# acproject/wsi-segmentation-pipeline

Hardware: AMD Instinct MI355X
Metric: patches/sec (256×256×3) whole-slide inference, 1/2/4/8 MI355X + CPU ref (higher is better)
Workload: dtype fp16 + MX-fp6 cross terms (fp32 accumulate); 1 GPU; cfg3: ONE 40000x40000 synthetic slide, tile 256 stride 256 -> 24648 tiles sharded over 1 rank(s) (each holds only its own slide regions: 4.80 GB on rank 0), ResNet-18 trunk + Classifier, fused read+normalise+conv HIP path, 1 all-gather, float64 stitch + softmax; tiles_total=24648, batch=6200, mode=mx, parallelism=tile-shard x1 + 1 all-gather, batches_in_flight=2

## Files before the change

### include/wsi_hip.h

```cpp
#ifndef WSI_HIP_H
#define WSI_HIP_H
#include <stddef.h>
#include <stdint.h>

#ifdef __cplusplus
extern "C" {
#endif

#define WSI_HIP_ABI_VERSION 8
int wsi_hip_abi_version(void);

size_t wsi_pf_bytes(int n, int h, int w, int c, int planes);
long long wsi_pf_pixel_index(int n, int y, int x, int h, int w);

size_t wsi_prepack_conv_bytes(int cout, int cin, int k, int planes);
int wsi_prepack_conv(const float* w, const float* bn_weight, const float* bn_bias, const float* bn_mean,
                     const float* bn_var, float eps, int cout, int cin, int k, int planes, void* wpk_out,
                     float* bias_out);
size_t wsi_prepack_stem_bytes(int planes);
int wsi_prepack_stem(const float* w, const float* bn_weight, const float* bn_bias, const float* bn_mean,
                     const float* bn_var, float eps, int planes, void* wpk_out, float* bias_out);
int wsi_prepack_stem_u8(const float* w, const float* bn_weight, const float* bn_bias, const float* bn_mean,
                        const float* bn_var, float eps, const float mean[3], const float std_[3], int planes,
                        void* wpk_out, float* bias_out);
int wsi_normalize_u8_lut(const float mean[3], const float std_[3], float* lut_out );

int wsi_stem_conv7x7_bn_relu_maxpool(const float* in_f32, const uint8_t* slide, long long slide_pitch_bytes,
                                     int slide_h, int slide_w, const int* tile_xy, const float* lut,
                                     const void* stem_wpk, const float* stem_bias,
                                     const void* stem_wpk_u8 ,
                                     const float* stem_bias_u8, const float* norm_mean_std ,
                                     int n, int h, int w, float* scratch, void* out_pf, int planes, void* stream);

enum {
    WSI_STEM_MODE_UNFUSED = 0,
    WSI_STEM_MODE_FUSED = 1,
    WSI_STEM_MODE_FUSED_LUT = 2,
    WSI_STEM_MODE_FUSED_ONE_STRIP = 3
};
int wsi_stem_set_mode(int fused, int rows_per_seg);

int wsi_conv3x3_bn_act(const void* in_pf, void* out_pf, const void* resid_pf, const void* wpk, const float* bias,
                       int n, int h_in, int w_in, int cin, int cout, int stride, int relu, int planes,
                       void* stream);
int wsi_conv1x1_bn(const void* in_pf, void* out_pf, const void* wpk, const float* bias, int n, int h_in, int w_in,
                   int cin, int cout, int stride, int planes, void* stream);
int wsi_conv3x3_up_concat_bn_act(const void* up_pf, const void* skip_pf, void* out_pf, const void* wpk, const float* bias, int n, int h, int w,
                                 int c_up, int c_skip, int cout, int relu, int planes, void* stream);
int wsi_conv3x3s2_ds_fused(const void* in_pf, void* out_conv_pf, void* out_ds_pf, const void* wpk3, const float* bias3,
                           const void* wpk1, const float* bias1, int n, int h_in, int w_in, int cin, int cout, int planes,
                           void* stream);
int wsi_s2_slab_images(int n, int h_in, int w_in, int cin, int planes);
size_t wsi_pf_split_bytes(int n, int h, int w, int c, int planes);
int wsi_conv3x3_bn_act_split(const void* in_pf, void* out_split, const void* resid_pf, const void* wpk, const float* bias,
                             int n, int h, int w, int cin, int cout, int relu, int planes, void* stream);
int wsi_conv3x3s2_ds_fused_split(const void* in_split, void* out_conv_pf, void* out_ds_pf, const void* wpk3,
                                 const float* bias3, const void* wpk1, const float* bias1, int n, int h_in, int w_in,
                                 int cin, int cout, int planes, void* stream);
enum {
    WSI_CONV_MODE_S2_GATHER = 0,
    WSI_CONV_MODE_S2_SLAB = 1,
    WSI_CONV_MODE_S2_SLAB_128 = 3,
    WSI_CONV_MODE_XCD_ORDER = 8,
    WSI_CONV_MODE_WIDE_FROM_256 = 16,
    WSI_CONV_MODE_WIDE_NEVER = 32,
    WSI_CONV_MODE_S2_ABLATE = 64,
    WSI_CONV_MODE_NO_S2_SPLIT = 128,
    WSI_CONV_MODE_XCD_RANGES_OFF = 256,
    WSI_CONV_MODE_XCD_RANGES_L1 = 512,
    WSI_CONV_MODE_L1_SLAB3 = 1024,
    WSI_CONV_MODE_NO_DS_FOLD = 2048,
    WSI_CONV_MODE_NO_SLAB_PAIR = 4096,
    WSI_CONV_MODE_L1_LINES128 = 16384,
    WSI_CONV_MODE_S2_NT2 = 32768,
    WSI_CONV_MODE_UNET_CONCAT_PASS = 65536,
    WSI_CONV_MODE_WIDE_NO_D8 = 131072,
    WSI_CONV_MODE_L1_PERSISTENT = 1048576,
    WSI_CONV_MODE_UNET_NO_TAIL = 2097152,
    WSI_CONV_MODE_UNET_TAIL_FORM1 = 4194304,
    WSI_CONV_MODE_UNET_X0_UNFUSED = 8388608
};
int wsi_conv_set_mode(int mode);
int wsi_conv3x3_bn_act_cfg(const void* in_pf, void* out_pf, const void* resid_pf, const void* wpk, const float* bias,
                           int n, int h_in, int w_in, int cin, int cout, int stride, int relu, int planes, int cfg,
                           void* stream);

int wsi_avgpool_fc(const void* in_pf, int n, int h, int w, int c, const float* fc_w, const float* fc_b, int k,
                   float* feat_out, float* logits_out, int planes, void* stream);
int wsi_linear(const float* x, const float* w, const float* bias, float* y, int b, int k, int j, int relu,
               void* stream);

int wsi_pf_pack(const float* in_nchw, void* out_pf, int n, int c, int h, int w, int planes, void* stream);
int wsi_pf_unpack(const void* in_pf, float* out_nchw, int n, int c, int h, int w, int planes, void* stream);

typedef struct {
    const void* stem_w;   const float* stem_b;
    const void* stem_w_u8; const float* stem_b_u8;
    float norm[6];
    const void* conv_w[16]; const float* conv_b[16];
    const void* down_w[3];  const float* down_b[3];
    const float* head_w;  const float* head_b;  int head_k;
    int planes;
} wsi_trunk_weights;

size_t wsi_trunk_workspace_bytes(int n, int h, int w, int planes);
int wsi_trunk_workspace_init(void* workspace, int n, int h, int w, int planes, void* stream);
int wsi_trunk_workspace_release(void* workspace);
int wsi_trunk_forward(const wsi_trunk_weights* wt, const float* in_f32, const uint8_t* slide,
                      long long slide_pitch_bytes, int slide_h, int slide_w, const int* tile_xy, const float* lut,
                      int n, int h, int w, void* workspace, int workspace_n, float* feat_out ,
                      float* logits_out , float* fmap_out ,
                      void* stream);
int wsi_trunk_set_chunks(int stem_chunk, int layer1_chunk);
int wsi_trunk_forward_tap(const wsi_trunk_weights* wt, const float* in_f32, const uint8_t* slide,
                          long long slide_pitch_bytes, int slide_h, int slide_w, const int* tile_xy, const float* lut,
                          int n, int h, int w, void* workspace, int workspace_n, int stop_after, float* tap_out_nchw,
                          void* stream);

int wsi_prof_begin(int max_records);
int wsi_prof_end(float* ms_out, int* kind_out, double* flops_out, int cap);

int wsi_tile_gather(const uint8_t* slide, long long slide_pitch_bytes, int slide_h, int slide_w, const int* tile_xy,
                    const float* lut, float* out_nchw, int n, int ph, int pw, void* stream);
int wsi_stitch_add(const float* tile_logits, const int* map_xy, int t, int c, int dy, int dx, double* pred, int map_h,
                   int map_w, void* stream);
int wsi_stitch_add_dense(const float* tile_pred, const int* map_xy, int t, int c, int ph, int pw, double* pred, int map_h,
                         int map_w, void* stream);
int wsi_softmax_threshold_argmax(const double* pred, int c, long long hw, const double* class_thresh, double* probs,
                                 uint8_t* classes, const uint8_t* mask, int heat_mode, uint8_t* heat, void* stream);
typedef struct wsi_ring wsi_ring;
typedef struct wsi_resample_plan wsi_resample_plan;
int wsi_ring_create(wsi_ring** out, int slots, size_t slot_bytes);
void* wsi_ring_host_slot(wsi_ring* ring, int slot);
int wsi_ring_wait_slot(wsi_ring* ring, int slot);
int wsi_ring_submit(wsi_ring* ring, int slot, int rows, int width, int channels, long long src_pitch, uint8_t* level_rows, long long level_pitch);
int wsi_ring_acquire(wsi_ring* ring, void* compute_stream);
int wsi_ring_fence(wsi_ring* ring, void* compute_stream);
int wsi_ring_device(const wsi_ring* ring);
int wsi_ring_drain(wsi_ring* ring);
void wsi_ring_destroy(wsi_ring* ring);
int wsi_resample_plan_create(wsi_resample_plan** out, int in_h, int in_w, int out_h, int out_w);
void wsi_resample_plan_destroy(wsi_resample_plan* plan);
size_t wsi_resample_scratch_bytes(const wsi_resample_plan* plan, int n);
int wsi_resample_tiles(const wsi_resample_plan* plan, const uint8_t* slide, long long pitch, int sh, int sw, const int* tile_xy, int n,
                       uint8_t* out, void* scratch, void* stream);
int wsi_find_nuclei_hsv(const uint8_t* rgb, long long npix, int pixel_stride, double mu_percent, uint8_t* mask_out, void* stream);
size_t wsi_connected_components_scratch_bytes(int h, int w);
int wsi_connected_components(const uint8_t* mask, int h, int w, int* labels_out, int* count_out, void* scratch, void* stream);
int wsi_kmeans_points(const int* points_xy, int n, double* centres_xy, int k, int max_iters, int* labels_out, void* scratch, void* stream);
int wsi_kmeans_seed_farthest(const int* points_xy, int n, int k, double* centres_xy_out, void* scratch, void* stream);
int wsi_find_nuclei_lab(const uint8_t* rgb, long long npix, int pixel_stride, double mu_percent, uint8_t* mask_out, void* scratch, void* stream);
size_t wsi_fill_holes_scratch_bytes(int h, int w);
int wsi_fill_holes(const uint8_t* mask, int h, int w, uint8_t* out, void* scratch, void* stream);
size_t wsi_slic_scratch_bytes(int h, int w, int k);
int wsi_slic(const uint8_t* rgb, int h, int w, const double* gauss_weights, int radius, double* segments, int k, int step_y, int step_x,
             double step, double compactness, int iters, int* labels_out, void* scratch, void* stream);
long long wsi_tile_grid_candidates(int iw, int ih, int ph, int pw, int sh, int sw);
size_t wsi_tile_grid_scratch_bytes(long long candidates);
int wsi_tile_grid(int iw, int ih, int ph, int pw, int sh, int sw, const uint8_t* mask, int mask_h, int mask_w, double m, double thresh,
                  int* tile_xy_out, int* count_out, void* scratch, void* stream);
int wsi_exponent_span(const float* values, long long n, int* out2, void* stream);
int wsi_paint_regions(const long long* pixel_idx, const int* region_of, long long n, const uint8_t* region_class, int* winner_scratch,
                      long long* label, long long npix, void* stream);

int wsi_resize_bilinear_f64(const double* src, int c, int hs, int ws, double* dst, int hd, int wd, void* stream);
int wsi_argmax_classes(const double* pred, int c, long long hw, uint8_t* classes, void* stream);
int wsi_morph_rect(const uint8_t* src, uint8_t* dst, uint8_t* tmp, int h, int w, int k, int op, void* stream);
int wsi_bwperim(const uint8_t* src, uint8_t* dst, int h, int w, void* stream);
size_t wsi_tumor_bed_workspace_bytes(int h, int w);
int wsi_convex_hull_image(const uint8_t* src, uint8_t* dst, int h, int w, void* workspace, void* stream);
int wsi_tumor_bed(const uint8_t* codes, int h, int w, int min_code, int open_k, int dilate_k, uint8_t* opened_out,
                  uint8_t* tb_pred_out, uint8_t* outline_out, void* workspace, void* stream);
int wsi_hull_polygon(void* workspace, int h, int w, double* out_xy, int cap, int* count_out, void* stream);
int wsi_mask_iou_counts(const uint8_t* a, const uint8_t* b, long long n, unsigned long long* out2, void* stream);
int wsi_score_counts(const uint8_t* p, const uint8_t* gt, const uint8_t* mask, long long n, unsigned long long* out6,
                     void* stream);
int wsi_esp(const double* pts_xy, int n, int num_pts, double* out_xy, double* scratch, void* stream);

typedef struct {
    const void* conv_w[10]; const float* conv_b[10];
    int cin[10], cout[10];
    const float* head_w; const float* head_b;
    int head_cin, classes;
    const void* tail_w;
} wsi_unet_decoder_weights;
size_t wsi_unet_tail_prepack_bytes(void);
int wsi_unet_tail_prepack(const float* w1, const float* bn1_weight, const float* bn1_bias, const float* bn1_mean, const float* bn1_var,
                          const float* w2, const float* bn2_weight, const float* bn2_bias, const float* bn2_mean, const float* bn2_var,
                          float eps, const float* head_w, const float* head_b, int cin, int cmid, int classes, void* out);
int wsi_unet_tail_bands(int n, int h, int cus);
int wsi_unet_tail_timeouts(unsigned long long* out, int reset);
size_t wsi_unet_workspace_bytes(const wsi_unet_decoder_weights* dw, int n, int h, int w, int planes);
int wsi_unet_workspace_init(const wsi_unet_decoder_weights* dw, void* workspace, int n, int h, int w, int planes, void* stream);
int wsi_unet_forward(const wsi_trunk_weights* wt, const wsi_unet_decoder_weights* dw, const float* in_f32, const uint8_t* slide,
                     long long slide_pitch_bytes, int slide_h, int slide_w, const int* tile_xy, const float* lut, int n, int h,
                     int w, void* workspace, int workspace_n, float* logits_out, float* enc_out[5], void* stream);
int wsi_unet_decoder(const wsi_unet_decoder_weights* dw, const float* const enc_nchw[5], int n, int h, int w, int planes,
                     void* workspace, int workspace_n, float* logits_out, void* stream);
int wsi_resize_nearest_f32(const float* src, long long planes_n, int hs, int ws, float* dst, int hd, int wd, void* stream);

#ifdef __cplusplus
}
#endif
#endif
```

### wsi_segmentation_pipeline_amd/csrc/capi.hip

```cpp
#include "internal.h"
#include "../../include/wsi_hip.h"

ConvRoutes g_routes;

StemArgs stem_args(const TileSource& src, const void* wpk, const float* bias, float* scratch, int n, int h, int w) {
    StemArgs a;
    a.mode = src.in_f32 ? 0 : 1;
    a.in_f32 = src.in_f32; a.slide = src.slide; a.slide_pitch = src.pitch; a.SH = src.SH; a.SW = src.SW;
    a.origins = src.tile_xy; a.lut = src.lut; a.wpk = wpk; a.bias = bias; a.out = scratch;
    a.N = n; a.H = h; a.W = w; a.wpk_u8 = nullptr; a.bias_u8 = nullptr;
    return a;
}

int stem_run(const TileSource& src, const void* stem_wpk, const float* stem_bias, const void* stem_wpk_u8, const float* stem_bias_u8,
             const float* norm_mean_std, int n, int h, int w, float* scratch, void* out_pf, int planes, void* stream, int out96,
             long long plane96, void* x0_pf) {
    if (!stem_wpk || !stem_bias || !scratch || !out_pf || n <= 0 || h % 16 || w % 4) return WSI_EINVAL;
    if (!src.valid()) return WSI_EINVAL;
    StemArgs a = stem_args(src, stem_wpk, stem_bias, scratch, n, h, w);
    if (stem_wpk_u8 && stem_bias_u8 && norm_mean_std && !src.in_f32 && g_routes.stem_u8x) { a.wpk_u8 = stem_wpk_u8; a.bias_u8 = stem_bias_u8; }
    if (out96 && planes != 3) return WSI_EINVAL;
    if (x0_pf && !(a.wpk_u8 && g_routes.stem_fused && planes == 2)) return WSI_EINVAL;
    if (g_routes.stem_fused || planes == 3) return wsi_stem_pool_dispatch(a, out_pf, planes, g_routes.stem_rows, (hipStream_t)stream, out96, plane96, x0_pf);
    int rc = wsi_stem_dispatch(a, planes, (hipStream_t)stream);
    if (rc) return rc;
    return wsi_maxpool_dispatch(scratch, out_pf, n, h / 2, w / 2, planes, (hipStream_t)stream);
}

#ifdef WSI_STUDY
static void* g_study_debug = nullptr;
extern "C" int wsi_study_set_debug(void* dev_buf) { g_study_debug = dev_buf; return WSI_OK; }
#endif

static ConvArgs conv_args(const ConvCall& c) {
    ConvArgs a;
    a.in = c.in; a.out = c.out; a.resid = c.resid; a.wpk = c.wpk; a.bias = c.bias;
    a.gi = pf_geom_fd(c.n, c.h, c.w, c.cin);
    a.go = pf_geom_fd(c.n, c.h / c.stride, c.w / c.stride, c.cout);
    a.stride = c.stride; a.ksize = c.ksize; a.relu = c.relu & 1; a.flags = 0;
    a.out2 = nullptr; a.wpk2 = nullptr; a.bias2 = nullptr;
    a.in_split_pixels = 0; a.out_split_pixels = 0;
    return a;
}

int conv_common(const ConvCall& c) {
    const hipStream_t st = (hipStream_t)c.stream;
    int cfg = c.cfg;
    if ((!c.in && !(c.in_up && c.up_c == c.cin)) || !c.out || !c.wpk || !c.bias || c.in == c.out || c.in_up == c.out || c.n <= 0) return WSI_EINVAL;
    if (c.line_flags && (c.planes != 3 || c.stride != 1 || c.ksize != 3 || c.cin != 64 || c.cout != 64 || (c.split_out && (c.line_flags & CONV_OUT96)) ||
                         (c.line_flags & ~(CONV_IN96 | CONV_OUT96 | CONV_RESID96)) || ((c.line_flags & CONV_RESID96) && !c.resid)))
        return WSI_EINVAL;
    if ((c.stride != 1 && c.stride != 2) || c.h % c.stride || c.w % c.stride) return WSI_EINVAL;
    if (c.planes == 3 && c.stride == 2 && c.resid) return WSI_EINVAL;
    ConvArgs a = conv_args(c);
    a.plane96 = c.line_flags ? (c.plane96 > 0 ? c.plane96 : (long long)pf_alloc_pixels(c.n, c.h, c.w) * 96) : 0;
#ifdef WSI_STUDY
    if (c.relu & 2) a.flags |= CONV_ABL_NO_STORE;
    if (c.relu & 64) a.flags |= CONV_ABL_DISPATCH_ONLY;
    if (c.relu & 128) a.flags |= CONV_ABL_NO_MAINLOOP;
    if (c.relu & 256) a.flags |= CONV_NONTEMPORAL;
    if (c.relu & 512) a.flags |= CONV_XCD_ORDER;
    if (c.relu & 16384) a.flags |= CONV_XCD_RANGES;
    if (c.relu & 65536) a.flags |= CONV_RESID_DIRECT;
    a.flags |= ((c.relu >> 10) & 15) << CONV_WCOPIES_SHIFT;
#else
    if (c.relu & ~1) return WSI_EINVAL;
#endif
    a.flags |= c.line_flags;
    if (c.in_up) {
        if (c.stride != 1 || c.ksize != 3 || c.h % 2 || c.w % 2 || c.up_c <= 0 || c.up_c > c.cin || c.resid || c.in2 || c.line_flags || c.split_out) return WSI_EINVAL;
        a.in_up = c.in_up; a.up_c = c.up_c; a.gup = pf_geom_fd(c.n, c.h / 2, c.w / 2, c.up_c);
    }
    if (c.in2) {
        if (c.planes != 3 || c.stride != 1 || c.ksize != 3 || c.resid || !c.wpk2 || !c.bias2 || c.in2_c <= 0 || c.in2_c % 32 || c.cout % 128 || cfg >= 0) return WSI_EINVAL;
        a.in2 = c.in2; a.in2_c = c.in2_c; a.wpk2 = c.wpk2; a.bias2 = c.bias2;
        cfg = 60;
    }
#ifdef WSI_STUDY
    if (cfg == 75 || cfg == 76) a.out2 = g_study_debug;
#endif
    a.out_split_pixels = c.split_out ? (c.split_pixels ? c.split_pixels : pf_alloc_pixels(c.n, c.h / 2, c.w / 2)) : 0;
    if (c.split_out && (c.stride != 1 || c.ksize != 3 || c.h % 2 || c.w % 2 || c.planes < 2)) return WSI_EINVAL;
    if (c.ksize == 3 && c.stride == 2 && c.cout % 128 == 0 && cfg != 0 && g_routes.s2_slab) {
        const int rc = wsi_s2_dispatch(a, c.planes, st);
        if (rc != WSI_EINVAL) return rc;
    }
    return wsi_conv_dispatch(a, c.planes, cfg, st);
}

static ConvArgs s2_ds_args(const void* in, void* out_conv_pf, void* out_ds_pf, const void* wpk3, const float* bias3, const void* wpk1,
                           const float* bias1, int n, int h_in, int w_in, int cin, int cout) {
    ConvArgs a = conv_args({.in = in, .out = out_conv_pf, .wpk = wpk3, .bias = bias3, .n = n, .h = h_in, .w = w_in, .cin = cin, .cout = cout,
                            .stride = 2, .ksize = 3, .relu = 1});
    a.out2 = out_ds_pf; a.wpk2 = out_ds_pf ? wpk1 : nullptr; a.bias2 = out_ds_pf ? bias1 : nullptr;
    return a;
}

static bool s2_ds_ok(const void* in, const void* out_conv_pf, const void* out_ds_pf, const void* wpk3, const float* bias3, const void* wpk1,
                     const float* bias1, int n, int h_in, int w_in, bool ds_optional) {
    if (!in || !out_conv_pf || !wpk3 || !bias3 || n <= 0 || h_in % 2 || w_in % 2) return false;
    if (out_ds_pf ? (!wpk1 || !bias1) : !ds_optional) return false;
    return in != out_conv_pf && in != out_ds_pf && out_conv_pf != out_ds_pf;
}

int s2_split_common(const void* in_split, void* out_conv_pf, void* out_ds_pf, const void* wpk3, const float* bias3, const void* wpk1,
                    const float* bias1, int n, int h_in, int w_in, int cin, int cout, int planes, void* stream, long long split_pixels) {
    if (!s2_ds_ok(in_split, out_conv_pf, out_ds_pf, wpk3, bias3, wpk1, bias1, n, h_in, w_in, true)) return WSI_EINVAL;
    ConvArgs a = s2_ds_args(in_split, out_conv_pf, out_ds_pf, wpk3, bias3, wpk1, bias1, n, h_in, w_in, cin, cout);
    a.in_split_pixels = split_pixels ? split_pixels : pf_alloc_pixels(n, h_in / 2, w_in / 2);
    return wsi_s2_dispatch(a, planes, (hipStream_t)stream);
}

extern "C" {

int wsi_hip_abi_version(void) { return WSI_HIP_ABI_VERSION; }

size_t wsi_pf_bytes(int n, int h, int w, int c, int planes) {
    if (n <= 0 || h <= 0 || w <= 0 || c <= 0 || planes < 1 || planes > 3) return 0;
    return (size_t)pf_alloc_pixels(n, h, w) * (size_t)c * (planes == 1 ? 2 : 4);
}
long long wsi_pf_pixel_index(int n, int y, int x, int h, int w) {
    return (long long)(w + 2) + (long long)n * (h + 1) * (w + 1) + (long long)y * (w + 1) + x;
}

int wsi_stem_set_mode(int fused, int rows_per_seg) {
    if (rows_per_seg <= 0) return WSI_EINVAL;
    g_routes.stem_fused = fused != WSI_STEM_MODE_UNFUSED; g_routes.stem_rows = rows_per_seg;
    g_routes.stem_u8x = fused != WSI_STEM_MODE_FUSED_LUT;
    g_routes.stem_shared_weights = fused != WSI_STEM_MODE_FUSED_ONE_STRIP;
    return WSI_OK;
}

int wsi_stem_conv7x7_bn_relu_maxpool(const float* in_f32, const uint8_t* slide, long long slide_pitch_bytes,
                                     int slide_h, int slide_w, const int* tile_xy, const float* lut,
                                     const void* stem_wpk, const float* stem_bias, const void* stem_wpk_u8,
                                     const float* stem_bias_u8, const float* norm_mean_std, int n, int h, int w,
                                     float* scratch, void* out_pf, int planes, void* stream) {
    return stem_run({in_f32, slide, slide_pitch_bytes, slide_h, slide_w, tile_xy, lut}, stem_wpk, stem_bias, stem_wpk_u8, stem_bias_u8,
                    norm_mean_std, n, h, w, scratch, out_pf, planes, stream, 0);
}

int wsi_conv3x3_bn_act(const void* in_pf, void* out_pf, const void* resid_pf, const void* wpk, const float* bias,
                       int n, int h_in, int w_in, int cin, int cout, int stride, int relu, int planes,
                       void* stream) {
    return conv_common({.in = in_pf, .out = out_pf, .resid = resid_pf, .wpk = wpk, .bias = bias, .n = n, .h = h_in, .w = w_in, .cin = cin,
                        .cout = cout, .stride = stride, .ksize = 3, .relu = relu, .planes = planes, .stream = stream});
}

size_t wsi_pf_split_bytes(int n, int h, int w, int c, int planes) {
    if (h % 2 || w % 2) return 0;
    return 4 * wsi_pf_bytes(n, h / 2, w / 2, c, planes);
}

int wsi_conv3x3_bn_act_split(const void* in_pf, void* out_split, const void* resid_pf, const void* wpk, const float* bias,
                             int n, int h, int w, int cin, int cout, int relu, int planes, void* stream) {
    return conv_common({.in = in_pf, .out = out_split, .resid = resid_pf, .wpk = wpk, .bias = bias, .n = n, .h = h, .w = w, .cin = cin,
                        .cout = cout, .stride = 1, .ksize = 3, .relu = relu, .planes = planes, .stream = stream, .split_out = 1});
}

int wsi_conv3x3s2_ds_fused_split(const void* in_split, void* out_conv_pf, void* out_ds_pf, const void* wpk3,
                                 const float* bias3, const void* wpk1, const float* bias1, int n, int h_in, int w_in,
                                 int cin, int cout, int planes, void* stream) {
    return s2_split_common(in_split, out_conv_pf, out_ds_pf, wpk3, bias3, wpk1, bias1, n, h_in, w_in, cin, cout, planes, stream, 0);
}

int wsi_conv3x3_bn_act_cfg(const void* in_pf, void* out_pf, const void* resid_pf, const void* wpk, const float* bias,
                           int n, int h_in, int w_in, int cin, int cout, int stride, int relu, int planes, int cfg,
                           void* stream) {
    return conv_common({.in = in_pf, .out = out_pf, .resid = resid_pf, .wpk = wpk, .bias = bias, .n = n, .h = h_in, .w = w_in, .cin = cin,
                        .cout = cout, .stride = stride, .ksize = 3, .relu = relu, .planes = planes, .stream = stream, .cfg = cfg});
}

int wsi_conv3x3_up_concat_bn_act(const void* up_pf, const void* skip_pf, void* out_pf, const void* wpk, const float* bias, int n, int h, int w,
                                 int c_up, int c_skip, int cout, int relu, int planes, void* stream) {
    if (!up_pf || c_up <= 0 || c_skip < 0 || (c_skip > 0 && !skip_pf)) return WSI_EINVAL;
    return conv_common({.in = c_skip ? skip_pf : nullptr, .out = out_pf, .wpk = wpk, .bias = bias, .n = n, .h = h, .w = w, .cin = c_up + c_skip,
                        .cout = cout, .stride = 1, .ksize = 3, .relu = relu, .planes = planes, .stream = stream, .in_up = up_pf, .up_c = c_up});
}

int wsi_s2_slab_images(int n, int h_in, int w_in, int cin, int planes) {
    if (n <= 0 || h_in <= 0 || w_in <= 0 || cin <= 0 || planes < 1 || planes > 3) return WSI_EINVAL;
    const unsigned long long pix = (unsigned long long)cin * (planes == 1 ? PFmt<1>::BPC : PFmt<2>::BPC);
    auto fits = [&](int m) { return (unsigned long long)pf_alloc_pixels(m, h_in, w_in) * pix < 0xffffffffull; };
    if (fits(n)) return n;
    if (!fits(1)) return 0;
    int lo = 1, hi = n;
    while (hi - lo > 1) {
        const int mid = lo + (hi - lo) / 2;
        (fits(mid) ? lo : hi) = mid;
    }
    return lo;
}

int wsi_conv3x3s2_ds_fused(const void* in_pf, void* out_conv_pf, void* out_ds_pf, const void* wpk3, const float* bias3,
                           const void* wpk1, const float* bias1, int n, int h_in, int w_in, int cin, int cout, int planes,
                           void* stream) {
    if (!s2_ds_ok(in_pf, out_conv_pf, out_ds_pf, wpk3, bias3, wpk1, bias1, n, h_in, w_in, false)) return WSI_EINVAL;
    ConvArgs a = s2_ds_args(in_pf, out_conv_pf, out_ds_pf, wpk3, bias3, wpk1, bias1, n, h_in, w_in, cin, cout);
    const int per = wsi_s2_slab_images(n, h_in, w_in, cin, planes);
    const size_t bpc = planes == 1 ? PFmt<1>::BPC : PFmt<2>::BPC;
    const size_t in_img = (size_t)(h_in + 1) * (w_in + 1) * cin * bpc, out_img = (size_t)(h_in / 2 + 1) * (w_in / 2 + 1) * cout * bpc;
    int rc = WSI_EINVAL;
    for (int n0 = 0; per > 0 && n0 < n; n0 += per) {
        const int nn = n - n0 < per ? n - n0 : per;
        a.in = (const char*)in_pf + n0 * in_img;
        a.out = (char*)out_conv_pf + n0 * out_img;
        a.out2 = (char*)out_ds_pf + n0 * out_img;
        a.gi = pf_geom_fd(nn, h_in, w_in, cin);
        a.go = pf_geom_fd(nn, h_in / 2, w_in / 2, cout);
        rc = wsi_s2_dispatch(a, planes, (hipStream_t)stream);
        if (rc) break;
    }
    if (rc == WSI_EINVAL) {
        ConvCall c = {.in = in_pf, .out = out_conv_pf, .wpk = wpk3, .bias = bias3, .n = n, .h = h_in, .w = w_in, .cin = cin, .cout = cout,
                      .stride = 2, .ksize = 3, .relu = 1, .planes = planes, .stream = stream, .cfg = 0};
        rc = conv_common(c);
        c.out = out_ds_pf; c.wpk = wpk1; c.bias = bias1; c.ksize = 1; c.relu = 0;
        if (!rc) rc = conv_common(c);
    }
    return rc;
}

int wsi_conv_set_mode(int mode) {
    ConvRoutes& r = g_routes;
    const int base = mode & 7;
    r.s2_slab = base != WSI_CONV_MODE_S2_GATHER;
    r.s2_small_tiles = base != WSI_CONV_MODE_S2_SLAB_128;
    r.xcd_order = (mode & WSI_CONV_MODE_XCD_ORDER) ? 1 : 0;
    r.wide_min_c = (mode & WSI_CONV_MODE_WIDE_FROM_256) ? 256 : (mode & WSI_CONV_MODE_WIDE_NEVER) ? (1 << 30) : 128;
    r.s2_ablate = (mode & WSI_CONV_MODE_S2_ABLATE) ? 1 : 0;
    r.s2_split = (mode & WSI_CONV_MODE_NO_S2_SPLIT) ? 0 : 1;
    r.xcd_ranges = (mode & WSI_CONV_MODE_XCD_RANGES_OFF) ? 0 : (mode & WSI_CONV_MODE_XCD_RANGES_L1) ? 1 : 2;
    r.l1_rows = (mode & WSI_CONV_MODE_L1_SLAB3) ? 0 : 1;
    r.ds_fold = (mode & WSI_CONV_MODE_NO_DS_FOLD) ? 0 : 1;
    r.slab_pair = (mode & WSI_CONV_MODE_NO_SLAB_PAIR) ? 0 : 1;
    r.l1_lines96 = (mode & WSI_CONV_MODE_L1_LINES128) ? 0 : 1;
    r.s2_nt4 = (mode & WSI_CONV_MODE_S2_NT2) ? 0 : 1;
    r.unet_fuse_up = (mode & WSI_CONV_MODE_UNET_CONCAT_PASS) ? 0 : 1;
    r.wide_d8 = (mode & WSI_CONV_MODE_WIDE_NO_D8) ? 0 : 1;
    r.l1p = (mode & WSI_CONV_MODE_L1_PERSISTENT) ? 1 : 0;
    r.unet_tail = (mode & WSI_CONV_MODE_UNET_NO_TAIL) ? 0 : 1;
    r.unet_tail_form = (mode & WSI_CONV_MODE_UNET_TAIL_FORM1) ? 1 : 2;
    r.unet_x0_fused = (mode & WSI_CONV_MODE_UNET_X0_UNFUSED) ? 0 : 1;
    return WSI_OK;
}

int wsi_conv1x1_bn(const void* in_pf, void* out_pf, const void* wpk, const float* bias, int n, int h_in, int w_in,
                   int cin, int cout, int stride, int planes, void* stream) {
    return conv_common({.in = in_pf, .out = out_pf, .wpk = wpk, .bias = bias, .n = n, .h = h_in, .w = w_in, .cin = cin, .cout = cout,
                        .stride = stride, .ksize = 1, .relu = 0, .planes = planes, .stream = stream});
}

int wsi_avgpool_fc(const void* in_pf, int n, int h, int w, int c, const float* fc_w, const float* fc_b, int k,
                   float* feat_out, float* logits_out, int planes, void* stream) {
    if (!in_pf || n <= 0 || (logits_out && (!fc_w || !fc_b || k <= 0))) return WSI_EINVAL;
    return wsi_avgpool_fc_dispatch(in_pf, pf_geom(n, h, w, c), fc_w, fc_b, k, feat_out, logits_out, planes,
                                   (hipStream_t)stream);
}

int wsi_linear(const float* x, const float* w, const float* bias, float* y, int b, int k, int j, int relu,
               void* stream) {
    if (!x || !w || !y) return WSI_EINVAL;
    return wsi_linear_dispatch(x, w, bias, y, b, k, j, relu, (hipStream_t)stream);
}

int wsi_pf_pack(const float* in_nchw, void* out_pf, int n, int c, int h, int w, int planes, void* stream) {
    if (!in_nchw || !out_pf || n <= 0 || planes < 1 || planes > 3 || c % (planes == 1 ? 64 : 32)) return WSI_EINVAL;
    return wsi_pf_pack_dispatch(in_nchw, out_pf, pf_geom(n, h, w, c), planes, (hipStream_t)stream);
}

int wsi_pf_unpack(const void* in_pf, float* out_nchw, int n, int c, int h, int w, int planes, void* stream) {
    if (!in_pf || !out_nchw || n <= 0 || planes < 1 || planes > 3 || c % (planes == 1 ? 64 : 32)) return WSI_EINVAL;
    return wsi_pf_unpack_dispatch(in_pf, out_nchw, pf_geom(n, h, w, c), planes, (hipStream_t)stream);
}

int wsi_tile_gather(const uint8_t* slide, long long slide_pitch_bytes, int slide_h, int slide_w, const int* tile_xy,
                    const float* lut, float* out_nchw, int n, int ph, int pw, void* stream) {
    if (!slide || !tile_xy || !lut || !out_nchw) return WSI_EINVAL;
    return wsi_tile_gather_dispatch(slide, slide_pitch_bytes, slide_h, slide_w, tile_xy, lut, out_nchw, n, ph, pw,
                                    (hipStream_t)stream);
}

int wsi_stitch_add(const float* tile_logits, const int* map_xy, int t, int c, int dy, int dx, double* pred, int map_h,
                   int map_w, void* stream) {
    if (!tile_logits || !map_xy || !pred || map_h <= 0 || map_w <= 0) return WSI_EINVAL;
    return wsi_stitch_add_dispatch(tile_logits, map_xy, t, c, dy, dx, pred, map_h, map_w, (hipStream_t)stream);
}

int wsi_stitch_add_dense(const float* tile_pred, const int* map_xy, int t, int c, int ph, int pw, double* pred, int map_h,
                         int map_w, void* stream) {
    if (!tile_pred || !map_xy || !pred || map_h <= 0 || map_w <= 0) return WSI_EINVAL;
    return wsi_stitch_add_dense_dispatch(tile_pred, map_xy, t, c, ph, pw, pred, map_h, map_w, (hipStream_t)stream);
}

int wsi_softmax_threshold_argmax(const double* pred, int c, long long hw, const double* class_thresh, double* probs,
                                 uint8_t* classes, const uint8_t* mask, int heat_mode, uint8_t* heat, void* stream) {
    if (!pred || !class_thresh) return WSI_EINVAL;
    return wsi_softmax_dispatch(pred, c, hw, class_thresh, probs, classes, mask, heat_mode, heat, (hipStream_t)stream);
}

int wsi_find_nuclei_hsv(const uint8_t* rgb, long long npix, int pixel_stride, double mu_percent, uint8_t* mask_out, void* stream) {
    if (!rgb || !mask_out) return WSI_EINVAL;
    return wsi_hsv_mask_dispatch(rgb, npix, pixel_stride, mu_percent, mask_out, (hipStream_t)stream);
}
size_t wsi_connected_components_scratch_bytes(int h, int w) { return (h <= 0 || w <= 0) ? 0 : wsi_cc_scratch_bytes(h, w); }
int wsi_connected_components(const uint8_t* mask, int h, int w, int* labels_out, int* count_out, void* scratch, void* stream) {
    if (!mask || !labels_out || !scratch) return WSI_EINVAL;
    return wsi_cc_dispatch(mask, h, w, labels_out, count_out, scratch, (hipStream_t)stream);
}
int wsi_find_nuclei_lab(const uint8_t* rgb, long long npix, int pixel_stride, double mu_percent, uint8_t* mask_out, void* scratch, void* stream) {
    return wsi_lab_mask_dispatch(rgb, npix, pixel_stride, mu_percent, mask_out, scratch, (hipStream_t)stream);
}
int wsi_fill_holes(const uint8_t* mask, int h, int w, uint8_t* out, void* scratch, void* stream) {
    return wsi_fill_holes_dispatch(mask, h, w, out, scratch, (hipStream_t)stream);
}
int wsi_slic(const uint8_t* rgb, int h, int w, const double* gauss_weights, int radius, double* segments, int k, int step_y, int step_x,
             double step, double compactness, int iters, int* labels_out, void* scratch, void* stream) {
    return wsi_slic_dispatch(rgb, h, w, gauss_weights, radius, segments, k, step_y, step_x, step, compactness, iters, labels_out, scratch,
                             (hipStream_t)stream);
}
int wsi_kmeans_points(const int* points_xy, int n, double* centres_xy, int k, int max_iters, int* labels_out, void* scratch, void* stream) {
    if (!points_xy || !centres_xy || !labels_out || !scratch) return WSI_EINVAL;
    return wsi_kmeans_dispatch(points_xy, n, centres_xy, k, max_iters, labels_out, scratch, (hipStream_t)stream);
}

int wsi_kmeans_seed_farthest(const int* points_xy, int n, int k, double* centres_xy_out, void* scratch, void* stream) {
    if (!points_xy || !centres_xy_out || !scratch) return WSI_EINVAL;
    return wsi_kmeans_seed_farthest_dispatch(points_xy, n, k, centres_xy_out, scratch, (hipStream_t)stream);
}

int wsi_tile_grid(int iw, int ih, int ph, int pw, int sh, int sw, const uint8_t* mask, int mask_h, int mask_w, double m, double thresh,
                  int* tile_xy_out, int* count_out, void* scratch, void* stream) {
    if (!tile_xy_out || !count_out || !scratch) return WSI_EINVAL;
    return wsi_tile_grid_dispatch(iw, ih, ph, pw, sh, sw, mask, mask_h, mask_w, m, thresh, tile_xy_out, count_out, scratch, (hipStream_t)stream);
}

int wsi_exponent_span(const float* values, long long n, int* out2, void* stream) {
    if (!values || !out2) return WSI_EINVAL;
    return wsi_exponent_span_dispatch(values, n, out2, (hipStream_t)stream);
}

int wsi_paint_regions(const long long* pixel_idx, const int* region_of, long long n, const uint8_t* region_class, int* winner_scratch,
                      long long* label, long long npix, void* stream) {
    if (!region_class || !winner_scratch || !label || (n && (!pixel_idx || !region_of))) return WSI_EINVAL;
    return wsi_paint_dispatch(pixel_idx, region_of, n, region_class, winner_scratch, label, npix, (hipStream_t)stream);
}

int wsi_resize_bilinear_f64(const double* src, int c, int hs, int ws, double* dst, int hd, int wd, void* stream) {
    if (!src || !dst || src == dst) return WSI_EINVAL;
    return wsi_resize_dispatch(src, c, hs, ws, dst, hd, wd, (hipStream_t)stream);
}
int wsi_argmax_classes(const double* pred, int c, long long hw, uint8_t* classes, void* stream) {
    if (!pred || !classes) return WSI_EINVAL;
    return wsi_argmax_dispatch(pred, c, hw, classes, (hipStream_t)stream);
}
int wsi_morph_rect(const uint8_t* src, uint8_t* dst, uint8_t* tmp, int h, int w, int k, int op, void* stream) {
    if (!src || !dst || !tmp) return WSI_EINVAL;
    return wsi_morph_dispatch(src, dst, tmp, h, w, k, op, (hipStream_t)stream);
}
int wsi_bwperim(const uint8_t* src, uint8_t* dst, int h, int w, void* stream) {
    if (!src || !dst) return WSI_EINVAL;
    return wsi_bwperim_dispatch(src, dst, h, w, (hipStream_t)stream);
}
size_t wsi_tumor_bed_workspace_bytes(int h, int w) {
    if (h <= 0 || w <= 0) return 0;
    return 3 * align_up((size_t)h * w, 256) + align_up(wsi_hull_ws_bytes(h), 256);
}
int wsi_convex_hull_image(const uint8_t* src, uint8_t* dst, int h, int w, void* workspace, void* stream) {
    if (!src || !dst || !workspace || src == dst) return WSI_EINVAL;
    return wsi_hull_dispatch(src, dst, h, w, (char*)workspace + 3 * align_up((size_t)h * w, 256), (hipStream_t)stream);
}
int wsi_tumor_bed(const uint8_t* codes, int h, int w, int min_code, int open_k, int dilate_k, uint8_t* opened_out,
                  uint8_t* tb_pred_out, uint8_t* outline_out, void* workspace, void* stream) {
    if (!codes || !tb_pred_out || !outline_out || !workspace || h <= 0 || w <= 0 || open_k <= 0 || dilate_k <= 0 ||
        tb_pred_out == outline_out)
        return WSI_EINVAL;
    hipStream_t st = (hipStream_t)stream;
    const size_t plane = align_up((size_t)h * w, 256);
    uint8_t *A = (uint8_t*)workspace, *B = A + plane, *Cc = B + plane;
    void* hws = Cc + plane;
    int rc = wsi_threshold_dispatch(codes, (long long)h * w, min_code, A, st);
    if (!rc) rc = wsi_morph_dispatch(A, B, Cc, h, w, open_k, 2, st);
    if (!rc && opened_out && hipMemcpyAsync(opened_out, B, (size_t)h * w, hipMemcpyDeviceToDevice, st) != hipSuccess) rc = WSI_EFAULT;
    if (!rc) rc = wsi_hull_dispatch(B, tb_pred_out, h, w, hws, st);
    if (!rc) rc = wsi_bwperim_dispatch(tb_pred_out, A, h, w, st);
    if (!rc) rc = wsi_morph_dispatch(A, outline_out, Cc, h, w, dilate_k, 1, st);
    return rc;
}
int wsi_hull_polygon(void* workspace, int h, int w, double* out_xy, int cap, int* count_out, void* stream) {
    if (!workspace || !out_xy || !count_out || h <= 0 || w <= 0 || cap <= 0) return WSI_EINVAL;
    char* hws = (char*)workspace + 3 * align_up((size_t)h * w, 256);
    int rc = wsi_hull_polygon_dispatch(hws, h, out_xy, cap, (hipStream_t)stream);
    if (rc) return rc;
    const int* counts = (const int*)hws + 2 * (2 * (size_t)h + 1);
    return hipMemcpyAsync(count_out, counts + 2, sizeof(int), hipMemcpyDeviceToDevice, (hipStream_t)stream) == hipSuccess ? WSI_OK : WSI_EFAULT;
}
// ... 20 lines not shown
```

### wsi_segmentation_pipeline_amd/csrc/common.h

```cpp
#pragma once
#include <hip/hip_runtime.h>
#include <stdint.h>

typedef __attribute__((ext_vector_type(8))) __bf16 bf16x8;
typedef __attribute__((ext_vector_type(4))) __bf16 bf16x4;
typedef __attribute__((ext_vector_type(16))) float f32x16;
typedef __attribute__((ext_vector_type(4))) float f32x4;

#define WSI_OK 0
#define WSI_EINVAL (-22)
#define WSI_ENOMEM (-12)
#define WSI_EFAULT (-14)

struct FastDiv { unsigned m; int s; };
static inline FastDiv fastdiv_make(int d) {
    FastDiv f;
    if (d <= 1) { f.m = 0u; f.s = -1; return f; }
    int l = 0;
    while ((1ll << l) < d) ++l;
    f.m = (unsigned)(((1ull << (31 + l)) / (unsigned long long)d) + 1ull);
    f.s = l - 1;
    return f;
}
#ifdef __HIPCC__
static inline __device__ int fd_div(int i, const FastDiv& f) { return f.s < 0 ? i : (int)(__umulhi((unsigned)i, f.m) >> f.s); }
#endif

struct PFGeom {
    int N, H, W, C;
    int P, S, G;
    int NS;
    FastDiv dHW, dW, dS, dP;
};

static inline __host__ __device__ PFGeom pf_geom(int n, int h, int w, int c) {
    PFGeom g;
    g.N = n; g.H = h; g.W = w; g.C = c;
    g.P = w + 1; g.S = (h + 1) * (w + 1); g.G = w + 2; g.NS = n * g.S;
    g.dHW.m = g.dW.m = g.dS.m = g.dP.m = 0u; g.dHW.s = g.dW.s = g.dS.s = g.dP.s = 0;
    return g;
}
static inline PFGeom pf_geom_fd(int n, int h, int w, int c) {
    PFGeom g = pf_geom(n, h, w, c);
    g.dHW = fastdiv_make(h * w); g.dW = fastdiv_make(w); g.dS = fastdiv_make(g.S); g.dP = fastdiv_make(g.P);
    return g;
}
static inline __device__ int pf_pos_of_index(const PFGeom& g, int i) {
    const int n = fd_div(i, g.dHW), rem = i - n * (g.H * g.W);
    const int y = fd_div(rem, g.dW), x = rem - y * g.W;
    return g.G + n * g.S + y * g.P + x;
}

#define PF_TILE_ROUND 512

static inline __host__ __device__ long long pf_alloc_pixels(int n, int h, int w) {
    long long P = w + 1, S = (long long)(h + 1) * P, G = P + 1;
    long long body = ((long long)n * S + PF_TILE_ROUND - 1) / PF_TILE_ROUND * PF_TILE_ROUND;
    return 2 * G + body + PF_TILE_ROUND;
}

static inline __device__ bool pf_is_pixel(const PFGeom& g, int q) {
    int r = q - g.G;
    if (r < 0 || r >= g.NS) return false;
    int x = r % g.P;
    int y = (r / g.P) % (g.H + 1);
    return x != g.W && y != g.H;
}

template <int PLANES> struct PFmt {
    static constexpr int BPC = PLANES == 1 ? 2 : 4;
    static constexpr int CPL = PLANES == 1 ? 64 : 32;
};
typedef __attribute__((ext_vector_type(8))) _Float16 f16x8;
typedef __attribute__((ext_vector_type(4))) _Float16 f16x4;
typedef __attribute__((ext_vector_type(8))) int i32x8;
typedef __attribute__((ext_vector_type(4))) unsigned int u32x4;
typedef __attribute__((ext_vector_type(2))) float f32x2;
typedef __attribute__((ext_vector_type(2))) _Float16 f16x2;
typedef __attribute__((ext_vector_type(4))) int i32x4;

struct ConvArgs {
    const void* in;
    void* out;
    const void* resid;
    const void* wpk;
    const float* bias;
    PFGeom gi, go;
    int stride;
    int ksize;
    int relu;
    int flags;
    void* out2;
    const void* wpk2;
    const float* bias2;
    long long out_split_pixels, in_split_pixels;
    int mtiles = 0;
    const void* in2 = nullptr;
    int in2_c = 0;
    const void* in_up = nullptr;
    int up_c = 0;
    PFGeom gup = {};
    long long plane96 = 0;
};

enum : int {
    CONV_XCD_ORDER = 1,
    CONV_XCD_RANGES = 2,
    CONV_RESID_DIRECT = 4,
    CONV_IN96 = 16, CONV_OUT96 = 32, CONV_RESID96 = 64,
    CONV_ABL_NO_STORE = 1 << 8, CONV_ABL_DISPATCH_ONLY = 1 << 9, CONV_ABL_NO_MAINLOOP = 1 << 10, CONV_NONTEMPORAL = 1 << 11,
    CONV_WCOPIES_SHIFT = 16,
};
#ifdef WSI_STUDY
#define CONV_STUDY(a, bits) ((a).flags & (bits))
#else
#define CONV_STUDY(a, bits) 0
#endif

static inline __device__ size_t pf_out_offset(const PFGeom& g, long long split_pixels, int q, size_t pixstride) {
    if (!split_pixels) return (size_t)q * pixstride;
    int r = q - g.G;
    const int n = fd_div(r, g.dS);
    r -= n * g.S;
    const int y = fd_div(r, g.dP), x = r - y * g.P;
    const int P2 = g.W / 2 + 1, S2 = (g.H / 2 + 1) * P2;
    const long long q2 = (long long)(P2 + 1) + (long long)n * S2 + (y >> 1) * P2 + (x >> 1);
    return (size_t)(((y & 1) * 2 + (x & 1)) * split_pixels + q2) * pixstride;
}

static inline __device__ f32x16 mfma_bf16(bf16x8 a, bf16x8 b, f32x16 c) {
    return __builtin_amdgcn_mfma_f32_32x32x16_bf16(a, b, c, 0, 0, 0);
}
template <int PLANES> struct PairElem { typedef __bf16 T; };
template <> struct PairElem<2> { typedef _Float16 T; };
template <int PLANES>
static inline __device__ f32x16 mfma16(bf16x8 a, bf16x8 b, f32x16 c) {
    typedef __attribute__((ext_vector_type(8))) _Float16 h8;
    if constexpr (PLANES == 2) return __builtin_amdgcn_mfma_f32_32x32x16_f16(__builtin_bit_cast(h8, a), __builtin_bit_cast(h8, b), c, 0, 0, 0);
    else return __builtin_amdgcn_mfma_f32_32x32x16_bf16(a, b, c, 0, 0, 0);
}

typedef __attribute__((ext_vector_type(6))) unsigned u32x6;
typedef __attribute__((ext_vector_type(16))) unsigned u32x16;
typedef __attribute__((ext_vector_type(32))) float f32x32;
static inline __host__ __device__ int mx6_scale_byte(float amax) {
    union { float f; unsigned u; } c;
    c.f = amax;
    const unsigned u = c.u & 0x7fffffffu;
    if (u == 0u) return 0;
    const int e = (int)(u >> 23) - 2 + ((u & 0x7fffffu) > 0x780000u ? 1 : 0);
    return e < 1 ? 1 : (e > 254 ? 254 : e);
}
static inline __host__ __device__ float mx_scale_value(int s) {
    union { float f; unsigned u; } c;
    c.u = (unsigned)s << 23;
    return c.f;
}
static inline __host__ __device__ int mx_line_pos(int c) { return 16 * ((c >> 2) & 1) + 4 * (c >> 3) + (c & 3); }
static inline __host__ __device__ int mx_line_chan(int p) { return 8 * ((p & 15) >> 2) + 4 * (p >> 4) + (p & 3); }
static inline __host__ __device__ int mx6_field_of_pos(int p) { return 2 * (p & 15) + (p >> 4); }
static inline __host__ __device__ int mx6_field_chan(int f) { return mx_line_chan(16 * (f & 1) + (f >> 1)); }
#define MX6_PLANE_LO(q) (64 + 16 * (q))
#define MX6_PLANE_HI(q) (96 + 16 * (q))
#define MX6_SCALE(q) (104 + 16 * (q))

static inline __host__ __device__ float fp6_value(unsigned c) {
    const int e = (c >> 3) & 3, m = c & 7;
    const float v = e ? (float)(8 + m) * (e == 1 ? 0.125f : e == 2 ? 0.25f : 0.5f) : (float)m * 0.125f;
    return (c & 32) ? -v : v;
}
static inline __host__ __device__ unsigned fp6_encode(float y) {
    union { float f; unsigned u; } c;
    c.f = y;
    const unsigned sign = (c.u >> 31) ? 32u : 0u;
    c.u &= 0x7fffffffu;
    const float a = c.f;
    if (!(a < 7.5f)) return sign | 31u;
    const float step = a < 2.f ? 0.125f : a < 4.f ? 0.25f : 0.5f;
    const float t = a / step;
    float r = (float)(int)t;
    const float frac = t - r;
    if (frac > 0.5f || (frac == 0.5f && ((int)r & 1))) r += 1.f;
    const float q = r * step;
    unsigned code;
    if (q < 1.f) code = (unsigned)(q * 8.f);
    else if (q < 2.f) code = 8u + (unsigned)((q - 1.f) * 8.f);
    else if (q < 4.f) code = 16u + (unsigned)((q - 2.f) * 4.f);
    else code = 24u + (unsigned)((q - 4.f) * 2.f);
    return sign | code;
}
static inline __host__ __device__ unsigned mx6_get_field(const unsigned* w, int f) {
    const int bit = 6 * f, d = bit >> 5, s = bit & 31;
    unsigned v = w[d] >> s;
    if (s > 26) v |= w[d + 1] << (32 - s);
    return v & 63u;
}
static inline __host__ __device__ void mx6_set_field(unsigned* w, int f, unsigned code) {
    const int bit = 6 * f, d = bit >> 5, s = bit & 31;
    w[d] |= code << s;
    if (s > 26) w[d + 1] |= code >> (32 - s);
}

#ifdef __HIPCC__
static __device__ __forceinline__ u32x6 mx6_pack32(f32x16 a, f32x16 b, float scale) {
    u32x6 r;
    asm volatile("v_cvt_scalef32_2xpk16_fp6_f32 %0, %1, %2, %3" : "=&v"(r) : "v"(a), "v"(b), "v"(scale));
    return r;
}
static __device__ __forceinline__ f32x32 mx6_unpack32(u32x6 q, float scale) {
    f32x32 r;
    asm volatile("v_cvt_scalef32_pk32_f32_fp6 %0, %1, %2" : "=&v"(r) : "v"(q), "v"(scale));
    return r;
}
static __device__ __forceinline__ void swap32_halves(f32x16& a, f32x16& b) {
#pragma unroll
    for (int k = 0; k < 16; k += 8) {
        float a0 = a[k], a1 = a[k + 1], a2 = a[k + 2], a3 = a[k + 3], a4 = a[k + 4], a5 = a[k + 5], a6 = a[k + 6], a7 = a[k + 7];
        float b0 = b[k], b1 = b[k + 1], b2 = b[k + 2], b3 = b[k + 3], b4 = b[k + 4], b5 = b[k + 5], b6 = b[k + 6], b7 = b[k + 7];
        asm volatile("s_nop 1\n\tv_permlane32_swap_b32 %0, %8\n\tv_permlane32_swap_b32 %1, %9\n\tv_permlane32_swap_b32 %2, %10\n\t"
                     "v_permlane32_swap_b32 %3, %11\n\tv_permlane32_swap_b32 %4, %12\n\tv_permlane32_swap_b32 %5, %13\n\t"
                     "v_permlane32_swap_b32 %6, %14\n\tv_permlane32_swap_b32 %7, %15\n\ts_nop 1"
                     : "+v"(a0), "+v"(a1), "+v"(a2), "+v"(a3), "+v"(a4), "+v"(a5), "+v"(a6), "+v"(a7),
                       "+v"(b0), "+v"(b1), "+v"(b2), "+v"(b3), "+v"(b4), "+v"(b5), "+v"(b6), "+v"(b7));
        a[k] = a0; a[k + 1] = a1; a[k + 2] = a2; a[k + 3] = a3; a[k + 4] = a4; a[k + 5] = a5; a[k + 6] = a6; a[k + 7] = a7;
        b[k] = b0; b[k + 1] = b1; b[k + 2] = b2; b[k + 3] = b3; b[k + 4] = b4; b[k + 5] = b5; b[k + 6] = b6; b[k + 7] = b7;
    }
}
static __device__ __forceinline__ void pair_max2(float& x, float& y) {
    float x2 = x, y2 = y;
    asm volatile("s_nop 1\n\tv_permlane32_swap_b32 %0, %1\n\tv_permlane32_swap_b32 %2, %3\n\ts_nop 1" : "+v"(x), "+v"(x2), "+v"(y), "+v"(y2));
    x = fmaxf(x, x2);
    y = fmaxf(y, y2);
}

#endif

static inline __device__ void split_f16(float x, _Float16& hi, _Float16& lo) {
    x = __builtin_amdgcn_fmed3f(x, -65504.f, 65504.f);
    hi = (_Float16)x;
    lo = (_Float16)(x - (float)hi);
}
static inline __device__ void split_f16x4(const float* v, f16x4& hi, f16x4& lo) {
#pragma unroll
    for (int i = 0; i < 4; ++i) {
        _Float16 a, b;
        split_f16(v[i], a, b);
        hi[i] = a;
        lo[i] = b;
    }
}
static inline __device__ const float* conv_wscale_inv(const void* wpk, int cout, int cin, int ksize) {
    return (const float*)((const char*)wpk + (size_t)(cout / 32) * (cin / 32) * ksize * ksize * 4096);
}

struct StemArgs {
    int mode;
    const float* in_f32;
    const uint8_t* slide;
    long long slide_pitch;
    int SH, SW;
    const int* origins;
    const float* lut;
    const void* wpk;
    const float* bias;
    float* out;
    int N, H, W;
    const void* wpk_u8;
    const float* bias_u8;
    void* out_pf = nullptr;
    int out_planes = 0;
};

struct ConvRoutes {
    int stem_fused = 1;
    int stem_rows = 64;
    int stem_u8x = 1;
    int stem_shared_weights = 1;
    int chunk_stem = 0;
    int chunk_l1 = 0;
    int s2_slab = 1;
    int s2_small_tiles = 1;
    int xcd_order = 0;
    int wide_min_c = 128;
    int s2_ablate = 0;
    int s2_split = 1;
    int xcd_ranges = 2;
    int l1_rows = 1;
    int ds_fold = 1;
    int slab_pair = 1;
    int l1_lines96 = 1;
    int s2_nt4 = 1;
    int unet_fuse_up = 1;
    int wide_d8 = 1;
    int l1p = 0;
    int unet_tail = 1;
    int unet_tail_form = 2;
    int unet_x0_fused = 1;
};
extern ConvRoutes g_routes;
```

### wsi_segmentation_pipeline_amd/csrc/conv.hip

```cpp
#include "conv_dev.h"
#include "internal.h"

template <int MT, int WM, int WN, int PLANES>
__global__ __launch_bounds__(WM* WN * 64) void conv_gather_kernel(ConvArgs a) {
    extern __shared__ __attribute__((aligned(16))) char smem[];
    constexpr int BM = WM * MT * 32;
    constexpr int NTHREADS = WM * WN * 64;
    constexpr int PPT = BM * 8 / NTHREADS;
    constexpr int PIX_STEP = NTHREADS / 8;
    const int tid = threadIdx.x, lane = tid & 63, wave = tid >> 6;
    const int wm = wave / WN, wn = wave % WN;
    const int l31 = lane & 31, h = lane >> 5;
    const int nblocks = a.go.C / (WN * 32);
    const int nb = blockIdx.x % nblocks;
    const int mtile = blockIdx.x / nblocks;
    const int q0 = a.go.G + mtile * BM;
    const int ntile = nb * WN + wn;
    const int NC = a.gi.C / PFmt<PLANES>::CPL;
    const int KS = a.ksize, NT = KS * KS, pad = KS / 2;
    const size_t in_pixstride = (size_t)a.gi.C * PFmt<PLANES>::BPC;
    const bf16x8* wbase = (const bf16x8*)a.wpk + (size_t)ntile * NC * NT * 4 * 64 + lane;

    int inq[PPT];
    const int sp = tid & 7;
// ... 547 lines not shown
        asm volatile("s_waitcnt lgkmcnt(0)" ::: "memory");
        __builtin_amdgcn_s_barrier();
        asm volatile("" ::: "memory");
    };

    const int ntile = wn;
    const __amdgpu_buffer_rsrc_t wrs = __builtin_amdgcn_make_buffer_rsrc(
        (void*)((const char*)a.wpk + (size_t)ntile * NC * 9 * 4096), 0, NC * 9 * 4096, 0x00020000);
    const int wvoff = lane * 16;
    f32x16 acc[1][MT];
    bf16x8 wbuf[3][4], xf[2][4];
    auto wload = [&](bf16x8(&w)[4], int soff) {
#pragma unroll
        for (int f = 0; f < 4; ++f)
            w[f] = __builtin_bit_cast(bf16x8, __builtin_amdgcn_raw_buffer_load_b128(wrs, wvoff, soff + f * 1024, 0));
    };
    const int xoff0 = wm * 32 + l31;

    if (producer) {
        dma_slab(0);
        asm volatile("s_waitcnt vmcnt(0)" ::: "memory");
    }
    barrier();
    if (producer && nunits > 1) dma_slab(1);
    mx96_rebuild_hi6(smem, NPIX, tid, 320);
    barrier();

    for (int k = 0; k < ntl; ++k) {
#pragma unroll
    for (int c = 0; c < NC; ++c) {
        const int u = k * NC + c;
        const bool last_line = c == NC - 1;
        if (producer) {
            asm volatile("s_waitcnt vmcnt(0)" ::: "memory");
        } else {
            const char* const xl = smem + (c & 1) * L1P_SLAB;
            auto xload = [&](bf16x8(&x)[4], int Pl) {
                asm volatile("" : "+v"(Pl));
                const int base = lds_xbase(Pl, h);
#pragma unroll
                for (int f = 0; f < 4; ++f) x[f] = *(const bf16x8*)(xl + (base ^ (f << 5)));
            };
            if (c == 0) acc_init_bias<MT>(acc[0], a.bias, ntile, lane);
#pragma unroll
            for (int dy = 0; dy < 3; ++dy) wload(wbuf[dy], (c * 9 + dy * 3) * 4096);
            int Pc = P;
            asm volatile("" : "+s"(Pc));
            const int sline = c * 9 * 4096;
            xload(xf[0], xoff0);
#pragma unroll
            for (int dx = 0; dx < 3; ++dx) {
#pragma unroll
                for (int j = 0; j < 6; ++j) {
                    const int kk = dx * 6 + j;
                    if (j < 5) xload(xf[(kk + 1) & 1], xoff0 + (j + 1) * Pc + dx);
                    else if (dx < 2) xload(xf[(kk + 1) & 1], xoff0 + dx + 1);
                    __builtin_amdgcn_sched_barrier(0);
#pragma unroll
                    for (int mt = 0; mt < MT; ++mt) {
                        const int dy = j - mt;
                        if (dy >= 0 && dy < 3) acc[0][mt] = mfma_mx6(acc[0][mt], wbuf[dy], xf[kk & 1]);
                    }
                    __builtin_amdgcn_sched_barrier(0);
                    if (j >= 3 && dx < 2) {
                        wload(wbuf[j - 3], sline + ((j - 3) * 3 + dx + 1) * 4096);
                        __builtin_amdgcn_sched_barrier(0);
                    }
                }
            }
        }
        barrier();
        if (producer) {
            if (u + 2 < nunits) dma_slab(u + 2);
            if (a.resid && u + 1 < nunits && (u + 1) % NC == NC - 1) dma_resid((u + 1) / NC);
        }
        if (u + 1 < nunits) mx96_rebuild_hi6(smem + ((c + 1) & 1) * L1P_SLAB, NPIX, tid, 320);
        barrier();
        if (!producer && last_line) {
            const int p0 = tile_p0(k);
            int qs[MT];
            bool valid[MT];
#pragma unroll
            for (int mt = 0; mt < MT; ++mt) {
                qs[mt] = p0 + mt * P + wm * 32 + l31;
                valid[mt] = true;
            }
            if (a.resid) {
                bf16x8 iw[4];
                {
                    int lo = l31;
                    asm volatile("" : "+v"(lo));
                    const int pp = mx_line_pos(lo), f0 = mx6_field_of_pos(pp);
                    f16x8 k0, k1;
#pragma unroll
                    for (int jj = 0; jj < 8; ++jj) {
                        k0[jj] = (pp == 8 * h + jj) ? (_Float16)1.0f : (_Float16)0.0f;
                        k1[jj] = (pp == 16 + 8 * h + jj) ? (_Float16)1.0f : (_Float16)0.0f;
                    }
                    unsigned q[6];
#pragma unroll
                    for (int d = 0; d < 6; ++d) {
                        const int bit = 6 * f0 + 3 - 32 * d;
                        q[d] = (h == 0 && bit >= 0 && bit < 32) ? (1u << (bit & 31)) : 0u;
                    }
                    iw[0] = __builtin_bit_cast(bf16x8, k0);
                    iw[1] = __builtin_bit_cast(bf16x8, k1);
                    iw[2] = __builtin_bit_cast(bf16x8, u32x4{q[0], q[1], q[2], q[3]});
                    iw[3] = __builtin_bit_cast(bf16x8, u32x4{q[4], q[5], 127u, 0u});
                }
#pragma unroll
                for (int mt = 0; mt < MT; ++mt) {
                    const char* t = stage + (wave * MT + mt) * 3072 + l31 * 96;
                    bf16x8 x[4];
                    x[0] = *(const bf16x8*)(t + h * 16);
                    x[1] = *(const bf16x8*)(t + (2 + h) * 16);
                    if (h == 0) {
                        x[2] = *(const bf16x8*)(t + 4 * 16);
                        x[3] = *(const bf16x8*)(t + 5 * 16);
                    } else {
                        x[2] = __builtin_bit_cast(bf16x8, u32x4{0u, 0u, 0u, 0u});
                        x[3] = x[2];
                    }
                    acc[0][mt] = mfma_mx6(acc[0][mt], iw, x);
                }
            }
            conv_epilogue_mx<MT>(a, acc[0], qs, valid, ntile, lane);
        }
    }
    }
}

static int g_l1p_grid = 0;
static int launch_l1p(const ConvArgs& a, hipStream_t st) {
    if (a.go.C != 64 || a.gi.C % 32 || a.gi.C < 64 || a.gi.W != 64 || a.gi.H % 4 || a.in2 || a.in_up || !(a.flags & CONV_IN96) ||
        (a.resid && !(a.flags & CONV_RESID96)))
        return WSI_EINVAL;
    if (!g_l1p_grid) {
        int dev = 0, cus = 0;
        if (hipGetDevice(&dev) != hipSuccess || hipDeviceGetAttribute(&cus, hipDeviceAttributeMultiprocessorCount, dev) != hipSuccess || cus < 8)
            return WSI_EFAULT;
        g_l1p_grid = cus / 8 * 8;
    }
    const long long mtiles = (long long)a.gi.N * a.gi.H * a.gi.W / 256;
    int grid = g_l1p_grid;
    if (mtiles < grid) grid = (int)((mtiles + 7) / 8 * 8);
    if (a.gi.C != 64) return WSI_EINVAL;
    auto k = conv3x3s1_l1p_kernel<2>;
    if (hipFuncSetAttribute((const void*)k, hipFuncAttributeMaxDynamicSharedMemorySize, L1P_LDS) != hipSuccess) return WSI_EINVAL;
    hipLaunchKernelGGL(k, dim3(grid), dim3(320), L1P_LDS, st, a);
    return hipGetLastError() == hipSuccess ? WSI_OK : WSI_EFAULT;
}


template <int PLANES, int MINW, int ABL = 0, int WM = 2, int WN = 2, int NT = 2, bool D8 = false>
__global__ __launch_bounds__(WM* WN * 64, MINW) void conv3x3s1_wide_kernel(ConvArgs a) {
    extern __shared__ __attribute__((aligned(16))) char smem[];
    constexpr int MT = 4, BM = WM * 128, NTHREADS = WM * WN * 64, NTILES = WN * NT, WB = NTILES * 4096;
    constexpr int D8_ZB = 304;
    static_assert(!D8 || (BM == 256 && NTHREADS == 256), "D8: four whole 8 x 8 images per tile, 32 slab pixels per DMA round");
    constexpr int RESID_NBUF = 4;
    char* const wl = smem;
    char* const xl = smem + 2 * WB;
    const int tid = threadIdx.x, lane = tid & 63;
    WSTAMP(const unsigned long long st_begin = __builtin_readcyclecounter(); unsigned long long st_pro = 0, st_line = 0, st_tap = 0, st_a = 0;)
    const int wave = __builtin_amdgcn_readfirstlane(tid >> 6);
    const int wm = wave / WN, wn = wave % WN;
    const int l31 = lane & 31, h = lane >> 5;
    const int nblocks = a.go.C / (NTILES * 32);
    int nb = blockIdx.x % nblocks, mtile = blockIdx.x / nblocks;
    if (a.flags & CONV_XCD_RANGES) {
        const int chunk = gridDim.x >> 3, lin = (blockIdx.x & 7) * chunk + (blockIdx.x >> 3);
        nb = lin % nblocks;
        mtile = lin / nblocks;
        if (mtile >= (a.gi.N * a.gi.H * a.gi.W + BM - 1) / BM) return;
    }
    const int P = a.gi.P;
    const int NC = a.gi.C / PFmt<PLANES>::CPL;
    const size_t in_pixstride = (size_t)a.gi.C * PFmt<PLANES>::BPC;
    int xoff[MT];
    bool valid[MT];
    int slab0, npieces;
    const int lpix = a.gi.W < 32 ? dense_lane_pixel(l31) : l31;
    const int Rtot = a.gi.N * a.gi.H * a.gi.W;
    if constexpr (D8) {
        const int i0 = mtile * BM, i1 = min(i0 + BM, Rtot) - 1, n0 = i0 >> 6;
        slab0 = a.gi.G + n0 * a.gi.S - P;
        npieces = (1 + 9 * ((i1 >> 6) - n0 + 1)) * 64;
#pragma unroll
        for (int mt = 0; mt < MT; ++mt) {
            const int i = i0 + wm * MT * 32 + mt * 32 + lpix;
            valid[mt] = i < Rtot;
            const int ii = valid[mt] ? i : i1;
            xoff[mt] = 8 * (9 * ((ii >> 6) - n0) + ((ii >> 3) & 7)) + (ii & 7) - 1;
        }
    } else {
        auto pos = [&](int i) { return pf_pos_of_index(a.gi, i); };
        const int i0 = mtile * BM, i1 = min(i0 + BM, Rtot) - 1;
        slab0 = pos(i0) - P - 1;
        npieces = (pos(i1) + P + 1 - slab0 + 1) * 8;
#pragma unroll
        for (int mt = 0; mt < MT; ++mt) {
            const int i = i0 + wm * MT * 32 + mt * 32 + lpix;
            valid[mt] = i < Rtot;
            xoff[mt] = pos(valid[mt] ? i : i1) - slab0 - (P + 1);
        }
    }
    const bool d8_left = D8 && (lpix & 7) == 0, d8_right = D8 && (lpix & 7) == 7;
    constexpr int RPIX = D8 ? 36 : NTHREADS / 8;
    static_assert((NTHREADS / 8) % 16 == 0, "whole swizzle periods per DMA round");
    const size_t slab_byte0 = (size_t)slab0 * in_pixstride;
    const size_t in_bytes = (size_t)pf_alloc_pixels(a.gi.N, a.gi.H, a.gi.W) * in_pixstride;
    const __amdgpu_buffer_rsrc_t xrs = __builtin_amdgcn_make_buffer_rsrc(
        (void*)((const char*)a.in + slab_byte0), 0, (int)min(in_bytes - slab_byte0, (size_t)0x7fffffff), 0x00020000);
    int xvoff;
    {
        const int i = wave * 64 + lane, Pl = i >> 3, sl = (i & 7) ^ ((Pl >> 1) & 7);
        xvoff = (D8 ? (Pl >> 3) * 9 + (Pl & 7) : Pl) * (int)in_pixstride + sl * 16;
    }
    if constexpr (D8) {
        if (tid < 128) *(u32x4*)(xl + D8_ZB * 128 + tid * 16) = u32x4{0u, 0u, 0u, 0u};
    }
    const __amdgpu_buffer_rsrc_t wrs = __builtin_amdgcn_make_buffer_rsrc(
        (void*)((const char*)a.wpk + (size_t)(nb * NTILES) * NC * 9 * 4096), 0, NTILES * NC * 9 * 4096, 0x00020000);
    const int wvoff = (tid & 255) * 16;
    const unsigned wl_addr = lds_addr_of(wl), xl_addr = lds_addr_of(xl);
    auto wdma = [&](int c, int t, int wboff) {
#pragma unroll
        for (int p0 = 0; p0 < NTILES * 256; p0 += NTHREADS) {
            static_assert((NTILES * 256) % NTHREADS == 0, "whole DMA rounds");
            const int pw = p0 + wave * 64;
            dma16_buf_asm(wrs, wl_addr + wboff + pw * 16, wvoff, (((pw >> 8) * NC + c) * 9 + t) * 4096);
        }
    };

    f32x16 acc[NT][MT];
#pragma unroll
    for (int nt = 0; nt < NT; ++nt) {
        if constexpr (PLANES == 3) acc_init_bias<MT>(acc[nt], a.bias, nb * NTILES + wn * NT + nt, lane);
        else {
#pragma unroll
            for (int mt = 0; mt < MT; ++mt)
#pragma unroll
                for (int r = 0; r < 16; ++r) acc[nt][mt][r] = 0.f;
        }
    }

    auto xload = [&](bf16x8(&x)[4], int Pl, int tx = 1) {
        asm volatile("" : "+v"(Pl));
        if constexpr (D8) {
            if (tx == 0) Pl = d8_left ? D8_ZB + (Pl & 15) : Pl;
            if (tx == 2) Pl = d8_right ? D8_ZB + (Pl & 15) : Pl;
        }
        const int base = lds_xbase(Pl, h);
#pragma unroll
        for (int f = 0; f < 4; ++f) x[f] = *(const bf16x8*)(xl + (base ^ (f << 5)));
    };
    auto wread = [&](bf16x8(&w)[4], const char* wb, int nt) {
        const char* src = wb + (wn * NT + nt) * 4096 + lane * 16;
#pragma unroll
        for (int f = 0; f < 4; ++f) w[f] = *(const bf16x8*)(src + f * 1024);
    };

    int kpar = 0;
    WSTAMP(const unsigned long long st_setup = __builtin_readcyclecounter();)
    for (int c = 0; c < NC; ++c) {
        WSTAMP(st_a = __builtin_readcyclecounter();)
        if (c) __syncthreads();
        for (int i0 = wave * 64, r = 0; i0 < npieces; i0 += NTHREADS, ++r)
            dma16_buf_asm(xrs, xl_addr + i0 * 16, xvoff, c * 128 + r * RPIX * (int)in_pixstride);
        wdma(c, 0, kpar * WB);
        asm volatile("s_waitcnt vmcnt(0)" ::: "memory");
        __syncthreads();
        WSTAMP(if (c) st_line += __builtin_readcyclecounter() - st_a; else st_pro = __builtin_readcyclecounter() - st_a;)
        int Pc = D8 ? 8 : P;
        asm volatile("" : "+s"(Pc));
        bf16x8 xf[2][4], wf[NT][4];
        xload(xf[0], xoff[0], 0);
#pragma unroll
        for (int t = 0; t < 9; ++t) {
            const char* wb = wl + kpar * WB;
            if (t < 8) wdma(c, t + 1, (kpar ^ 1) * WB);
#pragma unroll
            for (int nt = 0; nt < NT; ++nt) wread(wf[nt], wb, nt);
            const int toff = (t / 3) * Pc + (t % 3);
            const int toff_next = ((t + 1) / 3) * Pc + ((t + 1) % 3);
#pragma unroll
            for (int mt = 0; mt < MT; ++mt) {
                const int k = t * MT + mt;
                if constexpr (!(ABL & 32)) {
                    if (mt + 1 < MT) xload(xf[(k + 1) & 1], xoff[mt + 1] + toff, t % 3);
                    else if (t < 8) xload(xf[(k + 1) & 1], xoff[0] + toff_next, (t + 1) % 3);
                }
                __builtin_amdgcn_sched_barrier(0);
                const bf16x8(&x)[4] = xf[k & 1];
#pragma unroll
                for (int nt = 0; nt < NT; ++nt) {
                    mfma_step<PLANES>(acc[nt][mt], wf[nt], x);
                }
            }
            if (t < 8) {
                WSTAMP(st_a = __builtin_readcyclecounter();)
                asm volatile("s_waitcnt vmcnt(0)" ::: "memory");
                __syncthreads();
                WSTAMP(st_tap += __builtin_readcyclecounter() - st_a;)
            }
            kpar ^= 1;
        }
    }
    WSTAMP(const unsigned long long st_loop_end = __builtin_readcyclecounter();)
    int qs[MT];
#pragma unroll
    for (int mt = 0; mt < MT; ++mt) {
        if constexpr (D8) {
            const int i = mtile * BM + wm * MT * 32 + mt * 32 + lpix;
            qs[mt] = pf_pos_of_index(a.gi, valid[mt] ? i : min(mtile * BM + BM, Rtot) - 1);
        } else {
            qs[mt] = xoff[mt] + slab0 + (P + 1);
        }
    }
    if constexpr (PLANES == 3) {
        if (a.in2) {
            const int NC2 = a.in2_c / 32;
            const size_t ps2 = (size_t)a.in2_c * 4, sb2 = (size_t)slab0 * ps2;
            const size_t bytes2 = (size_t)pf_alloc_pixels(a.gi.N, a.gi.H, a.gi.W) * ps2;
            const __amdgpu_buffer_rsrc_t xrs2 = __builtin_amdgcn_make_buffer_rsrc(
                (void*)((const char*)a.in2 + sb2), 0, (int)min(bytes2 - sb2, (size_t)0x7fffffff), 0x00020000);
            int xvoff2;
            {
                const int i = wave * 64 + lane, Pl = i >> 3, sl = (i & 7) ^ ((Pl >> 1) & 7);
                xvoff2 = (D8 ? (Pl >> 3) * 9 + (Pl & 7) : Pl) * (int)ps2 + sl * 16;
            }
            const char* wsrc2 = (const char*)a.wpk2 + (size_t)(nb * NTILES) * NC2 * 4096 + (size_t)(tid & 255) * 16;
#pragma unroll
            for (int nt = 0; nt < NT; ++nt) {
                f32x16 b2[1];
                acc_init_bias<1>(b2, a.bias2, nb * NTILES + wn * NT + nt, lane);
#pragma unroll
                for (int mt = 0; mt < MT; ++mt)
#pragma unroll
                    for (int r = 0; r < 16; ++r) acc[nt][mt][r] += b2[0][r];
            }
            for (int c = 0; c < NC2; ++c) {
                __syncthreads();
                for (int i0 = wave * 64, r = 0; i0 < npieces; i0 += NTHREADS, ++r)
                    dma16_buf(xrs2, xl + (size_t)i0 * 16, xvoff2, c * 128 + r * RPIX * (int)ps2);
#pragma unroll
                for (int p0 = 0; p0 < NTILES * 256; p0 += NTHREADS) {
                    const int pw = p0 + wave * 64;
                    dma16(wsrc2 + (size_t)((pw >> 8) * NC2 + c) * 4096, wl + pw * 16);
                }
                asm volatile("s_waitcnt vmcnt(0)" ::: "memory");
                __syncthreads();
                bf16x8 wf2[NT][4];
#pragma unroll
                for (int nt = 0; nt < NT; ++nt) wread(wf2[nt], wl, nt);
#pragma unroll
                for (int mt = 0; mt < MT; ++mt) {
                    bf16x8 x2[4];
                    xload(x2, xoff[mt] + (D8 ? 8 : P) + 1);
#pragma unroll
                    for (int nt = 0; nt < NT; ++nt) mfma_step<PLANES>(acc[nt][mt], wf2[nt], x2);
                }
            }
        }
        if (a.resid) __syncthreads();
        conv_tail_mx<NT, MT, RESID_NBUF>(a, acc, qs, valid, nb * NTILES + wn * NT, lane, smem + wave * (RESID_NBUF * 4096), slab0);
    } else {
        char* scratch = nullptr;
        if (PLANES == 2 && a.resid && !(a.flags & CONV_RESID_DIRECT)) {
            __syncthreads();
            scratch = xl + wave * 8192;
        }
#pragma unroll
        for (int nt = 0; nt < NT; ++nt) conv_epilogue_q<MT, PLANES>(a, acc[nt], qs, valid, nb * NTILES + wn * NT + nt, lane, scratch);
    }
#ifdef WSI_STUDY
    asm volatile("s_waitcnt vmcnt(0)" ::: "memory");
    if (lane == 0 && (blockIdx.x & 63) == 0) {
        const unsigned long long st_end = __builtin_readcyclecounter();
        atomicAdd(&g_wide_stamps[0], 1ull);
        atomicAdd(&g_wide_stamps[1], st_end - st_begin);
        atomicAdd(&g_wide_stamps[2], st_setup - st_begin);
        atomicAdd(&g_wide_stamps[3], st_pro);
        atomicAdd(&g_wide_stamps[4], st_line);
        atomicAdd(&g_wide_stamps[5], st_tap);
        atomicAdd(&g_wide_stamps[6], st_end - st_loop_end);
    }
#endif
}


template <int PLANES, int MINW, int ABL = 0, int WM = 2, int WN = 2, int NT = 2, bool D8 = false>
static int launch_wide(const ConvArgs& a, hipStream_t st) {
    constexpr int BM = WM * 128, NTHREADS = WM * WN * 64, BN = WN * NT * 32;
    if (a.go.C % BN) return WSI_EINVAL;
    if constexpr (!D8 && ABL == 0 && WM == 2 && WN == 2 && NT == 2) {
        if (g_routes.wide_d8 && a.gi.W == 8 && a.gi.H == 8) return launch_wide<PLANES, MINW, 0, 2, 2, 2, true>(a, st);
    }
    const int nblocks = a.go.C / BN;
    const long long R = (long long)a.gi.N * a.gi.H * a.gi.W;
    const int mtiles = (int)((R + BM - 1) / BM);
    size_t xbytes = D8 ? (size_t)(304 + 16) * 128
                       : (size_t)((dense_max_slab_pixels(a, BM) * 8 + NTHREADS - 1) / NTHREADS * NTHREADS) * 16;
    if (xbytes < (size_t)WM * WN * 8192) xbytes = (size_t)WM * WN * 8192;
    size_t lds = 2 * (BN / 32) * 4096 + xbytes;
    if (PLANES == 3 && lds < (size_t)WM * WN * 4 * 4096) lds = (size_t)WM * WN * 4 * 4096;
    if (lds > 160 * 1024) return WSI_EINVAL;
    auto k = conv3x3s1_wide_kernel<PLANES, MINW, ABL, WM, WN, NT, D8>;
    if (lds > 64 * 1024 && hipFuncSetAttribute((const void*)k, hipFuncAttributeMaxDynamicSharedMemorySize, (int)lds) != hipSuccess)
        return WSI_EINVAL;
    const int grid = (a.flags & CONV_XCD_RANGES) ? (mtiles * nblocks + 7) / 8 * 8 : mtiles * nblocks;
    hipLaunchKernelGGL(k, dim3(grid), dim3(NTHREADS), lds, st, a);
    return hipGetLastError() == hipSuccess ? WSI_OK : WSI_EFAULT;
}


template <int MT, int WM, int WN, int PLANES, int MINW, bool FUSE, int PMAX = 34, int ABL = 0>
__global__ __launch_bounds__(WM* WN * 64, MINW) void conv3x3s2_slab_kernel(ConvArgs a) {
    extern __shared__ __attribute__((aligned(16))) char smem[];
    constexpr int BM = WM * MT * 32;
    constexpr int NTHREADS = WM * WN * 64;
    constexpr int KMAX = ((4 * BM + 2 * PMAX + 2) * 8 + NTHREADS - 1) / NTHREADS;
    constexpr int NT = FUSE ? 10 : 9;
    constexpr int RING = FUSE ? 2 : 3;
    const int tid = threadIdx.x, lane = tid & 63;
    const int wave = __builtin_amdgcn_readfirstlane(tid >> 6);
    const int wm = wave / WN, wn = wave % WN;
    const int l31 = lane & 31, h = lane >> 5;
    const int nblocks = a.go.C / (WN * 32);
    int nb = blockIdx.x % nblocks, mtile = blockIdx.x / nblocks;
    if (a.flags & CONV_XCD_ORDER) {
        const int per = 8 * nblocks, r = blockIdx.x % per;
        nb = r >> 3;
        mtile = (blockIdx.x / per) * 8 + (r & 7);
        if (mtile >= (a.go.NS + BM - 1) / BM) return;
    }
    const int P = a.go.P;
    const int q0 = a.go.G + mtile * BM;
    const int R01 = BM, R10 = 2 * BM + 1, R11 = 3 * BM + 1 + P;
    const int npix = 4 * BM + 2 * P + 2;
    const int npieces = npix * 8;
    const int ntile = nb * WN + wn;
    const int NC = a.gi.C / PFmt<PLANES>::CPL;
    const size_t in_pixstride = (size_t)a.gi.C * PFmt<PLANES>::BPC;
    const __amdgpu_buffer_rsrc_t wrs = __builtin_amdgcn_make_buffer_rsrc(
        (void*)((const char*)a.wpk + (size_t)ntile * NC * 9 * 4096), 0, NC * 9 * 4096, 0x00020000);
    const __amdgpu_buffer_rsrc_t wrd = __builtin_amdgcn_make_buffer_rsrc(
        (void*)((const char*)(FUSE ? a.wpk2 : a.wpk) + (size_t)ntile * NC * 4096), 0, NC * 4096, 0x00020000);
    const int wvoff = lane * 16;

    int srcpix[KMAX];
#pragma unroll
    for (int k = 0; k < KMAX; ++k) {
        const int i = wave * 64 + k * NTHREADS + lane;
        const int Pl = i >> 3;
        int reg = 0, j = Pl;
        if (Pl >= R11) { reg = 3; j = Pl - R11; }
        else if (Pl >= R10) { reg = 2; j = Pl - R10; }
        else if (Pl >= R01) { reg = 1; j = Pl - R01; }
        const int py = reg >> 1, px = reg & 1;
        const int v = q0 - (py ? P : 0) - px + j;
        int src = 0;
        int r = v - a.go.G;
        if (Pl < npix && r >= 0 && r < a.go.NS) {
            const int n = r / a.go.S;
            r -= n * a.go.S;
            const int y = r / P, x = r - y * P;
            if (x != a.go.W && y != a.go.H) src = a.gi.G + n * a.gi.S + (2 * y + py) * a.gi.P + 2 * x + px;
        }
        const int sl = (i & 7) ^ ((Pl >> 1) & 7);
        srcpix[k] = (int)((unsigned)src * (unsigned)in_pixstride + (unsigned)sl * 16u);
    }
    const __amdgpu_buffer_rsrc_t irs = __builtin_amdgcn_make_buffer_rsrc((void*)a.in, 0, 0xffffffff, 0x00020000);

    f32x16 acc[MT], accd[FUSE ? MT : 1];
    if constexpr (PLANES == 3) {
        acc_init_bias<MT>(acc, a.bias, ntile, lane);
        if constexpr (FUSE) acc_init_bias<MT>(accd, a.bias2, ntile, lane);
    } else {
#pragma unroll
        for (int mt = 0; mt < MT; ++mt)
#pragma unroll
            for (int r = 0; r < 16; ++r) acc[mt][r] = 0.f;
        if constexpr (FUSE) {
#pragma unroll
            for (int mt = 0; mt < MT; ++mt)
#pragma unroll
                for (int r = 0; r < 16; ++r) accd[mt][r] = 0.f;
        }
    }
    int xoff[MT];
#pragma unroll
    for (int mt = 0; mt < MT; ++mt) xoff[mt] = wm * MT * 32 + mt * 32 + l31;

    auto wload = [&](bf16x8(&w)[4], int c, int t) {
#pragma unroll
        for (int f = 0; f < 4; ++f) {
            const u32x4 v = (t < 9) ? __builtin_amdgcn_raw_buffer_load_b128(wrs, wvoff + f * 1024, (c * 9 + t) * 4096, 0)
                                    : __builtin_amdgcn_raw_buffer_load_b128(wrd, wvoff + f * 1024, c * 4096, 0);
            w[f] = __builtin_bit_cast(bf16x8, v);
        }
    };
    auto xload = [&](bf16x8(&x)[4], int Pl) {
        const int base = lds_xbase(Pl, h);
#pragma unroll
        for (int f = 0; f < 4; ++f) x[f] = *(const bf16x8*)(smem + (base ^ (f << 5)));
    };
    auto tap_off = [&](int t, int Pc) {
        if (t == 9) return 0;
        const int kh = t / 3, kw = t % 3;
        const int py = kh != 1, px = kw != 1;
        const int base = py ? (px ? 3 * BM + 1 + Pc : 2 * BM + 1) : (px ? BM : 0);
        const int back = (py ? Pc : 0) + px;
        return base + back + (kh == 0 ? -Pc : 0) + (kw == 0 ? -1 : 0);
    };

    bf16x8 wbuf[RING][4], xf[2][4];
    wload(wbuf[0], 0, 0);
    for (int c = 0; c < NC; ++c) {
        int Pc = P;
        asm volatile("" : "+s"(Pc));
        if (c) __syncthreads();
#pragma unroll
        for (int k = 0; k < KMAX; ++k) {
            const int i0 = wave * 64 + k * NTHREADS;
            if (i0 < npieces)
                dma16_buf(irs, smem + (size_t)i0 * 16, srcpix[k], c * 128);
        }
        asm volatile("s_waitcnt vmcnt(0)" ::: "memory");
        __syncthreads();
        xload(xf[0], xoff[0] + tap_off(0, Pc));
#pragma unroll
        for (int t = 0; t < NT; ++t) {
            asm volatile("" ::: "memory");
            if constexpr (!(ABL & 16)) {
                if (t + 1 < NT) wload(wbuf[(t + 1) % RING], c, t + 1);
                else if (c + 1 < NC) wload(wbuf[0], c + 1, 0);
            }
            asm volatile("" ::: "memory");
            const int toff = tap_off(t, Pc);
            const int toff_next = t + 1 < NT ? tap_off(t + 1, Pc) : 0;
#pragma unroll
            for (int mt = 0; mt < MT; ++mt) {
                const int k = t * MT + mt;
                if (mt + 1 < MT) xload(xf[(k + 1) & 1], xoff[mt + 1] + toff);
                else if (t + 1 < NT) xload(xf[(k + 1) & 1], xoff[0] + toff_next);
                const bf16x8(&w)[4] = wbuf[t % RING];
                const bf16x8(&x)[4] = xf[k & 1];
                f32x16& d = (FUSE && t == 9) ? accd[FUSE ? mt : 0] : acc[mt];
                if constexpr (PLANES == 3) {
                    d = mfma_mx6(d, w, x);
                } else if constexpr (PLANES == 2) {
                    mfma_step<2>(d, w, x);
                } else {
#pragma unroll
                    for (int f = 0; f < 4; ++f) d = mfma_bf16(w[f], x[f], d);
                }
            }
        }
    }
    conv_epilogue_any<MT, PLANES>(a, acc, q0 + wm * MT * 32, ntile, lane);
// ... 198 lines not shown
        if constexpr (DS) {
            ConvArgs a2 = a;
            a2.out = a.out2; a2.bias = a.bias2; a2.resid = nullptr; a2.relu = 0;
            a2.wpk = a.wpk2; a2.ksize = 1;
            if constexpr (PLANES == 3) conv_epilogue_mx<MT>(a2, accd[nt], qs, valid, ntile, lane);
            else conv_epilogue_q<MT, PLANES>(a2, accd[nt], qs, valid, ntile, lane);
        }
    }
}

template <int PLANES>
static int launch_s2wide(const ConvArgs& a, hipStream_t st) {
    constexpr int BM = 256, XB = 45056;
    const bool ds = a.out2 != nullptr;
    if (a.go.C % 128 || a.go.P > 34 || !a.in_split_pixels || (ds && (!a.wpk2 || !a.bias2)) || a.out_split_pixels) return WSI_EINVAL;
    const long long R = (long long)a.go.N * a.go.H * a.go.W;
    const bool nt4 = !ds && PLANES == 3 && g_routes.s2_nt4 && a.go.C % 256 == 0;
    const int nblocks = a.go.C / (nt4 ? 256 : 128);
    ConvArgs g = a;
    g.gi = a.go;
    const long long span = dense_max_slab_pixels(g, BM) - (a.go.P + 1);
    const bool dense = (span * 8 + 255) / 256 * 256 * 16 <= XB;
    const int mtiles = dense ? (int)((R + BM - 1) / BM) : (a.go.NS + BM - 1) / BM;
    const size_t lds = 4 * 16384 + 2 * XB;
    auto k = nt4 ? (dense ? conv3x3s2_wide_kernel<PLANES, true, false, 4> : conv3x3s2_wide_kernel<PLANES, false, false, 4>)
           : dense ? (ds ? conv3x3s2_wide_kernel<PLANES, true, true> : conv3x3s2_wide_kernel<PLANES, true, false>)
                   : (ds ? conv3x3s2_wide_kernel<PLANES, false, true> : conv3x3s2_wide_kernel<PLANES, false, false>);
    if (hipFuncSetAttribute((const void*)k, hipFuncAttributeMaxDynamicSharedMemorySize, (int)lds) != hipSuccess) return WSI_EINVAL;
    ConvArgs b = a;
    b.mtiles = mtiles;
    hipLaunchKernelGGL(k, dim3((mtiles * nblocks + 7) / 8 * 8), dim3(512), lds, st, b);
    return hipGetLastError() == hipSuccess ? WSI_OK : WSI_EFAULT;
}

int wsi_s2_dispatch(const ConvArgs& a_in, int planes, hipStream_t st) {
    ConvArgs a = a_in;
    if (a.in_split_pixels)
        return planes == 3 ? launch_s2wide<3>(a, st) : planes == 2 ? launch_s2wide<2>(a, st) : WSI_EINVAL;
    if (g_routes.xcd_order && a.go.C > 128) a.flags |= CONV_XCD_ORDER;
    if (a.gi.C % 64 || a.go.C % 128 || planes < 1 || planes > 3) return WSI_EINVAL;
    if (a.go.H * 2 != a.gi.H || a.go.W * 2 != a.gi.W || a.gi.N != a.go.N) return WSI_EINVAL;
    const bool fuse = a.out2 != nullptr;
    if (fuse && (!a.wpk2 || !a.bias2)) return WSI_EINVAL;
    if (a.go.P > 34) {
        if (planes == 3) return fuse ? launch_s2slab<2, 1, 4, 3, 2, true, 130>(a, st) : launch_s2slab<2, 1, 4, 3, 2, false, 130>(a, st);
        if (planes == 2) return fuse ? launch_s2slab<2, 1, 4, 2, 2, true, 130>(a, st) : launch_s2slab<2, 1, 4, 2, 2, false, 130>(a, st);
        return WSI_EINVAL;
    }
#ifdef WSI_STUDY
    if (g_routes.s2_ablate && planes == 3 && fuse) return launch_s2slab<2, 1, 4, 3, 3, true, 34, 16>(a, st);
#endif
    if (g_routes.s2_small_tiles) {
        if (planes == 3) return fuse ? launch_s2slab<2, 1, 4, 3, 3, true>(a, st) : launch_s2slab<2, 1, 4, 3, 3, false>(a, st);
        if (planes == 2) return fuse ? launch_s2slab<2, 1, 4, 2, 3, true>(a, st) : launch_s2slab<2, 1, 4, 2, 3, false>(a, st);
    }
    if (planes == 3) return fuse ? launch_s2slab<4, 1, 4, 3, 2, true>(a, st) : launch_s2slab<4, 1, 4, 3, 2, false>(a, st);
    if (planes == 2) return fuse ? launch_s2slab<4, 1, 4, 2, 2, true>(a, st) : launch_s2slab<4, 1, 4, 2, 2, false>(a, st);
    return fuse ? launch_s2slab<4, 1, 4, 1, 2, true>(a, st) : launch_s2slab<4, 1, 4, 1, 2, false>(a, st);
}

template <int MT, int WM, int WN, int PLANES>
static int launch_gather(const ConvArgs& a, hipStream_t st) {
    constexpr int BM = WM * MT * 32;
    if (a.go.C % (WN * 32)) return WSI_EINVAL;
    const int mtiles = (a.go.NS + BM - 1) / BM;
    const int nblocks = a.go.C / (WN * 32);
    const size_t lds = (size_t)BM * 128;
    hipLaunchKernelGGL((conv_gather_kernel<MT, WM, WN, PLANES>), dim3(mtiles * nblocks), dim3(WM * WN * 64), lds, st, a);
    return hipGetLastError() == hipSuccess ? WSI_OK : WSI_EFAULT;
}

#define SLAB3_CFGS(X) \
    X(20, 4, 1, 4, 2, false) \
    X(21, 4, 2, 2, 2, false) \
    X(25, 2, 2, 4, 3, false) \
    X(27, 4, 4, 2, 1, false) \
    X(28, 2, 2, 2, 3, true) \
    X(29, 2, 2, 2, 4, true) \
    X(39, 4, 4, 2, 1, true) \
    X(26, 4, 1, 2, 3, false) \
    X(30, 4, 1, 4, 2, true) \
    X(31, 4, 2, 2, 2, true) \
    X(32, 2, 2, 4, 3, true) \
    X(33, 8, 1, 4, 2, true) \
    X(34, 8, 1, 2, 2, true) \
    X(35, 8, 2, 2, 2, true) \
    X(36, 4, 2, 4, 2, true) \
    X(37, 4, 1, 4, 3, true) \
    X(38, 4, 2, 2, 3, true)



int wsi_slab_dispatch_cfg(const ConvArgs& a_in, int planes, int cfg, hipStream_t st) {
    ConvArgs a = a_in;
    if (g_routes.xcd_order && cfg >= 20 && cfg < 40 && !CONV_STUDY(a, ~7)) a.flags |= CONV_XCD_ORDER;
    if (g_routes.xcd_ranges && !CONV_STUDY(a, ~7) && ((cfg >= 20 && cfg < 42) || cfg == 60 || cfg == 90 || cfg == 91 || (cfg >= 70 && cfg < 90)) && (g_routes.xcd_ranges == 2 || a.go.C == 64)) a.flags |= CONV_XCD_RANGES;
    if ((a.flags & CONV_IN96) && !((cfg >= 20 && cfg <= 42) || cfg == 90 || cfg == 91)) return WSI_EINVAL;
    if (a.in_up && !((cfg >= 20 && cfg < 40) || cfg == 90 || cfg == 91)) return WSI_EINVAL;
    if (cfg < 20) return WSI_EINVAL;
    if (cfg >= 70 && cfg < 90) return wsi_pp_dispatch(a, planes, cfg, st);
    if (cfg == 90) return planes == 3 ? launch_slab3<2, 8, 1, 3, 1, true>(a, st) : planes == 2 ? launch_slab3<2, 8, 1, 2, 1, true>(a, st) : WSI_EINVAL;
    if (cfg == 91) return planes == 3 ? launch_slab3<2, 4, 1, 3, 2, true>(a, st) : planes == 2 ? launch_slab3<2, 4, 1, 2, 2, true>(a, st) : WSI_EINVAL;
    if (cfg == 42) return planes == 3 ? launch_l1p(a, st) : WSI_EINVAL;
    if (cfg == 40) return planes == 3 ? launch_rows<3>(a, st) : WSI_EINVAL;
    if (cfg == 41) return planes == 3 ? launch_rows<2>(a, st) : WSI_EINVAL;
    if (cfg == 60) return planes == 3 ? launch_wide<3, 2>(a, st) : planes == 2 ? launch_wide<2, 2>(a, st) : launch_wide<1, 2>(a, st);
#ifdef WSI_STUDY
    if (cfg == 61 && planes == 3) return launch_wide<3, 2, 32>(a, st);
    if (cfg == 67) return planes == 3 ? launch_wide<3, 1, 0, 4, 2, 1>(a, st) : planes == 2 ? launch_wide<2, 1, 0, 4, 2, 1>(a, st) : WSI_EINVAL;
    if (cfg == 68) return planes == 3 ? launch_wide<3, 2, 0, 2, 2, 1>(a, st) : planes == 2 ? launch_wide<2, 2, 0, 2, 2, 1>(a, st) : WSI_EINVAL;
    if (cfg >= 50 && cfg <= 53 && planes == 3) {
        switch (cfg) {
        case 50: return launch_slab3<4, 1, 4, 3, 2, true, 16>(a, st);
        case 51: return launch_slab3<4, 1, 4, 3, 2, true, 32>(a, st);
        case 52: return launch_slab3<4, 1, 4, 3, 2, true, 48>(a, st);
        case 53: return launch_slab3<4, 1, 4, 3, 2, true, 8>(a, st);
        }
    }
    switch (cfg) {
#define X(id, MT, WM, WN, MINW, DENSE) \
    case id: return planes == 3 ? launch_slab3<MT, WM, WN, 3, MINW, DENSE>(a, st) \
                  : planes == 2 ? launch_slab3<MT, WM, WN, 2, MINW, DENSE>(a, st) : launch_slab3<MT, WM, WN, 1, MINW, DENSE>(a, st);
        SLAB3_CFGS(X)
#undef X
    }
#else
    if (cfg == 30) return planes == 3 ? launch_slab3<4, 1, 4, 3, 2, true>(a, st) : planes == 2 ? launch_slab3<4, 1, 4, 2, 2, true>(a, st) : launch_slab3<4, 1, 4, 1, 2, true>(a, st);
    if (cfg == 31) return planes == 3 ? launch_slab3<4, 2, 2, 3, 2, true>(a, st) : planes == 2 ? launch_slab3<4, 2, 2, 2, 2, true>(a, st) : launch_slab3<4, 2, 2, 1, 2, true>(a, st);
    if (cfg == 38) {
        if (planes != 3) return WSI_EINVAL;
        const int rc = g_routes.slab_pair ? launch_slab3<4, 2, 2, 3, 3, true, 0, true>(a, st) : WSI_EINVAL;
        return rc != WSI_EINVAL ? rc : launch_slab3<4, 2, 2, 3, 3, true>(a, st);
    }
    if (cfg == 39) return planes == 3 ? launch_slab3<4, 4, 2, 3, 1, true>(a, st) : planes == 2 ? launch_slab3<4, 4, 2, 2, 1, true>(a, st) : launch_slab3<4, 4, 2, 1, 1, true>(a, st);
#endif
    return WSI_EINVAL;
}

static int slab_default_cfg(const ConvArgs& a, int planes, bool fallback) {
    if (a.go.C % 64) return fallback ? 91 : 90;
    if (a.in_up) return a.go.C % 128 == 0 ? 30 : (a.gi.W > 128 && !fallback ? 39 : 31);
    if (a.gi.W <= 4 && a.go.C % 128 == 0 && planes == 3) return 30;
    if (a.go.C % 128 == 0 && a.go.C >= g_routes.wide_min_c && !(planes == 1 && a.gi.W > 33)) return 60;
    if (a.go.C % 128 != 0 && a.gi.W > 128 && !fallback) return 39;
    if (a.go.C == 64 && a.gi.C == 64 && planes == 3 && !fallback && g_routes.l1_rows && g_routes.l1p && a.gi.W == 64 && a.gi.H % 4 == 0 && !a.in2 && (a.flags & CONV_IN96) &&
        (!a.resid || (a.flags & CONV_RESID96)))
        return 42;
    if (a.go.C % 128 != 0 && planes == 3 && !fallback && g_routes.l1_rows && a.gi.W == 64 && a.gi.H % 4 == 0 && !a.in2) return 40;
    if (a.go.C % 128 != 0 && planes == 3 && !fallback && a.gi.W != 64) return 31;
    if (a.go.C % 128 != 0 && planes == 3 && !fallback) return 38;
    return a.go.C % 128 == 0 ? 30 : 31;
}

int wsi_conv_dispatch(const ConvArgs& a, int planes, int cfg, hipStream_t st) {
    const int cout = a.go.C;
    if (planes < 1 || planes > 3) return WSI_EINVAL;
    const int cmul = planes == 1 ? 64 : 32;
    if (a.gi.C % cmul || cout % cmul) return WSI_EINVAL;
    if ((a.gi.C % 64 || cout % 64) && !(a.ksize == 3 && a.stride == 1)) return WSI_EINVAL;
    if (planes == 3 && !(a.ksize == 3 && a.stride == 1)) return WSI_EINVAL;
    if (a.ksize == 3 && a.stride == 1) {
        if (a.gi.H != a.go.H || a.gi.W != a.go.W || a.gi.N != a.go.N) return WSI_EINVAL;
        if (cfg >= 0) return wsi_slab_dispatch_cfg(a, planes, cfg, st);
        const int rc = wsi_slab_dispatch_cfg(a, planes, slab_default_cfg(a, planes, false), st);
        return rc != WSI_EINVAL ? rc : wsi_slab_dispatch_cfg(a, planes, slab_default_cfg(a, planes, true), st);
    }
    if ((a.ksize == 3 || a.ksize == 1) && (a.stride == 1 || a.stride == 2)) {
        if (a.go.H * a.stride != a.gi.H || a.go.W * a.stride != a.gi.W || a.gi.N != a.go.N) return WSI_EINVAL;
        if (cout % 128 == 0) return planes == 2 ? launch_gather<8, 1, 4, 2>(a, st) : launch_gather<8, 1, 4, 1>(a, st);
        return planes == 2 ? launch_gather<4, 2, 2, 2>(a, st) : launch_gather<4, 2, 2, 1>(a, st);
    }
    return WSI_EINVAL;
}
```

### wsi_segmentation_pipeline_amd/csrc/conv_dev.h

```cpp
#pragma once
#include "common.h"

static __device__ __forceinline__ void dma16(const void* gsrc, char* lds_wave_base) {
    __builtin_amdgcn_global_load_lds((const __attribute__((address_space(1))) void*)gsrc,
                                     (__attribute__((address_space(3))) void*)lds_wave_base, 16, 0, 0);
}

static __device__ __forceinline__ void dma16_buf(__amdgpu_buffer_rsrc_t rs, char* lds_wave_base, int voff, int soff) {
    __builtin_amdgcn_raw_ptr_buffer_load_lds(rs, (__attribute__((address_space(3))) void*)lds_wave_base, 16, voff, soff, 0, 0);
}

static __device__ __forceinline__ unsigned lds_addr_of(const char* p) {
    return (unsigned)(size_t)(const __attribute__((address_space(3))) char*)p;
}
static __device__ __forceinline__ void dma16_asm(const void* gsrc, unsigned lds) {
    unsigned keep;
    asm volatile("s_mov_b32 %0, m0\n\ts_mov_b32 m0, %1\n\ts_nop 0\n\tglobal_load_lds_dwordx4 %2, off\n\ts_mov_b32 m0, %0"
                 : "=&s"(keep) : "s"(lds), "v"(gsrc) : "memory");
}
static __device__ __forceinline__ void dma16_buf_asm(__amdgpu_buffer_rsrc_t rs, unsigned lds, int voff, int soff) {
    unsigned keep;
    asm volatile("s_mov_b32 %0, m0\n\ts_mov_b32 m0, %1\n\ts_nop 0\n\tbuffer_load_dwordx4 %2, %3, %4 offen lds\n\ts_mov_b32 m0, %0"
                 : "=&s"(keep) : "s"(lds), "v"(voff), "s"(rs), "s"(soff) : "memory");
}
// ... 89 lines not shown
            }
    }
    float bias[16], wsi[16];
#pragma unroll
    for (int g = 0; g < 4; ++g)
#pragma unroll
        for (int i = 0; i < 4; ++i) bias[g * 4 + i] = a.bias[ntile * 32 + 8 * g + 4 * h + i];
    if constexpr (PLANES == 2) {
        const float* ws = conv_wscale_inv(a.wpk, a.go.C, a.gi.C, a.ksize) + ntile * 32 + 4 * h;
#pragma unroll
        for (int g = 0; g < 4; ++g) {
            const f32x4 v = *(const f32x4*)(ws + 8 * g);
#pragma unroll
            for (int i = 0; i < 4; ++i) wsi[g * 4 + i] = v[i];
        }
    }
#pragma unroll
    for (int mt = 0; mt < MT; ++mt) {
        if (via_lds) {
            asm volatile("s_waitcnt vmcnt(0)" ::: "memory");
            if (mt + 1 < MT)
                resid_tile_dma(a.resid, valid[mt + 1] ? qs[mt + 1] : a.go.G, pixstride, (size_t)ntile * 128, lane, scratch + ((mt + 1) & 1) * 4096);
            const char* t = scratch + (mt & 1) * 4096 + l31 * 128 + 8 * h;
            const int sw = (l31 >> 1) & 7;
#pragma unroll
            for (int g = 0; g < 4; ++g) {
                rh[mt][g] = *(const Ex4*)(t + ((g ^ sw) << 4));
                rl[mt][g] = *(const Ex4*)(t + (((4 + g) ^ sw) << 4));
            }
        }
#pragma unroll
        for (int g = 0; g < 4; ++g) {
            float v[4];
#pragma unroll
            for (int i = 0; i < 4; ++i) {
                if constexpr (PLANES == 2) v[i] = acc[mt][4 * g + i] * wsi[4 * g + i] + bias[4 * g + i];
                else v[i] = acc[mt][4 * g + i] + bias[4 * g + i];
            }
            if (a.resid) {
#pragma unroll
                for (int i = 0; i < 4; ++i) v[i] += (float)rh[mt][g][i];
                if constexpr (PLANES == 2) {
#pragma unroll
                    for (int i = 0; i < 4; ++i) v[i] += (float)rl[mt][g][i];
                }
            }
            Ex4 hi, lo;
            if constexpr (PLANES == 2) {
                const float lo_clamp = a.relu ? 0.f : -65504.f;
#pragma unroll
                for (int i = 0; i < 4; ++i) {
                    v[i] = __builtin_amdgcn_fmed3f(v[i], lo_clamp, 65504.f);
                    hi[i] = (E)v[i];
                    lo[i] = (E)(v[i] - (float)hi[i]);
                }
            } else {
                if (a.relu) {
#pragma unroll
                    for (int i = 0; i < 4; ++i) v[i] = fmaxf(v[i], 0.f);
                }
#pragma unroll
                for (int i = 0; i < 4; ++i) {
                    hi[i] = (E)v[i];
                    lo[i] = (E)(v[i] - (float)hi[i]);
                }
            }
            if (valid[mt] && !CONV_STUDY(a, CONV_ABL_NO_STORE)) {
                char* op = (char*)a.out + ooff[mt] + 16 * g;
                if (CONV_STUDY(a, CONV_NONTEMPORAL)) {
                    __builtin_nontemporal_store(hi, (Ex4*)op);
                    if constexpr (PLANES == 2) __builtin_nontemporal_store(lo, (Ex4*)(op + 64));
                } else {
                    *(Ex4*)op = hi;
                    if constexpr (PLANES == 2) *(Ex4*)(op + 64) = lo;
                }
            }
        }
    }
}

static __device__ __forceinline__ f32x16 mfma_mx6(f32x16 d, const bf16x8 (&w)[4], const bf16x8 (&x)[4]) {
    d = __builtin_amdgcn_mfma_f32_32x32x16_f16(__builtin_bit_cast(f16x8, w[0]), __builtin_bit_cast(f16x8, x[0]), d, 0, 0, 0);
    d = __builtin_amdgcn_mfma_f32_32x32x16_f16(__builtin_bit_cast(f16x8, w[1]), __builtin_bit_cast(f16x8, x[1]), d, 0, 0, 0);
    const i32x4 wq = __builtin_bit_cast(i32x4, w[2]), wr = __builtin_bit_cast(i32x4, w[3]);
    const i32x4 xq = __builtin_bit_cast(i32x4, x[2]), xr = __builtin_bit_cast(i32x4, x[3]);
    const i32x8 wa = {wq[0], wq[1], wq[2], wq[3], wr[0], wr[1], wr[2], wr[3]}, xa = {xq[0], xq[1], xq[2], xq[3], xr[0], xr[1], xr[2], xr[3]};
    return __builtin_amdgcn_mfma_scale_f32_32x32x64_f8f6f4(wa, xa, d, 2, 2, 0, wr[2], 0, xr[2]);
}

template <int MT>
static __device__ __forceinline__ void acc_init_bias(f32x16 (&acc)[MT], const float* bias, int ntile, int lane) {
    const int h = lane >> 5;
    float b[16];
#pragma unroll
    for (int g = 0; g < 4; ++g) {
        const f32x4 v = *(const f32x4*)(bias + ntile * 32 + 8 * g + 4 * h);
#pragma unroll
        for (int i = 0; i < 4; ++i) b[4 * g + i] = v[i];
    }
#pragma unroll
    for (int mt = 0; mt < MT; ++mt)
#pragma unroll
        for (int r = 0; r < 16; ++r) acc[mt][r] = b[r];
}

template <int MT, int MTN = MT>
static __device__ __forceinline__ void conv_epilogue_mx(const ConvArgs& a, f32x16 (&acc)[MT], const int (&qs)[MT],
                                                        const bool (&valid)[MT], int ntile, int lane, int mt0 = 0) {
    const int h = lane >> 5;
    const bool o96 = a.flags & CONV_OUT96;
    const size_t pixstride = o96 ? (size_t)96 : (size_t)a.go.C * 4;
    const float lo_clamp = a.relu ? 0.f : -65504.f;
#pragma unroll
    for (int mt = mt0; mt < mt0 + MTN; ++mt) {
        const size_t loff = (size_t)(valid[mt] ? qs[mt] : a.go.G) * pixstride + (o96 ? (size_t)ntile * (size_t)a.plane96 : (size_t)ntile * 128);
        f32x16 v = acc[mt];
        f32x16 hi, lo;
        f16x8 hv[2];
        float mv = 0.f, ml = 0.f;
#pragma unroll
        for (int r = 0; r < 16; r += 2) {
            const float v0 = __builtin_amdgcn_fmed3f(v[r], lo_clamp, 65504.f);
            const float v1 = __builtin_amdgcn_fmed3f(v[r + 1], lo_clamp, 65504.f);
            const f16x2 hh = __builtin_convertvector(f32x2{v0, v1}, f16x2);
            hv[r >> 3][r & 7] = hh[0];
            hv[r >> 3][(r & 7) + 1] = hh[1];
            hi[r] = (float)hh[0];
            hi[r + 1] = (float)hh[1];
            lo[r] = v0 - hi[r];
            lo[r + 1] = v1 - hi[r + 1];
            mv = fmaxf(mv, fmaxf(fabsf(hi[r]), fabsf(hi[r + 1])));
            ml = fmaxf(ml, fmaxf(fabsf(lo[r]), fabsf(lo[r + 1])));
        }
        pair_max2(mv, ml);
        const int sh = mx6_scale_byte(mv), sl = mx6_scale_byte(ml);
        const int sb = h ? sh : sl;
        swap32_halves(lo, hi);
        const u32x6 q = mx6_pack32(lo, hi, sb ? mx_scale_value(sb) : 1.f);
        if (valid[mt] && !CONV_STUDY(a, CONV_ABL_NO_STORE)) {
            char* ol = (char*)a.out + (a.out_split_pixels ? pf_out_offset(a.go, a.out_split_pixels, qs[mt], pixstride) + (size_t)ntile * 128 : loff);
            *(f16x8*)(ol + 32 * h) = hv[0];
            *(f16x8*)(ol + 32 * h + 16) = hv[1];
            if (!o96) {
                *(u32x4*)(ol + MX6_PLANE_LO(0) + 16 * h) = u32x4{q[0], q[1], q[2], q[3]};
                *(u32x4*)(ol + MX6_PLANE_HI(0) + 16 * h) = u32x4{q[4], q[5], (unsigned)sb, 0u};
            } else if (h == 0) {
                *(u32x4*)(ol + 64) = u32x4{q[0], q[1], q[2], q[3]};
                *(u32x4*)(ol + 80) = u32x4{q[4], q[5], (unsigned)sl, (unsigned)sh};
            }
        }
    }
}

template <int NT, int MT, int NBUF>
static __device__ __forceinline__ void conv_tail_mx(const ConvArgs& a, f32x16 (&acc)[NT][MT], const int (&qs)[MT], const bool (&valid)[MT],
                                                    int ntile0, int lane, char* scratch, int slab0) {
    constexpr int T = NT * MT;
    static_assert(MT % NBUF == 0 || NBUF % MT == 0, "a batch is part of one channel tile or whole channel tiles");
    static_assert(NBUF <= T && T % NBUF == 0, "whole batches");
    if (!a.resid) {
#pragma unroll
        for (int nt = 0; nt < NT; ++nt) conv_epilogue_mx<MT>(a, acc[nt], qs, valid, ntile0 + nt, lane);
        return;
    }
    const int h = lane >> 5, l31 = lane & 31;
    const bool r96 = a.flags & CONV_RESID96;
    const int pixstride = r96 ? 96 : a.go.C * 4;
    const size_t rbase = (size_t)slab0 * pixstride, rbytes = (size_t)pf_alloc_pixels(a.go.N, a.go.H, a.go.W) * pixstride;
    const __amdgpu_buffer_rsrc_t rrs = __builtin_amdgcn_make_buffer_rsrc((void*)((const char*)a.resid + rbase), 0,
                                                                          (int)min(rbytes - rbase, (size_t)0x7fffffff), 0x00020000);
    bf16x8 iw[4];
    {
        const int p = mx_line_pos(l31), f0 = mx6_field_of_pos(p);
        f16x8 k0, k1;
#pragma unroll
        for (int j = 0; j < 8; ++j) {
            k0[j] = (p == 8 * h + j) ? (_Float16)1.0f : (_Float16)0.0f;
            k1[j] = (p == 16 + 8 * h + j) ? (_Float16)1.0f : (_Float16)0.0f;
        }
        unsigned q[6];
#pragma unroll
        for (int d = 0; d < 6; ++d) {
            const int bit = 6 * f0 + 3 - 32 * d;
            q[d] = (h == 0 && bit >= 0 && bit < 32) ? (1u << (bit & 31)) : 0u;
        }
        iw[0] = __builtin_bit_cast(bf16x8, k0);
        iw[1] = __builtin_bit_cast(bf16x8, k1);
        iw[2] = __builtin_bit_cast(bf16x8, u32x4{q[0], q[1], q[2], q[3]});
        iw[3] = __builtin_bit_cast(bf16x8, u32x4{q[4], q[5], 127u, 0u});
    }
    auto rdma = [&](int k) {
        const int nt = k / MT, mt = k % MT;
        int qr = qs[mt] - slab0;
        asm volatile("" : "+v"(qr));
        if (r96) {
            const __amdgpu_buffer_rsrc_t prs = __builtin_amdgcn_make_buffer_rsrc(
                (void*)((const char*)a.resid + (size_t)(ntile0 + nt) * (size_t)a.plane96 + rbase), 0, (int)min(rbytes - rbase, (size_t)0x7fffffff), 0x00020000);
            resid_tile_dma_buf96(prs, qr, pixstride, 0, lane, scratch + (k % NBUF) * 4096);
        }
        else resid_tile_dma_buf(rrs, qr, pixstride, (ntile0 + nt) * 128, lane, scratch + (k % NBUF) * 4096);
    };
    const int xb = l31 * 128 + ((h ^ ((l31 >> 1) & 7)) << 4);
#pragma unroll
    for (int k = 0; k < NBUF; ++k) rdma(k);
#pragma unroll
    for (int b0 = 0; b0 < T; b0 += NBUF) {
        asm volatile("s_waitcnt vmcnt(0)" ::: "memory");
#pragma unroll
        for (int k = b0; k < b0 + NBUF; ++k) {
            const char* t = scratch + (k % NBUF) * 4096;
            bf16x8 x[4];
#pragma unroll
            for (int f = 0; f < 4; ++f) x[f] = *(const bf16x8*)(t + (xb ^ (f << 5)));
            if (r96 && h) {
                x[2] = __builtin_bit_cast(bf16x8, u32x4{0u, 0u, 0u, 0u});
                x[3] = x[2];
            }
            acc[k / MT][k % MT] = mfma_mx6(acc[k / MT][k % MT], iw, x);
        }
        if (b0 + NBUF < T) {
            asm volatile("s_waitcnt lgkmcnt(0)" ::: "memory");
#pragma unroll
            for (int k = b0 + NBUF; k < b0 + 2 * NBUF; ++k) rdma(k);
        }
        if constexpr (NBUF >= MT) {
#pragma unroll
            for (int nt = b0 / MT; nt < (b0 + NBUF) / MT; ++nt) conv_epilogue_mx<MT>(a, acc[nt], qs, valid, ntile0 + nt, lane);
        } else {
            conv_epilogue_mx<MT, NBUF>(a, acc[b0 / MT], qs, valid, ntile0 + b0 / MT, lane, b0 % MT);
        }
    }
}

template <int MT, int PLANES>
static __device__ __forceinline__ void conv_epilogue(const ConvArgs& a, f32x16 (&acc)[MT], int q_base, int ntile,
                                                     int lane) {
    int qs[MT];
    bool valid[MT];
#pragma unroll
    for (int mt = 0; mt < MT; ++mt) {
        qs[mt] = q_base + mt * 32 + (lane & 31);
        valid[mt] = pf_is_pixel(a.go, qs[mt]);
    }
    conv_epilogue_q<MT, PLANES>(a, acc, qs, valid, ntile, lane);
}

template <int MT, int PLANES>
static __device__ __forceinline__ void conv_epilogue_any(const ConvArgs& a, f32x16 (&acc)[MT], int q_base, int ntile, int lane) {
    if constexpr (PLANES == 3) {
        int qs[MT];
        bool valid[MT];
#pragma unroll
        for (int mt = 0; mt < MT; ++mt) {
            qs[mt] = q_base + mt * 32 + (lane & 31);
            valid[mt] = pf_is_pixel(a.go, qs[mt]);
        }
        conv_epilogue_mx<MT>(a, acc, qs, valid, ntile, lane);
    } else {
        conv_epilogue<MT, PLANES>(a, acc, q_base, ntile, lane);
    }
}

template <int MT, int PLANES>
static __device__ __forceinline__ void mfma_line(f32x16 (&acc)[MT], const bf16x8 (&wf)[4], const char* smem,
                                                 const int (&xbase)[MT]) {
    bf16x8 xf[2][4];
#pragma unroll
    for (int f = 0; f < 4; ++f) xf[0][f] = *(const bf16x8*)(smem + (xbase[0] ^ (f << 5)));
#pragma unroll
    for (int mt = 0; mt < MT; ++mt) {
        const bf16x8(&x)[4] = xf[mt & 1];
        if (mt + 1 < MT) {
#pragma unroll
            for (int f = 0; f < 4; ++f) xf[(mt + 1) & 1][f] = *(const bf16x8*)(smem + (xbase[mt + 1] ^ (f << 5)));
        }
        if constexpr (PLANES == 2) {
            acc[mt] = mfma16<2>(wf[2], x[0], acc[mt]);
            acc[mt] = mfma16<2>(wf[3], x[1], acc[mt]);
            acc[mt] = mfma16<2>(wf[0], x[2], acc[mt]);
            acc[mt] = mfma16<2>(wf[1], x[3], acc[mt]);
            acc[mt] = mfma16<2>(wf[0], x[0], acc[mt]);
            acc[mt] = mfma16<2>(wf[1], x[1], acc[mt]);
        } else {
#pragma unroll
            for (int f = 0; f < 4; ++f) acc[mt] = mfma_bf16(wf[f], x[f], acc[mt]);
        }
    }
}

static __device__ __forceinline__ int dense_lane_pixel(int l31) {
    return l31 < 4 ? l31 : l31 < 12 ? l31 + 12 : l31 < 16 ? l31 - 8 : l31 < 20 ? l31 + 8 : l31 < 28 ? l31 - 12 : l31;
}

static __device__ __forceinline__ int lds_xbase(int Pl, int h) { return Pl * 128 + ((h ^ ((Pl >> 1) & 7)) << 4); }
template <int PLANES>
static __device__ __forceinline__ void mfma_step(f32x16& d, const bf16x8 (&w)[4], const bf16x8 (&x)[4]) {
    if constexpr (PLANES == 3) {
        d = mfma_mx6(d, w, x);
    } else if constexpr (PLANES == 2) {
        d = mfma16<2>(w[2], x[0], d);
        d = mfma16<2>(w[3], x[1], d);
        d = mfma16<2>(w[0], x[2], d);
        d = mfma16<2>(w[1], x[3], d);
        d = mfma16<2>(w[0], x[0], d);
        d = mfma16<2>(w[1], x[1], d);
    } else {
#pragma unroll
        for (int f = 0; f < 4; ++f) d = mfma_bf16(w[f], x[f], d);
    }
}
```

### wsi_segmentation_pipeline_amd/csrc/heads.hip

```cpp
#include "pf_lines.h"
#include "internal.h"

static __device__ __forceinline__ float wave_sum(float v) {
#pragma unroll
    for (int o = 32; o > 0; o >>= 1) v += __shfl_xor(v, o);
    return v;
}

template <int PLANES>
__global__ __launch_bounds__(256) void avgpool_fc_kernel(const void* in, PFGeom g, const float* w, const float* b, int K,
                                                         float* feat, float* logits) {
    extern __shared__ __attribute__((aligned(16))) char smem[];
    float* f = (float*)smem;
    const int n = blockIdx.x, tid = threadIdx.x;
    const size_t pixstride = (size_t)g.C * PFmt<PLANES>::BPC;
    const float inv = 1.0f / (float)(g.H * g.W);
    if constexpr (PLANES == 3) {
        const int NL = g.C / 32, HW = g.H * g.W;
        float* part = f + g.C;
        const int slice = tid & 3, line = (tid >> 2) % NL, pg = tid / (4 * NL), npg = 256 / (4 * NL);
        float sm[8] = {0.f, 0.f, 0.f, 0.f, 0.f, 0.f, 0.f, 0.f};
        if (pg < npg) {
            for (int p = pg; p < HW; p += npg) {
                const int y = p / g.W, x = p - y * g.W;
                const char* L = (const char*)in + (size_t)(g.G + n * g.S + y * g.P + x) * pixstride + (size_t)line * 128;
                const f16x8 hi = *(const f16x8*)(L + 16 * slice);
                const u32x4 p0 = *(const u32x4*)(L + MX6_PLANE_LO(0)), p1 = *(const u32x4*)(L + MX6_PLANE_HI(0));
                const unsigned sl = p1[2] & 255u;
                const f32x32 dd = mx6_unpack32(u32x6{p0[0], p0[1], p0[2], p0[3], p1[0], p1[1]}, sl ? mx_scale_value((int)sl) : 0.f);
                float d[8];
#pragma unroll
                for (int i = 0; i < 8; ++i) {
                    const float e0 = (slice >> 1) ? dd[2 * i + 1] : dd[2 * i], e1 = (slice >> 1) ? dd[16 + 2 * i + 1] : dd[16 + 2 * i];
                    d[i] = (slice & 1) ? e1 : e0;
                }
#pragma unroll
                for (int i = 0; i < 8; ++i) sm[i] += (float)hi[i] + d[i];
            }
#pragma unroll
            for (int i = 0; i < 8; ++i) part[pg * g.C + line * 32 + mx_line_chan(8 * slice + i)] = sm[i];
        }
        __syncthreads();
        for (int c = tid; c < g.C; c += 256) {
            float t = 0.f;
            for (int k = 0; k < npg; ++k) t += part[k * g.C + c];
            f[c] = t * inv;
            if (feat) feat[(size_t)n * g.C + c] = t * inv;
        }
    } else
    for (int c4 = tid; c4 < g.C / 4; c4 += 256) {
        const int c = c4 * 4;
        const size_t coff = PLANES == 2 ? (size_t)(c >> 5) * 128 + (c & 31) * 2 : (size_t)c * 2;
        float s[4] = {0.f, 0.f, 0.f, 0.f};
        for (int y = 0; y < g.H; ++y)
            for (int x = 0; x < g.W; ++x) {
                const char* p = (const char*)in + (size_t)(g.G + n * g.S + y * g.P + x) * pixstride + coff;
                typedef __attribute__((ext_vector_type(4))) typename PairElem<PLANES>::T Ex4;
                const Ex4 hi = *(const Ex4*)p;
#pragma unroll
                for (int k = 0; k < 4; ++k) s[k] += (float)hi[k];
                if constexpr (PLANES == 2) {
                    const Ex4 lo = *(const Ex4*)(p + 64);
#pragma unroll
                    for (int k = 0; k < 4; ++k) s[k] += (float)lo[k];
                }
            }
#pragma unroll
        for (int k = 0; k < 4; ++k) {
            f[c + k] = s[k] * inv;
            if (feat) feat[(size_t)n * g.C + c + k] = s[k] * inv;
        }
    }
    __syncthreads();
    if (!logits) return;
    const int lane = tid & 63, wave = tid >> 6;
    for (int k = wave; k < K; k += 4) {
        float acc = 0.f;
        for (int c = lane; c < g.C; c += 64) acc += f[c] * w[(size_t)k * g.C + c];
        acc = wave_sum(acc);
        if (lane == 0) logits[(size_t)n * K + k] = acc + b[k];
    }
}

template <int BT>
__global__ __launch_bounds__(256) void linear_kernel(const float* x, const float* w, const float* bias, float* y, int B,
                                                     int K, int J, int relu) {
    const int lane = threadIdx.x & 63;
    const int j = blockIdx.x * 4 + (threadIdx.x >> 6);
    if (j >= J) return;
    const f32x4* wr = (const f32x4*)(w + (size_t)j * K);
    for (int b0 = 0; b0 < B; b0 += BT) {
        float acc[BT];
#pragma unroll
        for (int t = 0; t < BT; ++t) acc[t] = 0.f;
        for (int k4 = lane; k4 < K / 4; k4 += 64) {
            const f32x4 wv = wr[k4];
#pragma unroll
            for (int t = 0; t < BT; ++t) {
                if (b0 + t < B) {
                    const f32x4 xv = ((const f32x4*)(x + (size_t)(b0 + t) * K))[k4];
                    acc[t] += wv[0] * xv[0] + wv[1] * xv[1] + wv[2] * xv[2] + wv[3] * xv[3];
                }
            }
        }
#pragma unroll
        for (int t = 0; t < BT; ++t) {
            const float s = wave_sum(acc[t]);
            if (lane == 0 && b0 + t < B) {
                float v = s + (bias ? bias[j] : 0.f);
                if (relu) v = fmaxf(v, 0.f);
                y[(size_t)(b0 + t) * J + j] = v;
            }
        }
    }
}

template <int JMAX>
__global__ __launch_bounds__(256) void linear_rows_kernel(const float* x, const float* w, const float* bias, float* y, int B, int K,
                                                          int J, int relu) {
    const int lane = threadIdx.x & 63;
    const int b = blockIdx.x * 4 + (threadIdx.x >> 6);
    if (b >= B) return;
    const f32x4* xr = (const f32x4*)(x + (size_t)b * K);
    float acc[JMAX];
#pragma unroll
    for (int j = 0; j < JMAX; ++j) acc[j] = 0.f;
    for (int k4 = lane; k4 < K / 4; k4 += 64) {
        const f32x4 xv = xr[k4];
#pragma unroll
        for (int j = 0; j < JMAX; ++j) {
            if (j < J) {
                const f32x4 wv = ((const f32x4*)(w + (size_t)j * K))[k4];
                acc[j] += wv[0] * xv[0] + wv[1] * xv[1] + wv[2] * xv[2] + wv[3] * xv[3];
            }
        }
    }
#pragma unroll
    for (int j = 0; j < JMAX; ++j) {
        if (j < J) {
            const float s = wave_sum(acc[j]);
            if (lane == 0) {
                float v = s + (bias ? bias[j] : 0.f);
                if (relu) v = fmaxf(v, 0.f);
                y[(size_t)b * J + j] = v;
            }
        }
    }
}

__global__ __launch_bounds__(256) void linear_mfma_f32_kernel(const float* x, const float* w, const float* bias, float* y, int B,
                                                              int K, int J, int relu) {
    constexpr int BM = 64, BN = 128, KB = 32;
    __shared__ float Xs[KB][BM];
    __shared__ float Ws[KB][BN];
    const int tid = threadIdx.x, lane = tid & 63, wave = tid >> 6;
    const int l31 = lane & 31, h = lane >> 5;
    const int n0 = blockIdx.x * BN, m0 = blockIdx.y * BM;
    const int xr = tid >> 2, xk = (tid & 3) * 8;
    const int wr = tid >> 1, wk = (tid & 1) * 16;
    const float* xp = x + (size_t)min(m0 + xr, B - 1) * K + xk;
    const float* wp = w + (size_t)(n0 + wr) * K + wk;
    f32x4 xv[2], wv[4];
    auto fetch = [&](int k0) {
#pragma unroll
        for (int q = 0; q < 2; ++q) xv[q] = *(const f32x4*)(xp + k0 + 4 * q);
#pragma unroll
        for (int q = 0; q < 4; ++q) wv[q] = *(const f32x4*)(wp + k0 + 4 * q);
    };
    auto commit = [&]() {
#pragma unroll
        for (int q = 0; q < 2; ++q)
#pragma unroll
            for (int e = 0; e < 4; ++e) Xs[xk + 4 * q + e][xr] = xv[q][e];
#pragma unroll
        for (int q = 0; q < 4; ++q)
#pragma unroll
            for (int e = 0; e < 4; ++e) Ws[wk + 4 * q + e][wr] = wv[q][e];
    };
    f32x16 acc[2];
#pragma unroll
    for (int mt = 0; mt < 2; ++mt)
#pragma unroll
        for (int r = 0; r < 16; ++r) acc[mt][r] = 0.f;
    fetch(0);
    for (int k0 = 0; k0 < K; k0 += KB) {
        __syncthreads();
        commit();
        __syncthreads();
        if (k0 + KB < K) fetch(k0 + KB);
#pragma unroll
        for (int kk = 0; kk < KB / 2; ++kk) {
            const float b = Ws[2 * kk + h][wave * 32 + l31];
#pragma unroll
            for (int mt = 0; mt < 2; ++mt)
                acc[mt] = __builtin_amdgcn_mfma_f32_32x32x2f32(Xs[2 * kk + h][mt * 32 + l31], b, acc[mt], 0, 0, 0);
        }
    }
    const int j = n0 + wave * 32 + l31;
    const float bj = bias ? bias[j] : 0.f;
#pragma unroll
    for (int mt = 0; mt < 2; ++mt)
#pragma unroll
        for (int r = 0; r < 16; ++r) {
            const int row = m0 + mt * 32 + (r & 3) + 8 * (r >> 2) + 4 * h;
            if (row < B) {
                float v = acc[mt][r] + bj;
                if (relu) v = fmaxf(v, 0.f);
                y[(size_t)row * J + j] = v;
            }
        }
}

template <int PLANES>
__global__ __launch_bounds__(256) void pf_pack_kernel(const float* in, void* out, PFGeom g) {
    const long long total = (long long)g.N * g.H * g.W * g.C;
    for (long long i = blockIdx.x * 256LL + threadIdx.x; i < total; i += (long long)gridDim.x * 256) {
        const int c = (int)(i % g.C);
        long long p = i / g.C;
        const int x = (int)(p % g.W); p /= g.W;
        const int y = (int)(p % g.H);
        const int n = (int)(p / g.H);
        const float v = in[(((size_t)n * g.C + c) * g.H + y) * g.W + x];
        char* o = (char*)out + (size_t)(g.G + n * g.S + y * g.P + x) * ((size_t)g.C * PLANES * 2);
        if constexpr (PLANES == 2) {
            _Float16 hi, lo;
            split_f16(v, hi, lo);
            *(_Float16*)(o + (c >> 5) * 128 + (c & 31) * 2) = hi;
            *(_Float16*)(o + (c >> 5) * 128 + 64 + (c & 31) * 2) = lo;
        } else {
            *(__bf16*)(o + c * 2) = (__bf16)v;
        }
    }
}

template <int PLANES>
__global__ __launch_bounds__(256) void pf_unpack_kernel(const void* in, float* out, PFGeom g) {
    const long long total = (long long)g.N * g.H * g.W * g.C;
    for (long long i = blockIdx.x * 256LL + threadIdx.x; i < total; i += (long long)gridDim.x * 256) {
        const int c = (int)(i % g.C);
        long long p = i / g.C;
        const int x = (int)(p % g.W); p /= g.W;
        const int y = (int)(p % g.H);
        const int n = (int)(p / g.H);
        const char* o = (const char*)in + (size_t)(g.G + n * g.S + y * g.P + x) * ((size_t)g.C * PLANES * 2);
        float v;
        if constexpr (PLANES == 2)
            v = (float)*(const _Float16*)(o + (c >> 5) * 128 + (c & 31) * 2) +
                (float)*(const _Float16*)(o + (c >> 5) * 128 + 64 + (c & 31) * 2);
        else
            v = (float)*(const __bf16*)(o + c * 2);
        out[(((size_t)n * g.C + c) * g.H + y) * g.W + x] = v;
    }
}

__global__ __launch_bounds__(256) void pf_pack_mx_kernel(const float* in, void* out, PFGeom g) {
    const long long total = (long long)g.N * g.H * g.W * (g.C / 32);
    for (long long i = blockIdx.x * 256LL + threadIdx.x; i < total; i += (long long)gridDim.x * 256) {
        const int l = (int)(i % (g.C / 32));
        long long p = i / (g.C / 32);
        const int x = (int)(p % g.W); p /= g.W;
        const int y = (int)(p % g.H);
        const int n = (int)(p / g.H);
        float v[32];
        for (int c = 0; c < 32; ++c) v[c] = in[(((size_t)n * g.C + 32 * l + c) * g.H + y) * g.W + x];
        mx_line_encode(v, (char*)out + (size_t)(g.G + n * g.S + y * g.P + x) * ((size_t)g.C * 4) + (size_t)l * 128);
    }
}

__global__ __launch_bounds__(256) void pf_unpack_mx_kernel(const void* in, float* out, PFGeom g) {
    const long long total = (long long)g.N * g.H * g.W * g.C;
    for (long long i = blockIdx.x * 256LL + threadIdx.x; i < total; i += (long long)gridDim.x * 256) {
        const int c = (int)(i % g.C);
        long long p = i / g.C;
        const int x = (int)(p % g.W); p /= g.W;
        const int y = (int)(p % g.H);
        const int n = (int)(p / g.H);
        const char* line = (const char*)in + (size_t)(g.G + n * g.S + y * g.P + x) * ((size_t)g.C * 4) + (size_t)(c >> 5) * 128;
        out[(((size_t)n * g.C + c) * g.H + y) * g.W + x] = mx_line_decode(line, c & 31);
    }
}

static int grid_for(long long total) {
    long long g = (total + 255) / 256;
    return (int)(g > 16384 ? 16384 : (g < 1 ? 1 : g));
}

int wsi_avgpool_fc_dispatch(const void* in, const PFGeom& g, const float* w, const float* b, int K, float* feat,
                            float* logits, int planes, hipStream_t st) {
    if (g.N <= 0 || g.H <= 0 || g.W <= 0 || g.C <= 0 || planes < 1 || planes > 3 || g.C % (planes == 1 ? PFmt<1>::CPL : PFmt<2>::CPL)) return WSI_EINVAL;
    size_t lds = (size_t)g.C * 4;
    if (planes == 3) {
        if (g.C > 2048) return WSI_EINVAL;
        lds += (size_t)(256 / (4 * (g.C / 32))) * g.C * 4;
    }
    if (planes == 3)
        hipLaunchKernelGGL(avgpool_fc_kernel<3>, dim3(g.N), dim3(256), lds, st, in, g, w, b, K, feat, logits);
    else if (planes == 2)
        hipLaunchKernelGGL(avgpool_fc_kernel<2>, dim3(g.N), dim3(256), lds, st, in, g, w, b, K, feat, logits);
    else
        hipLaunchKernelGGL(avgpool_fc_kernel<1>, dim3(g.N), dim3(256), lds, st, in, g, w, b, K, feat, logits);
    return hipGetLastError() == hipSuccess ? WSI_OK : WSI_EFAULT;
}

int wsi_linear_dispatch(const float* x, const float* w, const float* bias, float* y, int B, int K, int J, int relu,
                        hipStream_t st) {
    if (K % 4 || B <= 0 || J <= 0) return WSI_EINVAL;
    if (J % 128 == 0 && K % 32 == 0 && B >= 8 && (long long)J * K >= (1 << 20)) {
        hipLaunchKernelGGL(linear_mfma_f32_kernel, dim3(J / 128, (B + 63) / 64), dim3(256), 0, st, x, w, bias, y, B, K, J, relu);
        return hipGetLastError() == hipSuccess ? WSI_OK : WSI_EFAULT;
    }
    if (J <= 16 && B >= 32) {
        if (J <= 4) hipLaunchKernelGGL(linear_rows_kernel<4>, dim3((B + 3) / 4), dim3(256), 0, st, x, w, bias, y, B, K, J, relu);
        else hipLaunchKernelGGL(linear_rows_kernel<16>, dim3((B + 3) / 4), dim3(256), 0, st, x, w, bias, y, B, K, J, relu);
        return hipGetLastError() == hipSuccess ? WSI_OK : WSI_EFAULT;
    }
    hipLaunchKernelGGL(linear_kernel<8>, dim3((J + 3) / 4), dim3(256), 0, st, x, w, bias, y, B, K, J, relu);
    return hipGetLastError() == hipSuccess ? WSI_OK : WSI_EFAULT;
}

int wsi_pf_pack_dispatch(const float* in, void* out, const PFGeom& g, int planes, hipStream_t st) {
    const long long total = (long long)g.N * g.H * g.W * g.C;
    if (planes == 3)
        hipLaunchKernelGGL(pf_pack_mx_kernel, dim3(grid_for(total / 32)), dim3(256), 0, st, in, out, g);
    else if (planes == 2)
        hipLaunchKernelGGL(pf_pack_kernel<2>, dim3(grid_for(total)), dim3(256), 0, st, in, out, g);
    else
        hipLaunchKernelGGL(pf_pack_kernel<1>, dim3(grid_for(total)), dim3(256), 0, st, in, out, g);
    return hipGetLastError() == hipSuccess ? WSI_OK : WSI_EFAULT;
}

int wsi_pf_unpack_dispatch(const void* in, float* out, const PFGeom& g, int planes, hipStream_t st) {
    const long long total = (long long)g.N * g.H * g.W * g.C;
    if (planes == 3)
        hipLaunchKernelGGL(pf_unpack_mx_kernel, dim3(grid_for(total)), dim3(256), 0, st, in, out, g);
    else if (planes == 2)
        hipLaunchKernelGGL(pf_unpack_kernel<2>, dim3(grid_for(total)), dim3(256), 0, st, in, out, g);
    else
        hipLaunchKernelGGL(pf_unpack_kernel<1>, dim3(grid_for(total)), dim3(256), 0, st, in, out, g);
    return hipGetLastError() == hipSuccess ? WSI_OK : WSI_EFAULT;
}
```

### wsi_segmentation_pipeline_amd/csrc/internal.h

```cpp
#pragma once
#include "common.h"

int wsi_conv_dispatch(const ConvArgs& a, int planes, int cfg, hipStream_t st);
int wsi_s2_dispatch(const ConvArgs& a, int planes, hipStream_t st);
int wsi_pp_dispatch(const ConvArgs& a, int planes, int cfg, hipStream_t st);
long long dense_max_slab_pixels(const ConvArgs& a, int BM);
int wsi_stem_dispatch(const StemArgs& a, int planes, hipStream_t st);
int wsi_maxpool_dispatch(const float* in, void* out, int N, int Hc, int Wc, int planes, hipStream_t st);
int wsi_stem_pool_dispatch(const StemArgs& a, void* out_pf, int planes, int rows_per_seg, hipStream_t st, int out96 = 0, long long plane96 = 0, void* x0_pf = nullptr);
int wsi_avgpool_fc_dispatch(const void* in, const PFGeom& g, const float* w, const float* b, int K, float* feat,
                            float* logits, int planes, hipStream_t st);
int wsi_linear_dispatch(const float* x, const float* w, const float* bias, float* y, int B, int K, int J, int relu,
                        hipStream_t st);
int wsi_pf_pack_dispatch(const float* in, void* out, const PFGeom& g, int planes, hipStream_t st);
int wsi_pf_unpack_dispatch(const void* in, float* out, const PFGeom& g, int planes, hipStream_t st);
int wsi_upsample_concat_dispatch(const void* x, const void* skip, void* out, int n, int h, int w, int cx, int cs, int planes, hipStream_t st);
int wsi_nhwc_to_pf_dispatch(const float* in, void* out, int n, int h, int w, int c, int planes, hipStream_t st);
int wsi_unet_head_dispatch(const void* in, int n, int h, int w, int c_pf, const float* wt, const float* b, int cin, int k, float* out,
                           int planes, hipStream_t st);
int wsi_resize_nearest_dispatch(const float* src, long long planes_n, int hs, int ws, float* dst, int hd, int wd, hipStream_t st);
int wsi_unet_tail_dispatch(const void* x4, const void* blob, int n, int h, int w, int classes, float* logits, hipStream_t st);
int wsi_tile_gather_dispatch(const uint8_t* slide, long long pitch, int SH, int SW, const int* origins, const float* lut,
                             float* out, int N, int ph, int pw, hipStream_t st);
int wsi_stitch_add_dispatch(const float* logits, const int* txy, int T, int C, int dy, int dx, double* pred, int MH, int MW,
                            hipStream_t st);
int wsi_stitch_add_dense_dispatch(const float* tiles, const int* txy, int T, int C, int ph, int pw, double* pred, int MH,
                                  int MW, hipStream_t st);
int wsi_softmax_dispatch(const double* pred, int C, long long HW, const double* thresh, double* probs, uint8_t* classes,
                         const uint8_t* mask, int heat_mode, uint8_t* heat, hipStream_t st);
int wsi_paint_dispatch(const long long* idx, const int* region_of, long long n, const uint8_t* cls, int* winner, long long* label,
                       long long npix, hipStream_t st);
int wsi_exponent_span_dispatch(const float* v, long long n, int* out2, hipStream_t st);
int wsi_hsv_mask_dispatch(const uint8_t* rgb, long long npix, int stride, double thresh, uint8_t* mask, hipStream_t st);
int wsi_lab_mask_dispatch(const uint8_t* rgb, long long npix, int stride, double mu_percent, uint8_t* mask, void* scratch, hipStream_t st);
size_t wsi_cc_scratch_bytes(int H, int W);
int wsi_cc_dispatch(const uint8_t* mask, int H, int W, int* labels_out, int* count_out, void* scratch, hipStream_t st, int conn4 = 0);
int wsi_fill_holes_dispatch(const uint8_t* mask, int H, int W, uint8_t* out, void* scratch, hipStream_t st);
int wsi_kmeans_dispatch(const int* pts, int n, double* centres, int k, int iters, int* labels, void* scratch, hipStream_t st);
int wsi_kmeans_seed_farthest_dispatch(const int* pts, int n, int k, double* centres, void* scratch, hipStream_t st);
int wsi_slic_dispatch(const uint8_t* rgb, int H, int W, const double* fw, int radius, double* segs, int K, int step_y, int step_x,
                      double step, double compactness, int iters, int* labels, void* scratch, hipStream_t st);
int wsi_tile_grid_dispatch(int iw, int ih, int ph, int pw, int sh, int sw, const uint8_t* mask, int MH, int MW, double m, double thresh,
                           int* out_xy, int* count_out, void* scratch, hipStream_t st);
int wsi_resize_dispatch(const double* src, int C, int Hs, int Ws, double* dst, int Hd, int Wd, hipStream_t st);
int wsi_argmax_dispatch(const double* pred, int C, long long HW, uint8_t* classes, hipStream_t st);
int wsi_threshold_dispatch(const uint8_t* src, long long n, int lo, uint8_t* dst, hipStream_t st);
int wsi_morph_dispatch(const uint8_t* src, uint8_t* dst, uint8_t* tmp, int H, int W, int k, int op, hipStream_t st);
int wsi_bwperim_dispatch(const uint8_t* src, uint8_t* dst, int H, int W, hipStream_t st);
size_t wsi_hull_ws_bytes(int H);
int wsi_hull_dispatch(const uint8_t* src, uint8_t* dst, int H, int W, void* ws, hipStream_t st);
int wsi_hull_polygon_dispatch(void* ws, int H, double* out_xy, int cap, hipStream_t st);
int wsi_iou_counts_dispatch(const uint8_t* a, const uint8_t* b, long long n, unsigned long long* out, hipStream_t st);
int wsi_score_counts_dispatch(const uint8_t* p, const uint8_t* gt, const uint8_t* mask, long long n, unsigned long long* out, hipStream_t st);
int wsi_esp_dispatch(const double* pts, int n, int num, double* out, double* scratch, hipStream_t st);

static inline size_t align_up(size_t x, size_t a) { return (x + a - 1) / a * a; }

struct TileSource {
    const float* in_f32;
    const uint8_t* slide;
    long long pitch; int SH, SW;
    const int* tile_xy;
    const float* lut;
    bool valid() const { return in_f32 || (slide && tile_xy && lut); }
    TileSource from_image(int n0, int h, int w) const {
        return {in_f32 ? in_f32 + (size_t)n0 * 3 * h * w : nullptr, slide, pitch, SH, SW, tile_xy ? tile_xy + 2 * n0 : nullptr, lut};
    }
};
StemArgs stem_args(const TileSource& src, const void* wpk, const float* bias, float* scratch, int n, int h, int w);
int stem_run(const TileSource& src, const void* stem_wpk, const float* stem_bias, const void* stem_wpk_u8, const float* stem_bias_u8,
             const float* norm_mean_std, int n, int h, int w, float* scratch, void* out_pf, int planes, void* stream, int out96,
             long long plane96 = 0, void* x0_pf = nullptr);

struct ConvCall {
    const void* in;
    void* out;
    const void* resid = nullptr;
    const void* wpk; const float* bias;
    int n, h, w, cin, cout, stride, ksize, relu, planes;
    void* stream;
    int cfg = -1;
    int split_out = 0; long long split_pixels = 0;
    const void* in2 = nullptr; int in2_c = 0; const void* wpk2 = nullptr; const float* bias2 = nullptr;
    int line_flags = 0;
    const void* in_up = nullptr; int up_c = 0;
    long long plane96 = 0;
};
int conv_common(const ConvCall& c);
int s2_split_common(const void* in_split, void* out_conv_pf, void* out_ds_pf, const void* wpk3, const float* bias3, const void* wpk1,
                    const float* bias1, int n, int h_in, int w_in, int cin, int cout, int planes, void* stream, long long split_pixels);
```

### wsi_segmentation_pipeline_amd/csrc/trunk.hip

```cpp
#include "internal.h"
#include "../../include/wsi_hip.h"
#include <mutex>
#include <unordered_map>

extern "C" {

#define WSI_PROF_MAX 16384
static struct {
    int enabled, count, cap;
    hipEvent_t ev[2 * WSI_PROF_MAX];
    int kind[WSI_PROF_MAX];
    double flops[WSI_PROF_MAX];
    int created;
} g_prof;

int wsi_prof_begin(int max_records) {
    if (max_records <= 0 || max_records > WSI_PROF_MAX) return WSI_EINVAL;
    for (; g_prof.created < 2 * max_records; ++g_prof.created)
        if (hipEventCreate(&g_prof.ev[g_prof.created]) != hipSuccess) return WSI_ENOMEM;
    g_prof.cap = max_records; g_prof.count = 0; g_prof.enabled = 1;
    return WSI_OK;
}

int wsi_prof_end(float* ms_out, int* kind_out, double* flops_out, int cap) {
    g_prof.enabled = 0;
    int n = g_prof.count < cap ? g_prof.count : cap;
    for (int i = 0; i < n; ++i) {
        if (hipEventSynchronize(g_prof.ev[2 * i + 1]) != hipSuccess) return WSI_EFAULT;
        float ms = 0.f;
        if (hipEventElapsedTime(&ms, g_prof.ev[2 * i], g_prof.ev[2 * i + 1]) != hipSuccess) return WSI_EFAULT;
        ms_out[i] = ms; kind_out[i] = g_prof.kind[i]; flops_out[i] = g_prof.flops[i];
    }
    g_prof.count = 0;
    return n;
}

struct ProfScope {
    const hipStream_t st;
    int i = -1;
    ProfScope(hipStream_t st, int kind, double flops) : st(st) {
        if (!g_prof.enabled || g_prof.count >= g_prof.cap) return;
        i = g_prof.count++;
        g_prof.kind[i] = kind; g_prof.flops[i] = flops;
        (void)hipEventRecord(g_prof.ev[2 * i], st);
    }
    ~ProfScope() { if (i >= 0) (void)hipEventRecord(g_prof.ev[2 * i + 1], st); }
    void relabel(int kind) { if (i >= 0) g_prof.kind[i] = kind; }
};
static inline double conv_flops(int n, int ho, int wo, int ci, int co, int taps) { return 2.0 * n * ho * wo * (double)co * ci * taps; }

static std::mutex g_ws_mutex;
struct WsTag { int layout; size_t bytes; };
static std::unordered_map<const void*, WsTag> g_ws_layout;
static int ws_layout_switch(const void* ws, int want, size_t need) {
    std::lock_guard<std::mutex> lk(g_ws_mutex);
    auto it = g_ws_layout.find(ws);
    const int have = it == g_ws_layout.end() ? -2 : it->second.layout;
    const size_t bytes = it == g_ws_layout.end() ? 0 : it->second.bytes;
    if (bytes && need > bytes) return -1;
    g_ws_layout[ws] = WsTag{want, bytes};
    if (have == want || have == -1) return 0;
    return (have >= 0 && have / 2 != want / 2) ? 2 : 1;
}
int wsi_trunk_workspace_release(void* workspace) {
    std::lock_guard<std::mutex> lk(g_ws_mutex);
    g_ws_layout.erase(workspace);
    return WSI_OK;
}

int wsi_trunk_set_chunks(int stem_chunk, int layer1_chunk) {
    if (stem_chunk < 0 || layer1_chunk < 0) return WSI_EINVAL;
    if (stem_chunk && layer1_chunk && layer1_chunk % stem_chunk) return WSI_EINVAL;
    g_routes.chunk_stem = stem_chunk; g_routes.chunk_l1 = layer1_chunk;
    return WSI_OK;
}
struct TrunkPlan {
    size_t stem_scratch;
    size_t buf[4][4];
    size_t total;
    int sh[4], sw[4], sc[4];
};

static int trunk_plan(int n, int h, int w, int planes, TrunkPlan& p) {
    if (n <= 0 || h <= 0 || w <= 0 || h % 32 || w % 32 || planes < 1 || planes > 3) return WSI_EINVAL;
    size_t off = 0;
    p.stem_scratch = off;
    off += align_up((size_t)n * (h / 2) * (w / 2) * 64 * sizeof(float), 256);
    for (int s = 0; s < 4; ++s) {
        p.sh[s] = h >> (2 + s); p.sw[s] = w >> (2 + s); p.sc[s] = 64 << s;
        for (int b = 0; b < 3; ++b) {
            p.buf[s][b] = off;
            off += align_up(wsi_pf_bytes(n, p.sh[s], p.sw[s], p.sc[s], planes), 256);
        }
        p.buf[s][3] = off;
        if (s < 3 && planes >= 2) off += align_up(wsi_pf_split_bytes(n, p.sh[s], p.sw[s], p.sc[s], planes), 256);
    }
    p.total = off;
    return WSI_OK;
}

size_t wsi_trunk_workspace_bytes(int n, int h, int w, int planes) {
    TrunkPlan p;
    return trunk_plan(n, h, w, planes, p) ? 0 : p.total;
}

int wsi_trunk_workspace_init(void* workspace, int n, int h, int w, int planes, void* stream) {
    TrunkPlan p;
    if (!workspace || trunk_plan(n, h, w, planes, p)) return WSI_EINVAL;
    {
        std::lock_guard<std::mutex> lk(g_ws_mutex);
        g_ws_layout[workspace] = WsTag{-1, p.total};
    }
    return hipMemsetAsync((char*)workspace + p.buf[0][0], 0, p.total - p.buf[0][0], (hipStream_t)stream) == hipSuccess
               ? WSI_OK
               : WSI_EFAULT;
}

struct TrunkResult { size_t last_off; int last_stage; size_t stage_off[4]; };
struct TrunkOpts {
    bool allow_split = true;
    char* x0_out = nullptr;
};
static int trunk_run(const wsi_trunk_weights* wt, const TileSource& src, int n, int cap, int h, int w, void* workspace,
                     int stop_after, hipStream_t st, const TrunkPlan& p, TrunkResult& res, const TrunkOpts& opt = {}) {
    char* ws = (char*)workspace;
    const int planes = wt->planes;
    int rc = WSI_OK;
    auto conv3 = [&](const void* in, void* out, const void* resid, int wi, int n0, int H, int W, int C) {
        return ConvCall{.in = in, .out = out, .resid = resid, .wpk = wt->conv_w[wi], .bias = wt->conv_b[wi], .n = n0, .h = H, .w = W, .cin = C,
                        .cout = C, .stride = 1, .ksize = 3, .relu = 1, .planes = planes, .stream = st};
    };
    auto run = [&](int kind, const ConvCall& c) {
        ProfScope ps(st, kind, conv_flops(c.n, c.h / c.stride, c.w / c.stride, c.cin, c.cout, c.ksize * c.ksize));
        return conv_common(c);
    };
    const size_t bpc = planes == 1 ? PFmt<1>::BPC : PFmt<2>::BPC;
    const int cs = g_routes.chunk_stem > 0 ? g_routes.chunk_stem : n, c1 = g_routes.chunk_l1 > 0 ? g_routes.chunk_l1 : n;
    const int H1 = p.sh[0], W1 = p.sw[0];
    const int do_l1 = stop_after != 0;
    auto can_split = [&](int s) { return opt.allow_split && g_routes.s2_split && g_routes.s2_slab && stop_after >= 8 && planes >= 2 && s < 3 && p.sw[s + 1] <= 33; };
    const bool split0 = can_split(0);
    const bool l96 = g_routes.l1_lines96 && planes == 3 && split0;
    if (const int dirty = ws_layout_switch(workspace, 2 * planes + (l96 ? 1 : 0), p.total)) {
        if (dirty < 0) return WSI_EINVAL;
        const size_t nbytes = dirty == 2 ? p.total - p.buf[0][0] : p.buf[0][3] - p.buf[0][0];
        if (hipMemsetAsync(ws + p.buf[0][0], 0, nbytes, st) != hipSuccess) return WSI_EFAULT;
    }
    auto img_off = [&](int s, int n0) { return (size_t)n0 * (p.sh[s] + 1) * (p.sw[s] + 1) * (s == 0 && l96 ? (size_t)96 : (size_t)p.sc[s] * bpc); };
    const long long plane96 = l96 ? (long long)pf_alloc_pixels(cap, p.sh[0], p.sw[0]) * 96 : 0;
    auto split_off = [&](int n0) { return (size_t)n0 * (p.sh[1] + 1) * (p.sw[1] + 1) * p.sc[0] * bpc; };

    int l1_out = 0;
    for (int n1 = 0; n1 < n; n1 += c1) {
        const int nn1 = n - n1 < c1 ? n - n1 : c1;
        for (int n0 = n1; n0 < n1 + nn1; n0 += cs) {
            const int nn = n1 + nn1 - n0 < cs ? n1 + nn1 - n0 : cs;
            ProfScope ps(st, 4, 2.0 * nn * (h / 2) * (w / 2) * 64.0 * 147.0);
            rc = stem_run(src.from_image(n0, h, w), wt->stem_w, wt->stem_b, wt->stem_w_u8, wt->stem_b_u8, wt->norm,
                          nn, h, w, (float*)(ws + p.stem_scratch), ws + p.buf[0][0] + img_off(0, n0),
                          planes, st, l96 ? 1 : 0, plane96,
                          opt.x0_out ? opt.x0_out + (size_t)n0 * (h / 2 + 1) * (w / 2 + 1) * 64 * bpc : nullptr);
            if (rc) return rc;
        }
        if (!do_l1) continue;
        int cur = 0;
        for (int b = 0; b < 2 && (stop_after >= 8 || b < stop_after); ++b) {
            const int m = (cur + 1) % 3, o = (cur + 2) % 3;
            char *x = ws + p.buf[0][cur] + img_off(0, n1), *mid = ws + p.buf[0][m] + img_off(0, n1),
                 *out = ws + p.buf[0][o] + img_off(0, n1);
            const int f_in = l96 ? CONV_IN96 : 0, f_res = l96 ? CONV_RESID96 : 0;
            ConvCall c = conv3(x, mid, nullptr, 2 * b, nn1, H1, W1, 64);
            c.line_flags = f_in | (l96 ? CONV_OUT96 : 0); c.plane96 = plane96;
            if ((rc = run(5, c))) return rc;
            c = conv3(mid, out, x, 2 * b + 1, nn1, H1, W1, 64);
            c.line_flags = f_in | f_res | (l96 && b == 0 ? CONV_OUT96 : 0); c.plane96 = plane96;
            if (b == 1 && split0) {
                c.out = ws + p.buf[0][3] + split_off(n1);
                c.split_out = 1; c.split_pixels = pf_alloc_pixels(cap, H1 / 2, W1 / 2);
            }
            if ((rc = run(5, c))) return rc;
            cur = o;
        }
        l1_out = cur;
    }
    res.last_off = res.stage_off[0] = p.buf[0][l1_out]; res.last_stage = 0;
    if (stop_after >= 0 && stop_after <= 2) return WSI_OK;

    int cur = l1_out;
    const void* x = split0 ? ws + p.buf[0][3] : ws + p.buf[0][cur];
    bool x_split = split0;
    int block = 2;
    for (int s = 1; s < 4; ++s) {
        const int H = p.sh[s], W = p.sw[s], C = p.sc[s];
        for (int b = 0; b < 2; ++b) {
            const int wi = s * 4 + b * 2;
            void *mid, *out;
            const void* resid;
            const bool fold = b == 0 && x_split && planes == 3 && g_routes.ds_fold && g_routes.s2_slab && C % 128 == 0;
            const void* fold_in2 = fold ? x : nullptr;
            if (b == 0) {
                mid = ws + p.buf[s][1];
                void* ds = fold ? nullptr : ws + p.buf[s][2];
                out = ws + p.buf[s][0];
                if (g_routes.s2_slab) {
                    ProfScope ps(st, 2, conv_flops(n, H, W, C / 2, C, fold ? 9 : 10));
                    rc = x_split ? s2_split_common(x, mid, ds, wt->conv_w[wi], wt->conv_b[wi], wt->down_w[s - 1],
                                                   wt->down_b[s - 1], n, 2 * H, 2 * W, C / 2, C, planes, st, pf_alloc_pixels(cap, H, W))
                                 : wsi_conv3x3s2_ds_fused(x, mid, ds, wt->conv_w[wi], wt->conv_b[wi], wt->down_w[s - 1], wt->down_b[s - 1], n,
                                                          2 * H, 2 * W, C / 2, C, planes, st);
                    if (rc) return rc;
                } else {
                    ConvCall c = conv3(x, mid, nullptr, wi, n, 2 * H, 2 * W, C / 2);
                    c.cout = C; c.stride = 2;
                    if ((rc = run(2, c))) return rc;
                    c.out = ds; c.wpk = wt->down_w[s - 1]; c.bias = wt->down_b[s - 1]; c.ksize = 1; c.relu = 0;
                    if ((rc = run(3, c))) return rc;
                }
                resid = ds;
                cur = 0;
                res.last_off = p.buf[s][0];
            } else {
                const int m = (cur + 1) % 3, o = (cur + 2) % 3;
                mid = ws + p.buf[s][m];
                out = ws + p.buf[s][o];
                if ((rc = run(1, conv3(x, mid, nullptr, wi, n, H, W, C)))) return rc;
                resid = x;
                cur = o;
                res.last_off = p.buf[s][o];
            }
            x_split = !fold_in2 && b == 1 && can_split(s);
            if (x_split) out = ws + p.buf[s][3];
            ConvCall c = conv3(mid, out, resid, wi + 1, n, H, W, C);
            if (x_split) { c.split_out = 1; c.split_pixels = pf_alloc_pixels(cap, H / 2, W / 2); }
            if (fold_in2) {
                c.in2 = fold_in2; c.in2_c = C / 2; c.wpk2 = wt->down_w[s - 1]; c.bias2 = wt->down_b[s - 1];
                ProfScope ps(st, 1, 2.0 * n * H * W * (double)C * (C * 9 + C / 2));
                if ((rc = conv_common(c))) return rc;
            } else if ((rc = run(1, c)))
                return rc;
            x = out;
            if (b == 1) res.stage_off[s] = (size_t)((char*)out - ws);
            ++block;
            res.last_stage = s;
            if (block == stop_after) return WSI_OK;
        }
    }
    return WSI_OK;
}

int wsi_trunk_forward(const wsi_trunk_weights* wt, const float* in_f32, const uint8_t* slide,
                      long long slide_pitch_bytes, int slide_h, int slide_w, const int* tile_xy, const float* lut,
                      int n, int h, int w, void* workspace, int workspace_n, float* feat_out, float* logits_out,
                      float* fmap_out, void* stream) {
    TrunkPlan p;
    const int cap = workspace_n > 0 ? workspace_n : n;
    if (!wt || !workspace || n <= 0 || cap < n || trunk_plan(cap, h, w, wt->planes, p)) return WSI_EINVAL;
    if (logits_out && (!wt->head_w || !wt->head_b || wt->head_k <= 0)) return WSI_EINVAL;
    TrunkResult res;
    int rc = trunk_run(wt, {in_f32, slide, slide_pitch_bytes, slide_h, slide_w, tile_xy, lut}, n, cap, h, w, workspace, 8,
                       (hipStream_t)stream, p, res);
    if (rc) return rc;
    const char* last = (const char*)workspace + res.last_off;
    if (feat_out || logits_out) {
        rc = wsi_avgpool_fc(last, n, p.sh[3], p.sw[3], 512, wt->head_w, wt->head_b, wt->head_k, feat_out, logits_out,
                            wt->planes, stream);
        if (rc) return rc;
    }
    if (fmap_out) rc = wsi_pf_unpack(last, fmap_out, n, 512, p.sh[3], p.sw[3], wt->planes, stream);
    return rc;
}

int wsi_trunk_forward_tap(const wsi_trunk_weights* wt, const float* in_f32, const uint8_t* slide,
                          long long slide_pitch_bytes, int slide_h, int slide_w, const int* tile_xy, const float* lut,
                          int n, int h, int w, void* workspace, int workspace_n, int stop_after, float* tap_out_nchw,
                          void* stream) {
    TrunkPlan p;
    const int cap = workspace_n > 0 ? workspace_n : n;
    if (!wt || !workspace || !tap_out_nchw || stop_after < 0 || stop_after > 8 || n <= 0 || cap < n ||
        trunk_plan(cap, h, w, wt->planes, p))
        return WSI_EINVAL;
    TrunkResult res;
    int rc = trunk_run(wt, {in_f32, slide, slide_pitch_bytes, slide_h, slide_w, tile_xy, lut}, n, cap, h, w, workspace,
                       stop_after, (hipStream_t)stream, p, res);
    if (rc) return rc;
    const int stage = res.last_stage;
    return wsi_pf_unpack((const char*)workspace + res.last_off, tap_out_nchw, n, p.sc[stage], p.sh[stage], p.sw[stage], wt->planes,
                         stream);
}

static const int kUnetSkipC[5] = {256, 128, 64, 64, 0};
struct EncMap { int c, h, w; };
static EncMap enc_map(int i, int h, int w) {
    static const int ec[5] = {512, 256, 128, 64, 64};
    return {ec[i], i < 4 ? h >> (5 - i) : h / 2, i < 4 ? w >> (5 - i) : w / 2};
}
struct UnetPlan {
    size_t x0, cat[5], mid[5], out[5], total;
    int r_h[5], r_w[5], cx[5];
};
static int unet_plan(const wsi_unet_decoder_weights* dw, int n, int h, int w, int planes, UnetPlan& u) {
    if (!dw || n <= 0 || h % 32 || w % 32 || planes < 1 || planes > 3) return WSI_EINVAL;
    size_t off = 0;
    u.x0 = off; off += align_up(wsi_pf_bytes(n, h / 2, w / 2, 64, planes), 256);
    int cprev = 512;
    for (int L = 0; L < 5; ++L) {
        u.r_h[L] = (h / 16) << L; u.r_w[L] = (w / 16) << L; u.cx[L] = cprev;
        const int cin = cprev + kUnetSkipC[L], cout = dw->cout[2 * L];
        if (dw->cin[2 * L] != cin || dw->cin[2 * L + 1] != cout || dw->cout[2 * L + 1] != cout || cout % (planes == 1 ? 64 : 32) || cout <= 0) return WSI_EINVAL;
        u.cat[L] = off; off += align_up(wsi_pf_bytes(n, u.r_h[L], u.r_w[L], cin, planes), 256);
        u.mid[L] = off; off += align_up(wsi_pf_bytes(n, u.r_h[L], u.r_w[L], cout, planes), 256);
        u.out[L] = off; off += align_up(wsi_pf_bytes(n, u.r_h[L], u.r_w[L], cout, planes), 256);
        cprev = cout;
    }
    if (dw->head_cin <= 0 || dw->head_cin > cprev || dw->classes <= 0) return WSI_EINVAL;
    u.total = off;
    return WSI_OK;
}

size_t wsi_unet_workspace_bytes(const wsi_unet_decoder_weights* dw, int n, int h, int w, int planes) {
    UnetPlan u;
    const size_t t = wsi_trunk_workspace_bytes(n, h, w, planes);
    return (!t || unet_plan(dw, n, h, w, planes, u)) ? 0 : align_up(t, 256) + u.total;
}

int wsi_unet_workspace_init(const wsi_unet_decoder_weights* dw, void* workspace, int n, int h, int w, int planes, void* stream) {
    UnetPlan u;
    if (!workspace || unet_plan(dw, n, h, w, planes, u)) return WSI_EINVAL;
    int rc = wsi_trunk_workspace_init(workspace, n, h, w, planes, stream);
    if (rc) return rc;
    char* base = (char*)workspace + align_up(wsi_trunk_workspace_bytes(n, h, w, planes), 256);
    return hipMemsetAsync(base, 0, u.total, (hipStream_t)stream) == hipSuccess ? WSI_OK : WSI_EFAULT;
}

static int unet_decoder_run(const wsi_unet_decoder_weights* dw, const UnetPlan& u, const void* const enc[5], int n, int planes, char* dec,
                            float* logits_out, hipStream_t st) {
    const void* x = enc[0];
    int rc = WSI_OK;
    const bool tail = planes == 2 && dw->tail_w && g_routes.unet_tail && u.cx[4] == 32 && kUnetSkipC[4] == 0 && dw->classes <= 4 &&
                      u.r_w[3] % 32 == 0 && u.r_w[3] <= 128 &&
                      (size_t)pf_alloc_pixels(n, u.r_h[3], u.r_w[3]) * 128 <= (size_t)0x7fffffff;
    for (int L = 0; L < (tail ? 4 : 5) && !rc; ++L) {
        const int H = u.r_h[L], W = u.r_w[L], cin = dw->cin[2 * L], cout = dw->cout[2 * L];
        auto conv3 = [&](const void* in, void* out, int j, int ci) {
            return ConvCall{.in = in, .out = out, .wpk = dw->conv_w[j], .bias = dw->conv_b[j], .n = n, .h = H, .w = W, .cin = ci, .cout = cout,
                            .stride = 1, .ksize = 3, .relu = 1, .planes = planes, .stream = st};
        };
        {
            ProfScope ps(st, 6, conv_flops(n, H, W, cin, cout, 9));
            rc = g_routes.unet_fuse_up ? wsi_conv3x3_up_concat_bn_act(x, L < 4 ? enc[L + 1] : nullptr, dec + u.mid[L], dw->conv_w[2 * L], dw->conv_b[2 * L],
                                                                      n, H, W, u.cx[L], kUnetSkipC[L], cout, 1, planes, st)
                                       : WSI_EINVAL;
            if (rc == WSI_EINVAL) ps.relabel(9);
        }
        if (rc == WSI_EINVAL) {
            { ProfScope ps(st, 7, 0.0); rc = wsi_upsample_concat_dispatch(x, L < 4 ? enc[L + 1] : nullptr, dec + u.cat[L], n, H / 2, W / 2, u.cx[L], kUnetSkipC[L], planes, st); }
            ProfScope ps(st, 6, conv_flops(n, H, W, cin, cout, 9));
            if (!rc) rc = conv_common(conv3(dec + u.cat[L], dec + u.mid[L], 2 * L, cin));
        }
        ProfScope ps(st, 6, conv_flops(n, H, W, cout, cout, 9));
        if (!rc) rc = conv_common(conv3(dec + u.mid[L], dec + u.out[L], 2 * L + 1, cout));
        x = dec + u.out[L];
    }
    if (tail) {
        ProfScope ps(st, 10, 2.0 * n * u.r_h[4] * u.r_w[4] * (9.0 * (32.0 * 16.0 + 16.0 * 16.0) + 16.0 * dw->classes));
        if (!rc) rc = wsi_unet_tail_dispatch(x, dw->tail_w, n, u.r_h[3], u.r_w[3], dw->classes, logits_out, st);
        return rc;
    }
    ProfScope ps(st, 8, 2.0 * n * u.r_h[4] * u.r_w[4] * (double)dw->head_cin * dw->classes);
    if (!rc) rc = wsi_unet_head_dispatch(x, n, u.r_h[4], u.r_w[4], dw->cout[9], dw->head_w, dw->head_b, dw->head_cin, dw->classes, logits_out, planes, st);
    return rc;
}

int wsi_unet_forward(const wsi_trunk_weights* wt, const wsi_unet_decoder_weights* dw, const float* in_f32, const uint8_t* slide,
                     long long slide_pitch_bytes, int slide_h, int slide_w, const int* tile_xy, const float* lut, int n, int h,
                     int w, void* workspace, int workspace_n, float* logits_out, float* enc_out[5], void* stream) {
    TrunkPlan p;
    UnetPlan u;
    const int cap = workspace_n > 0 ? workspace_n : n;
    if (!wt || !dw || !workspace || n <= 0 || cap < n || (!logits_out && !enc_out) || h % 32 || w % 32) return WSI_EINVAL;
    if (trunk_plan(cap, h, w, wt->planes, p) || unet_plan(dw, cap, h, w, wt->planes, u)) return WSI_EINVAL;
    const TileSource src = {in_f32, slide, slide_pitch_bytes, slide_h, slide_w, tile_xy, lut};
    if (!src.valid()) return WSI_EINVAL;
    hipStream_t st = (hipStream_t)stream;
    char* ws = (char*)workspace;
    char* dec = ws + align_up(p.total, 256);
    const int planes = wt->planes;
    TrunkResult res;
    const ConvRoutes& r = g_routes;
    const bool x0_fused = r.unet_x0_fused && !in_f32 && planes == 2 && wt->stem_w_u8 && wt->stem_b_u8 && r.stem_u8x && r.stem_fused &&
                          r.stem_shared_weights;
    int rc = trunk_run(wt, src, n, cap, h, w, workspace, 8, st, p, res, {.allow_split = false, .x0_out = x0_fused ? dec + u.x0 : nullptr});
    if (rc) return rc;
    StemArgs a = stem_args(src, wt->stem_w, wt->stem_b, (float*)(ws + p.stem_scratch), n, h, w);
    {
        ProfScope ps(st, 7, 0.0);
        if (x0_fused) {
        } else if (r.unet_fuse_up) {
            a.out_pf = dec + u.x0; a.out_planes = planes;
            rc = wsi_stem_dispatch(a, planes == 1 ? 1 : 2, st);
        } else {
            rc = wsi_stem_dispatch(a, planes == 1 ? 1 : 2, st);
            if (!rc) rc = wsi_nhwc_to_pf_dispatch(a.out, dec + u.x0, n, h / 2, w / 2, 64, planes, st);
        }
    }
    if (rc) return rc;
    const void* enc[5] = {ws + res.stage_off[3], ws + res.stage_off[2], ws + res.stage_off[1], ws + res.stage_off[0], dec + u.x0};
    if (enc_out) {
        for (int i = 0; i < 5 && !rc; ++i) {
            const EncMap m = enc_map(i, h, w);
            if (enc_out[i]) rc = wsi_pf_unpack(enc[i], enc_out[i], n, m.c, m.h, m.w, planes, stream);
        }
        if (rc) return rc;
    }
// ... 26 lines not shown
```

### wsi_segmentation_pipeline_amd/native.py

```python
import contextlib
import ctypes as C
import enum
import os
import subprocess

_HERE = os.path.dirname(os.path.abspath(__file__))
LIB_PATH = os.path.join(_HERE, 'lib', 'libwsi_hip.so')
CSRC = os.path.join(_HERE, 'csrc')

_lib = None


class NativeLibraryMissing(RuntimeError):
    pass


class WsiTrunkWeights(C.Structure):
    _fields_ = [
        ('stem_w', C.c_void_p), ('stem_b', C.c_void_p),
        ('stem_w_u8', C.c_void_p), ('stem_b_u8', C.c_void_p), ('norm', C.c_float * 6),
        ('conv_w', C.c_void_p * 16), ('conv_b', C.c_void_p * 16),
        ('down_w', C.c_void_p * 3), ('down_b', C.c_void_p * 3),
        ('head_w', C.c_void_p), ('head_b', C.c_void_p), ('head_k', C.c_int),
        ('planes', C.c_int),
    ]


class WsiUnetDecoderWeights(C.Structure):
    _fields_ = [
        ('conv_w', C.c_void_p * 10), ('conv_b', C.c_void_p * 10), ('cin', C.c_int * 10), ('cout', C.c_int * 10),
        ('head_w', C.c_void_p), ('head_b', C.c_void_p), ('head_cin', C.c_int), ('classes', C.c_int), ('tail_w', C.c_void_p),
    ]


_vp, _i, _ll, _sz, _f, _d = C.c_void_p, C.c_int, C.c_longlong, C.c_size_t, C.c_float, C.c_double
SIGNATURES = {
    'wsi_hip_abi_version': (_i, []),
    'wsi_pf_bytes': (_sz, [_i, _i, _i, _i, _i]),
    'wsi_pf_pixel_index': (_ll, [_i, _i, _i, _i, _i]),
    'wsi_prepack_conv_bytes': (_sz, [_i, _i, _i, _i]),
    'wsi_prepack_conv': (_i, [_vp, _vp, _vp, _vp, _vp, _f, _i, _i, _i, _i, _vp, _vp]),
    'wsi_unet_tail_prepack_bytes': (_sz, []),
    'wsi_unet_tail_prepack': (_i, [_vp] * 10 + [_f, _vp, _vp, _i, _i, _i, _vp]),
    'wsi_unet_tail_bands': (_i, [_i, _i, _i]),
    'wsi_unet_tail_timeouts': (_i, [C.POINTER(C.c_ulonglong), _i]),
    'wsi_prepack_stem_bytes': (_sz, [_i]),
    'wsi_prepack_stem': (_i, [_vp, _vp, _vp, _vp, _vp, _f, _i, _vp, _vp]),
    'wsi_prepack_stem_u8': (_i, [_vp, _vp, _vp, _vp, _vp, _f, _vp, _vp, _i, _vp, _vp]),
    'wsi_normalize_u8_lut': (_i, [_vp, _vp, _vp]),
    'wsi_stem_conv7x7_bn_relu_maxpool': (_i, [_vp, _vp, _ll, _i, _i, _vp, _vp, _vp, _vp, _vp, _vp, _vp, _i, _i, _i, _vp, _vp, _i, _vp]),
    'wsi_stem_set_mode': (_i, [_i, _i]),
    'wsi_conv3x3_bn_act': (_i, [_vp, _vp, _vp, _vp, _vp, _i, _i, _i, _i, _i, _i, _i, _i, _vp]),
    'wsi_conv3x3_bn_act_cfg': (_i, [_vp, _vp, _vp, _vp, _vp, _i, _i, _i, _i, _i, _i, _i, _i, _i, _vp]),
    'wsi_conv3x3s2_ds_fused': (_i, [_vp, _vp, _vp, _vp, _vp, _vp, _vp, _i, _i, _i, _i, _i, _i, _vp]),
    'wsi_s2_slab_images': (_i, [_i, _i, _i, _i, _i]),
    'wsi_pf_split_bytes': (_sz, [_i, _i, _i, _i, _i]),
    'wsi_conv3x3_bn_act_split': (_i, [_vp] * 5 + [_i] * 7 + [_vp]),
    'wsi_conv3x3_up_concat_bn_act': (_i, [_vp] * 5 + [_i] * 8 + [_vp]),
    'wsi_conv3x3s2_ds_fused_split': (_i, [_vp] * 7 + [_i] * 6 + [_vp]),
    'wsi_conv_set_mode': (_i, [_i]),
    'wsi_conv1x1_bn': (_i, [_vp, _vp, _vp, _vp, _i, _i, _i, _i, _i, _i, _i, _vp]),
    'wsi_avgpool_fc': (_i, [_vp, _i, _i, _i, _i, _vp, _vp, _i, _vp, _vp, _i, _vp]),
    'wsi_linear': (_i, [_vp, _vp, _vp, _vp, _i, _i, _i, _i, _vp]),
    'wsi_pf_pack': (_i, [_vp, _vp, _i, _i, _i, _i, _i, _vp]),
    'wsi_pf_unpack': (_i, [_vp, _vp, _i, _i, _i, _i, _i, _vp]),
    'wsi_trunk_workspace_bytes': (_sz, [_i, _i, _i, _i]),
    'wsi_trunk_workspace_init': (_i, [_vp, _i, _i, _i, _i, _vp]),
    'wsi_trunk_workspace_release': (_i, [_vp]),
    'wsi_trunk_forward': (_i, [C.POINTER(WsiTrunkWeights), _vp, _vp, _ll, _i, _i, _vp, _vp, _i, _i, _i, _vp, _i, _vp, _vp, _vp, _vp]),
    'wsi_trunk_forward_tap': (_i, [C.POINTER(WsiTrunkWeights), _vp, _vp, _ll, _i, _i, _vp, _vp, _i, _i, _i, _vp, _i, _i, _vp, _vp]),
    'wsi_trunk_set_chunks': (_i, [_i, _i]),
    'wsi_prof_begin': (_i, [_i]),
    'wsi_prof_end': (_i, [_vp, _vp, _vp, _i]),
    'wsi_tile_gather': (_i, [_vp, _ll, _i, _i, _vp, _vp, _vp, _i, _i, _i, _vp]),
    'wsi_stitch_add': (_i, [_vp, _vp, _i, _i, _i, _i, _vp, _i, _i, _vp]),
    'wsi_stitch_add_dense': (_i, [_vp, _vp, _i, _i, _i, _i, _vp, _i, _i, _vp]),
    'wsi_softmax_threshold_argmax': (_i, [_vp, _i, _ll, _vp, _vp, _vp, _vp, _i, _vp, _vp]),
    'wsi_ring_create': (_i, [_vp, _i, _sz]),
    'wsi_ring_host_slot': (_vp, [_vp, _i]),
    'wsi_ring_wait_slot': (_i, [_vp, _i]),
    'wsi_ring_submit': (_i, [_vp, _i, _i, _i, _i, _ll, _vp, _ll]),
    'wsi_ring_fence': (_i, [_vp, _vp]),
    'wsi_ring_acquire': (_i, [_vp, _vp]),
    'wsi_ring_device': (_i, [_vp]),
    'wsi_ring_drain': (_i, [_vp]),
    'wsi_ring_destroy': (None, [_vp]),
    'wsi_resample_plan_create': (_i, [_vp, _i, _i, _i, _i]),
    'wsi_resample_plan_destroy': (None, [_vp]),
    'wsi_resample_scratch_bytes': (_sz, [_vp, _i]),
    'wsi_resample_tiles': (_i, [_vp, _vp, _ll, _i, _i, _vp, _i, _vp, _vp, _vp]),
    'wsi_find_nuclei_hsv': (_i, [_vp, _ll, _i, C.c_double, _vp, _vp]),
    'wsi_connected_components_scratch_bytes': (_sz, [_i, _i]),
    'wsi_connected_components': (_i, [_vp, _i, _i, _vp, _vp, _vp, _vp]),
    'wsi_kmeans_points': (_i, [_vp, _i, _vp, _i, _i, _vp, _vp, _vp]),
    'wsi_kmeans_seed_farthest': (_i, [_vp, _i, _i, _vp, _vp, _vp]),
    'wsi_find_nuclei_lab': (_i, [_vp, _ll, _i, _d, _vp, _vp, _vp]),
    'wsi_fill_holes_scratch_bytes': (_sz, [_i, _i]),
    'wsi_fill_holes': (_i, [_vp, _i, _i, _vp, _vp, _vp]),
    'wsi_slic_scratch_bytes': (_sz, [_i, _i, _i]),
    'wsi_slic': (_i, [_vp, _i, _i, _vp, _i, _vp, _i, _i, _i, _d, _d, _i, _vp, _vp, _vp]),
    'wsi_tile_grid_candidates': (_ll, [_i, _i, _i, _i, _i, _i]),
    'wsi_tile_grid_scratch_bytes': (_sz, [_ll]),
    'wsi_tile_grid': (_i, [_i, _i, _i, _i, _i, _i, _vp, _i, _i, C.c_double, C.c_double, _vp, _vp, _vp, _vp]),
    'wsi_exponent_span': (_i, [_vp, _ll, _vp, _vp]),
    'wsi_paint_regions': (_i, [_vp, _vp, _ll, _vp, _vp, _vp, _ll, _vp]),
    'wsi_resize_bilinear_f64': (_i, [_vp, _i, _i, _i, _vp, _i, _i, _vp]),
    'wsi_argmax_classes': (_i, [_vp, _i, _ll, _vp, _vp]),
    'wsi_morph_rect': (_i, [_vp, _vp, _vp, _i, _i, _i, _i, _vp]),
    'wsi_bwperim': (_i, [_vp, _vp, _i, _i, _vp]),
    'wsi_tumor_bed_workspace_bytes': (_sz, [_i, _i]),
    'wsi_convex_hull_image': (_i, [_vp, _vp, _i, _i, _vp, _vp]),
    'wsi_tumor_bed': (_i, [_vp, _i, _i, _i, _i, _i, _vp, _vp, _vp, _vp, _vp]),
    'wsi_hull_polygon': (_i, [_vp, _i, _i, _vp, _i, _vp, _vp]),
    'wsi_mask_iou_counts': (_i, [_vp, _vp, _ll, _vp, _vp]),
    'wsi_score_counts': (_i, [_vp, _vp, _vp, _ll, _vp, _vp]),
    'wsi_esp': (_i, [_vp, _i, _i, _vp, _vp, _vp]),
    'wsi_unet_workspace_bytes': (_sz, [C.POINTER(WsiUnetDecoderWeights), _i, _i, _i, _i]),
    'wsi_unet_workspace_init': (_i, [C.POINTER(WsiUnetDecoderWeights), _vp, _i, _i, _i, _i, _vp]),
    'wsi_unet_forward': (_i, [C.POINTER(WsiTrunkWeights), C.POINTER(WsiUnetDecoderWeights), _vp, _vp, _ll, _i, _i, _vp, _vp, _i, _i, _i,
                              _vp, _i, _vp, C.POINTER(C.c_void_p * 5), _vp]),
    'wsi_resize_nearest_f32': (_i, [_vp, _ll, _i, _i, _vp, _i, _i, _vp]),
    'wsi_unet_decoder': (_i, [C.POINTER(WsiUnetDecoderWeights), C.POINTER(C.c_void_p * 5), _i, _i, _i, _i, _vp, _i, _vp, _vp]),
}


def build(verbose=False):
    res = subprocess.run(['make', '-C', CSRC, '-j8'], stdout=subprocess.PIPE, stderr=subprocess.STDOUT, text=True)
    if verbose or res.returncode:
        print(res.stdout)
    if res.returncode:
        raise RuntimeError('hipcc build of libwsi_hip.so failed')
    global _lib
    _lib = None
    return LIB_PATH


ABI_VERSION = 8


def load():
    global _lib
    if _lib is not None:
        return _lib
    if not os.path.exists(LIB_PATH):
        raise NativeLibraryMissing(
            '%s not found: the WSI inference path has no CPU fallback - build it first '
            '(python -c "import __graft_entry__ as g; g.build()" or make -C %s)' % (LIB_PATH, CSRC))
    lib = C.CDLL(LIB_PATH)
    for name, (res, args) in SIGNATURES.items():
        fn = getattr(lib, name)
        fn.restype = res
        fn.argtypes = args
    if lib.wsi_hip_abi_version() != ABI_VERSION:
        raise RuntimeError('libwsi_hip.so ABI version mismatch')
    _lib = lib
    return lib


class ConvMode(enum.IntFlag):
    S2_GATHER = 0
    S2_SLAB = 1
    S2_SLAB_128 = 3
    XCD_ORDER = 8
    WIDE_FROM_256 = 16
    WIDE_NEVER = 32
    S2_ABLATE = 64
    NO_S2_SPLIT = 128
    XCD_RANGES_OFF = 256
    XCD_RANGES_L1 = 512
    L1_SLAB3 = 1024
    NO_DS_FOLD = 2048
    NO_SLAB_PAIR = 4096
    L1_LINES128 = 16384
    S2_NT2 = 32768
    UNET_CONCAT_PASS = 65536
    WIDE_NO_D8 = 131072
    L1_PERSISTENT = 1048576
    UNET_NO_TAIL = 2097152
    UNET_TAIL_FORM1 = 4194304
    UNET_X0_UNFUSED = 8388608


class StemMode(enum.IntEnum):
    UNFUSED = 0
    FUSED = 1
    FUSED_LUT = 2
    FUSED_ONE_STRIP = 3


@contextlib.contextmanager
def conv_mode(flags=0, base=ConvMode.S2_SLAB):
    lib = load()
    check(lib.wsi_conv_set_mode(int(base) | int(flags)), 'wsi_conv_set_mode')
    try:
        yield
    finally:
        lib.wsi_conv_set_mode(int(ConvMode.S2_SLAB))


@contextlib.contextmanager
def stem_mode(fused, rows=64):
    lib = load()
    check(lib.wsi_stem_set_mode(int(fused), rows), 'wsi_stem_set_mode')
    try:
        yield
    finally:
        lib.wsi_stem_set_mode(int(StemMode.FUSED), 64)


def check(rc, what):
    if rc != 0:
        raise RuntimeError('%s failed with code %d (see include/wsi_hip.h error conventions)' % (what, rc))
```

Before: 117,800 patches/s.

## Fuse final layer4 conv epilogue with global average pool, skip fmap store

```diff
diff --git a/include/wsi_hip.h b/include/wsi_hip.h
--- a/include/wsi_hip.h
+++ b/include/wsi_hip.h
@@ -7,7 +7,7 @@
 extern "C" {
 #endif
 
-#define WSI_HIP_ABI_VERSION 8
+#define WSI_HIP_ABI_VERSION 9
 int wsi_hip_abi_version(void);
 
 size_t wsi_pf_bytes(int n, int h, int w, int c, int planes);
@@ -45,6 +45,8 @@
                        void* stream);
 int wsi_conv1x1_bn(const void* in_pf, void* out_pf, const void* wpk, const float* bias, int n, int h_in, int w_in,
                    int cin, int cout, int stride, int planes, void* stream);
+int wsi_conv3x3_bn_act_avgpool(const void* in_pf, const void* resid_pf, const void* wpk, const float* bias, int n, int h, int w,
+                               int cin, int cout, int relu, int planes, float* feat_out, void* stream);
 int wsi_conv3x3_up_concat_bn_act(const void* up_pf, const void* skip_pf, void* out_pf, const void* wpk, const float* bias, int n, int h, int w,
                                  int c_up, int c_skip, int cout, int relu, int planes, void* stream);
 int wsi_conv3x3s2_ds_fused(const void* in_pf, void* out_conv_pf, void* out_ds_pf, const void* wpk3, const float* bias3,
@@ -78,7 +80,8 @@
     WSI_CONV_MODE_L1_PERSISTENT = 1048576,
     WSI_CONV_MODE_UNET_NO_TAIL = 2097152,
     WSI_CONV_MODE_UNET_TAIL_FORM1 = 4194304,
-    WSI_CONV_MODE_UNET_X0_UNFUSED = 8388608
+    WSI_CONV_MODE_UNET_X0_UNFUSED = 8388608,
+    WSI_CONV_MODE_NO_POOL_FUSE = 16777216
 };
 int wsi_conv_set_mode(int mode);
 int wsi_conv3x3_bn_act_cfg(const void* in_pf, void* out_pf, const void* resid_pf, const void* wpk, const float* bias,
diff --git a/wsi_segmentation_pipeline_amd/csrc/capi.hip b/wsi_segmentation_pipeline_amd/csrc/capi.hip
--- a/wsi_segmentation_pipeline_amd/csrc/capi.hip
+++ b/wsi_segmentation_pipeline_amd/csrc/capi.hip
@@ -46,13 +46,14 @@
 int conv_common(const ConvCall& c) {
     const hipStream_t st = (hipStream_t)c.stream;
     int cfg = c.cfg;
-    if ((!c.in && !(c.in_up && c.up_c == c.cin)) || !c.out || !c.wpk || !c.bias || c.in == c.out || c.in_up == c.out || c.n <= 0) return WSI_EINVAL;
+    if ((!c.in && !(c.in_up && c.up_c == c.cin)) || (!c.out && !c.pool_out) || !c.wpk || !c.bias || c.in == c.out || (c.in_up && c.in_up == c.out) || c.n <= 0) return WSI_EINVAL;
     if (c.line_flags && (c.planes != 3 || c.stride != 1 || c.ksize != 3 || c.cin != 64 || c.cout != 64 || (c.split_out && (c.line_flags & CONV_OUT96)) ||
                          (c.line_flags & ~(CONV_IN96 | CONV_OUT96 | CONV_RESID96)) || ((c.line_flags & CONV_RESID96) && !c.resid)))
         return WSI_EINVAL;
     if ((c.stride != 1 && c.stride != 2) || c.h % c.stride || c.w % c.stride) return WSI_EINVAL;
     if (c.planes == 3 && c.stride == 2 && c.resid) return WSI_EINVAL;
     ConvArgs a = conv_args(c);
+    a.pool_out = c.pool_out;
     a.plane96 = c.line_flags ? (c.plane96 > 0 ? c.plane96 : (long long)pf_alloc_pixels(c.n, c.h, c.w) * 96) : 0;
 #ifdef WSI_STUDY
     if (c.relu & 2) a.flags |= CONV_ABL_NO_STORE;
@@ -81,6 +82,7 @@
 #endif
     a.out_split_pixels = c.split_out ? (c.split_pixels ? c.split_pixels : pf_alloc_pixels(c.n, c.h / 2, c.w / 2)) : 0;
     if (c.split_out && (c.stride != 1 || c.ksize != 3 || c.h % 2 || c.w % 2 || c.planes < 2)) return WSI_EINVAL;
+    if (a.pool_out) return wsi_conv_dispatch(a, c.planes, c.cfg, st);
     if (c.ksize == 3 && c.stride == 2 && c.cout % 128 == 0 && cfg != 0 && g_routes.s2_slab) {
         const int rc = wsi_s2_dispatch(a, c.planes, st);
         if (rc != WSI_EINVAL) return rc;
@@ -145,6 +147,13 @@
                        void* stream) {
     return conv_common({.in = in_pf, .out = out_pf, .resid = resid_pf, .wpk = wpk, .bias = bias, .n = n, .h = h_in, .w = w_in, .cin = cin,
                         .cout = cout, .stride = stride, .ksize = 3, .relu = relu, .planes = planes, .stream = stream});
+}
+
+int wsi_conv3x3_bn_act_avgpool(const void* in_pf, const void* resid_pf, const void* wpk, const float* bias, int n, int h, int w, int cin,
+                               int cout, int relu, int planes, float* feat_out, void* stream) {
+    if (!feat_out) return WSI_EINVAL;
+    return conv_common({.in = in_pf, .out = nullptr, .resid = resid_pf, .wpk = wpk, .bias = bias, .n = n, .h = h, .w = w, .cin = cin, .cout = cout,
+                        .stride = 1, .ksize = 3, .relu = relu, .planes = planes, .stream = stream, .pool_out = feat_out});
 }
 
 size_t wsi_pf_split_bytes(int n, int h, int w, int c, int planes) {
@@ -242,6 +251,7 @@
     r.unet_tail = (mode & WSI_CONV_MODE_UNET_NO_TAIL) ? 0 : 1;
     r.unet_tail_form = (mode & WSI_CONV_MODE_UNET_TAIL_FORM1) ? 1 : 2;
     r.unet_x0_fused = (mode & WSI_CONV_MODE_UNET_X0_UNFUSED) ? 0 : 1;
+    r.pool_fuse = (mode & WSI_CONV_MODE_NO_POOL_FUSE) ? 0 : 1;
     return WSI_OK;
 }
 
diff --git a/wsi_segmentation_pipeline_amd/csrc/common.h b/wsi_segmentation_pipeline_amd/csrc/common.h
--- a/wsi_segmentation_pipeline_amd/csrc/common.h
+++ b/wsi_segmentation_pipeline_amd/csrc/common.h
@@ -101,6 +101,7 @@
     int up_c = 0;
     PFGeom gup = {};
     long long plane96 = 0;
+    float* pool_out = nullptr;
 };
 
 enum : int {
@@ -296,5 +297,6 @@
     int unet_tail = 1;
     int unet_tail_form = 2;
     int unet_x0_fused = 1;
+    int pool_fuse = 1;
 };
 extern ConvRoutes g_routes;
diff --git a/wsi_segmentation_pipeline_amd/csrc/conv.hip b/wsi_segmentation_pipeline_amd/csrc/conv.hip
--- a/wsi_segmentation_pipeline_amd/csrc/conv.hip
+++ b/wsi_segmentation_pipeline_amd/csrc/conv.hip
@@ -723,12 +723,13 @@
 }
 
 
-template <int PLANES, int MINW, int ABL = 0, int WM = 2, int WN = 2, int NT = 2, bool D8 = false>
+template <int PLANES, int MINW, int ABL = 0, int WM = 2, int WN = 2, int NT = 2, bool D8 = false, bool POOL = false>
 __global__ __launch_bounds__(WM* WN * 64, MINW) void conv3x3s1_wide_kernel(ConvArgs a) {
     extern __shared__ __attribute__((aligned(16))) char smem[];
     constexpr int MT = 4, BM = WM * 128, NTHREADS = WM * WN * 64, NTILES = WN * NT, WB = NTILES * 4096;
     constexpr int D8_ZB = 304;
     static_assert(!D8 || (BM == 256 && NTHREADS == 256), "D8: four whole 8 x 8 images per tile, 32 slab pixels per DMA round");
+    static_assert(!POOL || (D8 && PLANES == 3 && ABL == 0), "POOL: whole images per wave, mode-3 line values");
     constexpr int RESID_NBUF = 4;
     char* const wl = smem;
     char* const xl = smem + 2 * WB;
@@ -934,6 +935,12 @@
                 }
             }
         }
+        if constexpr (POOL) {
+            __syncthreads();
+            conv_tail_mx_pool<NT, MT, RESID_NBUF>(a, acc, qs, valid, nb * NTILES + wn * NT, lane, smem + wave * (RESID_NBUF * 4096), slab0,
+                                                  mtile * (BM / 64) + wm * 2, lpix);
+            return;
+        }
         if (a.resid) __syncthreads();
         conv_tail_mx<NT, MT, RESID_NBUF>(a, acc, qs, valid, nb * NTILES + wn * NT, lane, smem + wave * (RESID_NBUF * 4096), slab0);
     } else {
@@ -961,13 +968,19 @@
 }
 
 
-template <int PLANES, int MINW, int ABL = 0, int WM = 2, int WN = 2, int NT = 2, bool D8 = false>
+template <int PLANES, int MINW, int ABL = 0, int WM = 2, int WN = 2, int NT = 2, bool D8 = false, bool POOL = false>
 static int launch_wide(const ConvArgs& a, hipStream_t st) {
     constexpr int BM = WM * 128, NTHREADS = WM * WN * 64, BN = WN * NT * 32;
     if (a.go.C % BN) return WSI_EINVAL;
     if constexpr (!D8 && ABL == 0 && WM == 2 && WN == 2 && NT == 2) {
-        if (g_routes.wide_d8 && a.gi.W == 8 && a.gi.H == 8) return launch_wide<PLANES, MINW, 0, 2, 2, 2, true>(a, st);
-    }
+        if (g_routes.wide_d8 && a.gi.W == 8 && a.gi.H == 8) {
+            if constexpr (PLANES == 3) {
+                if (a.pool_out) return launch_wide<3, MINW, 0, 2, 2, 2, true, true>(a, st);
+            }
+            return launch_wide<PLANES, MINW, 0, 2, 2, 2, true>(a, st);
+        }
+    }
+    if (!POOL && a.pool_out) return WSI_EINVAL;
     const int nblocks = a.go.C / BN;
     const long long R = (long long)a.gi.N * a.gi.H * a.gi.W;
     const int mtiles = (int)((R + BM - 1) / BM);
@@ -977,7 +990,7 @@
     size_t lds = 2 * (BN / 32) * 4096 + xbytes;
     if (PLANES == 3 && lds < (size_t)WM * WN * 4 * 4096) lds = (size_t)WM * WN * 4 * 4096;
     if (lds > 160 * 1024) return WSI_EINVAL;
-    auto k = conv3x3s1_wide_kernel<PLANES, MINW, ABL, WM, WN, NT, D8>;
+    auto k = conv3x3s1_wide_kernel<PLANES, MINW, ABL, WM, WN, NT, D8, POOL>;
     if (lds > 64 * 1024 && hipFuncSetAttribute((const void*)k, hipFuncAttributeMaxDynamicSharedMemorySize, (int)lds) != hipSuccess)
         return WSI_EINVAL;
     const int grid = (a.flags & CONV_XCD_RANGES) ? (mtiles * nblocks + 7) / 8 * 8 : mtiles * nblocks;
@@ -1482,9 +1495,20 @@
     return a.go.C % 128 == 0 ? 30 : 31;
 }
 
+bool wsi_conv_pool_route(int planes, int h, int w, int cout) {
+    return planes == 3 && h == 8 && w == 8 && cout > 0 && cout % 128 == 0 && cout <= 512 && cout >= g_routes.wide_min_c && g_routes.wide_d8;
+}
+
 int wsi_conv_dispatch(const ConvArgs& a, int planes, int cfg, hipStream_t st) {
     const int cout = a.go.C;
     if (planes < 1 || planes > 3) return WSI_EINVAL;
+    if (a.pool_out) {
+        if (!wsi_conv_pool_route(planes, a.gi.H, a.gi.W, cout) || a.stride != 1 || a.ksize != 3 || a.gi.C % 32 || cfg >= 0 || a.in2 || a.in_up ||
+            a.out_split_pixels || a.in_split_pixels || (a.flags & (CONV_IN96 | CONV_OUT96 | CONV_RESID96)) || a.gi.H != a.go.H || a.gi.W != a.go.W ||
+            a.gi.N != a.go.N)
+            return WSI_EINVAL;
+        return wsi_slab_dispatch_cfg(a, planes, 60, st);
+    }
     const int cmul = planes == 1 ? 64 : 32;
     if (a.gi.C % cmul || cout % cmul) return WSI_EINVAL;
     if ((a.gi.C % 64 || cout % 64) && !(a.ksize == 3 && a.stride == 1)) return WSI_EINVAL;
diff --git a/wsi_segmentation_pipeline_amd/csrc/conv_dev.h b/wsi_segmentation_pipeline_amd/csrc/conv_dev.h
--- a/wsi_segmentation_pipeline_amd/csrc/conv_dev.h
+++ b/wsi_segmentation_pipeline_amd/csrc/conv_dev.h
@@ -265,6 +265,27 @@
     }
 }
 
+static __device__ __forceinline__ void mx_identity_frags(bf16x8 (&iw)[4], int lane) {
+    const int h = lane >> 5, l31 = lane & 31;
+    const int p = mx_line_pos(l31), f0 = mx6_field_of_pos(p);
+    f16x8 k0, k1;
+#pragma unroll
+    for (int j = 0; j < 8; ++j) {
+        k0[j] = (p == 8 * h + j) ? (_Float16)1.0f : (_Float16)0.0f;
+        k1[j] = (p == 16 + 8 * h + j) ? (_Float16)1.0f : (_Float16)0.0f;
+    }
+    unsigned q[6];
+#pragma unroll
+    for (int d = 0; d < 6; ++d) {
+        const int bit = 6 * f0 + 3 - 32 * d;
+        q[d] = (h == 0 && bit >= 0 && bit < 32) ? (1u << (bit & 31)) : 0u;
+    }
+    iw[0] = __builtin_bit_cast(bf16x8, k0);
+    iw[1] = __builtin_bit_cast(bf16x8, k1);
+    iw[2] = __builtin_bit_cast(bf16x8, u32x4{q[0], q[1], q[2], q[3]});
+    iw[3] = __builtin_bit_cast(bf16x8, u32x4{q[4], q[5], 127u, 0u});
+}
+
 template <int NT, int MT, int NBUF>
 static __device__ __forceinline__ void conv_tail_mx(const ConvArgs& a, f32x16 (&acc)[NT][MT], const int (&qs)[MT], const bool (&valid)[MT],
                                                     int ntile0, int lane, char* scratch, int slab0) {
@@ -342,6 +363,126 @@
         } else {
             conv_epilogue_mx<MT, NBUF>(a, acc[b0 / MT], qs, valid, ntile0 + b0 / MT, lane, b0 % MT);
         }
+    }
+}
+
+template <int NPG>
+static __device__ __forceinline__ float pool_row_sum(const float* row, int key) {
+    float part[NPG];
+#pragma unroll
+    for (int g = 0; g < NPG; ++g) part[g] = 0.f;
+#pragma unroll
+    for (int k = 0; k < 16; ++k) {
+        const f32x4 x = *(const f32x4*)(row + ((k ^ key) << 2));
+#pragma unroll
+        for (int g = 0; g < 4; ++g) part[(4 * k + g) % NPG] += x[g];
+    }
+    float t = 0.f;
+#pragma unroll
+    for (int g = 0; g < NPG; ++g) t += part[g];
+    return t;
+}
+
+template <int NT, int MT, int NBUF>
+static __device__ __forceinline__ void conv_tail_mx_pool(const ConvArgs& a, f32x16 (&acc)[NT][MT], const int (&qs)[MT], const bool (&valid)[MT],
+                                                         int ntile0, int lane, char* scratch, int slab0, int img0, int lpix) {
+    static_assert(MT == 4 && NBUF == MT, "two images per wave; a residual batch is one channel tile");
+    const int h = lane >> 5, l31 = lane & 31;
+    const float lo_clamp = a.relu ? 0.f : -65504.f;
+    auto quantise = [&](f32x16& v) {
+        f32x16 hi, lo;
+        float ml = 0.f, unused = 0.f;
+#pragma unroll
+        for (int r = 0; r < 16; r += 2) {
+            const float v0 = __builtin_amdgcn_fmed3f(v[r], lo_clamp, 65504.f);
+            const float v1 = __builtin_amdgcn_fmed3f(v[r + 1], lo_clamp, 65504.f);
+            const f16x2 hh = __builtin_convertvector(f32x2{v0, v1}, f16x2);
+            hi[r] = (float)hh[0];
+            hi[r + 1] = (float)hh[1];
+            lo[r] = v0 - hi[r];
+            lo[r + 1] = v1 - hi[r + 1];
+            ml = fmaxf(ml, fmaxf(fabsf(lo[r]), fabsf(lo[r + 1])));
+        }
+        pair_max2(ml, unused);
+        const int sl = mx6_scale_byte(ml);
+        f32x16 lo2 = lo;
+        swap32_halves(lo, lo2);
+        const u32x6 q = mx6_pack32(lo, lo2, sl ? mx_scale_value(sl) : 1.f);
+        const f32x32 dd = mx6_unpack32(q, sl ? mx_scale_value(sl) : 0.f);
+        f32x16 d, dp;
+#pragma unroll
+        for (int r = 0; r < 16; ++r) { d[r] = dd[2 * r]; dp[r] = dd[2 * r + 1]; }
+        swap32_halves(d, dp);
+#pragma unroll
+        for (int r = 0; r < 16; ++r) v[r] = hi[r] + d[r];
+    };
+    float* const rows = (float*)scratch;
+    auto pool = [&](f32x16 (&v)[MT], int ntile) {
+        asm volatile("s_waitcnt lgkmcnt(0)" ::: "memory");
+#pragma unroll
+        for (int mt = 0; mt < MT; ++mt) {
+            const int p = (mt & 1) * 32 + lpix;
+#pragma unroll
+            for (int r = 0; r < 16; ++r) {
+                const int c = 8 * (r >> 2) + 4 * h + (r & 3);
+                rows[((mt >> 1) * 32 + c) * 64 + (p ^ ((c & 15) << 2))] = v[mt][r];
+            }
+        }
+        asm volatile("s_waitcnt lgkmcnt(0)" ::: "memory");
+        const int im = h, c = l31;
+        const float* row = rows + (im * 32 + c) * 64;
+        float t;
+        switch (256 / (a.go.C >> 3)) {
+        case 16: t = pool_row_sum<16>(row, c & 15); break;
+        case 8: t = pool_row_sum<8>(row, c & 15); break;
+        case 5: t = pool_row_sum<5>(row, c & 15); break;
+        default: t = pool_row_sum<4>(row, c & 15); break;
+        }
+        if (h ? valid[2] : valid[0]) a.pool_out[(size_t)(img0 + im) * a.go.C + ntile * 32 + c] = t * (1.0f / 64);
+    };
+    if (a.resid) {
+        const int pixstride = a.go.C * 4;
+        const size_t rbase = (size_t)slab0 * pixstride, rbytes = (size_t)pf_alloc_pixels(a.go.N, a.go.H, a.go.W) * pixstride;
+        const __amdgpu_buffer_rsrc_t rrs = __builtin_amdgcn_make_buffer_rsrc((void*)((const char*)a.resid + rbase), 0,
+                                                                              (int)min(rbytes - rbase, (size_t)0x7fffffff), 0x00020000);
+        bf16x8 iw[4];
+        mx_identity_frags(iw, lane);
+        auto rdma = [&](int nt) {
+#pragma unroll
+            for (int mt = 0; mt < MT; ++mt) {
+                int qr = qs[mt] - slab0;
+                asm volatile("" : "+v"(qr));
+                resid_tile_dma_buf(rrs, qr, pixstride, (ntile0 + nt) * 128, lane, scratch + mt * 4096);
+            }
+        };
+        const int xb = l31 * 128 + ((h ^ ((l31 >> 1) & 7)) << 4);
+        rdma(0);
+#pragma unroll
+        for (int nt = 0; nt < NT; ++nt) {
+            asm volatile("s_waitcnt vmcnt(0)" ::: "memory");
+#pragma unroll
+            for (int mt = 0; mt < MT; ++mt) {
+                const char* t = scratch + mt * 4096;
+                bf16x8 x[4];
+#pragma unroll
+                for (int f = 0; f < 4; ++f) x[f] = *(const bf16x8*)(t + (xb ^ (f << 5)));
+                acc[nt][mt] = mfma_mx6(acc[nt][mt], iw, x);
+            }
+            asm volatile("s_waitcnt lgkmcnt(0)" ::: "memory");
+            if (nt + 1 < NT) rdma(nt + 1);
+            if (nt + 1 < NT) {
+#pragma unroll
+                for (int mt = 0; mt < MT; ++mt) quantise(acc[nt][mt]);
+            }
+        }
+    }
+#pragma unroll
+    for (int nt = 0; nt < NT; ++nt) {
+        if (!a.resid || nt == NT - 1) {
+#pragma unroll
+            for (int mt = 0; mt < MT; ++mt) quantise(acc[nt][mt]);
+        }
+        pool(acc[nt], ntile0 + nt);
     }
 }
 
diff --git a/wsi_segmentation_pipeline_amd/csrc/heads.hip b/wsi_segmentation_pipeline_amd/csrc/heads.hip
--- a/wsi_segmentation_pipeline_amd/csrc/heads.hip
+++ b/wsi_segmentation_pipeline_amd/csrc/heads.hip
@@ -5,6 +5,16 @@
 #pragma unroll
     for (int o = 32; o > 0; o >>= 1) v += __shfl_xor(v, o);
     return v;
+}
+
+static __device__ __forceinline__ void head_fc(const float* f, int C, const float* w, const float* b, int K, int first, int step, int lane,
+                                               float* logits) {
+    for (int k = first; k < K; k += step) {
+        float acc = 0.f;
+        for (int c = lane; c < C; c += 64) acc += f[c] * w[(size_t)k * C + c];
+        acc = wave_sum(acc);
+        if (lane == 0) logits[k] = acc + b[k];
+    }
 }
 
 template <int PLANES>
@@ -73,13 +83,14 @@
     }
     __syncthreads();
     if (!logits) return;
-    const int lane = tid & 63, wave = tid >> 6;
-    for (int k = wave; k < K; k += 4) {
-        float acc = 0.f;
-        for (int c = lane; c < g.C; c += 64) acc += f[c] * w[(size_t)k * g.C + c];
-        acc = wave_sum(acc);
-        if (lane == 0) logits[(size_t)n * K + k] = acc + b[k];
-    }
+    head_fc(f, g.C, w, b, K, tid >> 6, 4, tid & 63, logits + (size_t)n * K);
+}
+
+template <int ROWS>
+__global__ __launch_bounds__(256) void fc_rows_kernel(const float* feat, int N, int C, const float* w, const float* b, int K, float* logits) {
+    const int lane = threadIdx.x & 63;
+    const int n0 = (blockIdx.x * 4 + (threadIdx.x >> 6)) * ROWS;
+    for (int n = n0; n < n0 + ROWS && n < N; ++n) head_fc(feat + (size_t)n * C, C, w, b, K, 0, 1, lane, logits + (size_t)n * K);
 }
 
 template <int BT>
@@ -302,6 +313,13 @@
     return hipGetLastError() == hipSuccess ? WSI_OK : WSI_EFAULT;
 }
 
+int wsi_fc_rows_dispatch(const float* feat, int n, int c, const float* w, const float* b, int K, float* logits, hipStream_t st) {
+    if (!feat || !w || !b || !logits || n <= 0 || c <= 0 || K <= 0) return WSI_EINVAL;
+    constexpr int ROWS = 4;
+    hipLaunchKernelGGL(fc_rows_kernel<ROWS>, dim3((n + 4 * ROWS - 1) / (4 * ROWS)), dim3(256), 0, st, feat, n, c, w, b, K, logits);
+    return hipGetLastError() == hipSuccess ? WSI_OK : WSI_EFAULT;
+}
+
 int wsi_linear_dispatch(const float* x, const float* w, const float* bias, float* y, int B, int K, int J, int relu,
                         hipStream_t st) {
     if (K % 4 || B <= 0 || J <= 0) return WSI_EINVAL;
diff --git a/wsi_segmentation_pipeline_amd/csrc/internal.h b/wsi_segmentation_pipeline_amd/csrc/internal.h
--- a/wsi_segmentation_pipeline_amd/csrc/internal.h
+++ b/wsi_segmentation_pipeline_amd/csrc/internal.h
@@ -5,11 +5,13 @@
 int wsi_s2_dispatch(const ConvArgs& a, int planes, hipStream_t st);
 int wsi_pp_dispatch(const ConvArgs& a, int planes, int cfg, hipStream_t st);
 long long dense_max_slab_pixels(const ConvArgs& a, int BM);
+bool wsi_conv_pool_route(int planes, int h, int w, int cout);
 int wsi_stem_dispatch(const StemArgs& a, int planes, hipStream_t st);
 int wsi_maxpool_dispatch(const float* in, void* out, int N, int Hc, int Wc, int planes, hipStream_t st);
 int wsi_stem_pool_dispatch(const StemArgs& a, void* out_pf, int planes, int rows_per_seg, hipStream_t st, int out96 = 0, long long plane96 = 0, void* x0_pf = nullptr);
 int wsi_avgpool_fc_dispatch(const void* in, const PFGeom& g, const float* w, const float* b, int K, float* feat,
                             float* logits, int planes, hipStream_t st);
+int wsi_fc_rows_dispatch(const float* feat, int n, int c, const float* w, const float* b, int K, float* logits, hipStream_t st);
 int wsi_linear_dispatch(const float* x, const float* w, const float* bias, float* y, int B, int K, int J, int relu,
                         hipStream_t st);
 int wsi_pf_pack_dispatch(const float* in, void* out, const PFGeom& g, int planes, hipStream_t st);
@@ -85,6 +87,7 @@
     int line_flags = 0;
     const void* in_up = nullptr; int up_c = 0;
     long long plane96 = 0;
+    float* pool_out = nullptr;
 };
 int conv_common(const ConvCall& c);
 int s2_split_common(const void* in_split, void* out_conv_pf, void* out_ds_pf, const void* wpk3, const float* bias3, const void* wpk1,
diff --git a/wsi_segmentation_pipeline_amd/csrc/trunk.hip b/wsi_segmentation_pipeline_amd/csrc/trunk.hip
--- a/wsi_segmentation_pipeline_amd/csrc/trunk.hip
+++ b/wsi_segmentation_pipeline_amd/csrc/trunk.hip
@@ -120,6 +120,7 @@
 struct TrunkOpts {
     bool allow_split = true;
     char* x0_out = nullptr;
+    float* pool_out = nullptr;
 };
 static int trunk_run(const wsi_trunk_weights* wt, const TileSource& src, int n, int cap, int h, int w, void* workspace,
                      int stop_after, hipStream_t st, const TrunkPlan& p, TrunkResult& res, const TrunkOpts& opt = {}) {
@@ -232,6 +233,7 @@
             if (x_split) out = ws + p.buf[s][3];
             ConvCall c = conv3(mid, out, resid, wi + 1, n, H, W, C);
             if (x_split) { c.split_out = 1; c.split_pixels = pf_alloc_pixels(cap, H / 2, W / 2); }
+            if (opt.pool_out && s == 3 && b == 1) { c.out = nullptr; c.pool_out = opt.pool_out; }
             if (fold_in2) {
                 c.in2 = fold_in2; c.in2_c = C / 2; c.wpk2 = wt->down_w[s - 1]; c.bias2 = wt->down_b[s - 1];
                 ProfScope ps(st, 1, 2.0 * n * H * W * (double)C * (C * 9 + C / 2));
@@ -256,9 +258,17 @@
     const int cap = workspace_n > 0 ? workspace_n : n;
     if (!wt || !workspace || n <= 0 || cap < n || trunk_plan(cap, h, w, wt->planes, p)) return WSI_EINVAL;
     if (logits_out && (!wt->head_w || !wt->head_b || wt->head_k <= 0)) return WSI_EINVAL;
+    int rc = WSI_OK;
     TrunkResult res;
-    int rc = trunk_run(wt, {in_f32, slide, slide_pitch_bytes, slide_h, slide_w, tile_xy, lut}, n, cap, h, w, workspace, 8,
-                       (hipStream_t)stream, p, res);
+    if (g_routes.pool_fuse && !fmap_out && (feat_out || logits_out) && wsi_conv_pool_route(wt->planes, p.sh[3], p.sw[3], 512)) {
+        float* pooled = feat_out ? feat_out : (float*)((char*)workspace + p.stem_scratch);
+        rc = trunk_run(wt, {in_f32, slide, slide_pitch_bytes, slide_h, slide_w, tile_xy, lut}, n, cap, h, w, workspace, 8,
+                       (hipStream_t)stream, p, res, {.pool_out = pooled});
+        if (rc || !logits_out) return rc;
+        return wsi_fc_rows_dispatch(pooled, n, 512, wt->head_w, wt->head_b, wt->head_k, logits_out, (hipStream_t)stream);
+    }
+    rc = trunk_run(wt, {in_f32, slide, slide_pitch_bytes, slide_h, slide_w, tile_xy, lut}, n, cap, h, w, workspace, 8,
+                   (hipStream_t)stream, p, res);
     if (rc) return rc;
     const char* last = (const char*)workspace + res.last_off;
     if (feat_out || logits_out) {
diff --git a/wsi_segmentation_pipeline_amd/native.py b/wsi_segmentation_pipeline_amd/native.py
--- a/wsi_segmentation_pipeline_amd/native.py
+++ b/wsi_segmentation_pipeline_amd/native.py
@@ -51,6 +51,7 @@
     'wsi_stem_conv7x7_bn_relu_maxpool': (_i, [_vp, _vp, _ll, _i, _i, _vp, _vp, _vp, _vp, _vp, _vp, _vp, _i, _i, _i, _vp, _vp, _i, _vp]),
     'wsi_stem_set_mode': (_i, [_i, _i]),
     'wsi_conv3x3_bn_act': (_i, [_vp, _vp, _vp, _vp, _vp, _i, _i, _i, _i, _i, _i, _i, _i, _vp]),
+    'wsi_conv3x3_bn_act_avgpool': (_i, [_vp] * 4 + [_i] * 7 + [_vp, _vp]),
     'wsi_conv3x3_bn_act_cfg': (_i, [_vp, _vp, _vp, _vp, _vp, _i, _i, _i, _i, _i, _i, _i, _i, _i, _vp]),
     'wsi_conv3x3s2_ds_fused': (_i, [_vp, _vp, _vp, _vp, _vp, _vp, _vp, _i, _i, _i, _i, _i, _i, _vp]),
     'wsi_s2_slab_images': (_i, [_i, _i, _i, _i, _i]),
@@ -135,7 +136,7 @@
     return LIB_PATH
 
 
-ABI_VERSION = 8
+ABI_VERSION = 9
 
 
 def load():
@@ -179,6 +180,7 @@
     UNET_NO_TAIL = 2097152
     UNET_TAIL_FORM1 = 4194304
     UNET_X0_UNFUSED = 8388608
+    NO_POOL_FUSE = 16777216
 
 
 class StemMode(enum.IntEnum):
```

After: 119,300 patches/s (median of 6 runs). +1.3%, better.
